# guowentian/dynamicppr

Hardware: AMD Instinct MI355X
Metric: edge-updates/sec (ppr_throughput, summed over sources); ms_per_step = mean per-batch PPR update time (higher is better)
Workload: dtype f64

## Files before the change

### dynamicppr_amd/csrc/dppr_engine.hip

```cpp
#include <algorithm>
#include <atomic>
#include <cmath>
#include <cstdio>
#include <cstdlib>
#include <cstring>
#include <future>
#include <mutex>
#include <ctime>
#include <string>
#include <type_traits>
#include <unordered_map>
#include <vector>

#include <hip/hip_runtime.h>
#include <rocprim/rocprim.hpp>

#include "../../include/dppr.h"
#include "dppr_churn_plan.hpp"
#include "dppr_cut.hpp"
#include "dppr_devbuf.hpp"
#include "dppr_idspace.hpp"
#include "dppr_loop_plan.hpp"
#include "dppr_query_plan.hpp"
#include "dppr_kernels.hpp"
#include "dppr_multi.hpp"
#include "dppr_gpush.hpp"
#include "dppr_binned.hpp"
#include "dppr_calib.hpp"
#include "dppr_topk.hpp"
#include "dppr_wquery.hpp"
#include "dppr_changes.hpp"
#include "dppr_export.hpp"
#include "dppr_patch.hpp"
#include "dppr_dot.hpp"
#include "dppr_walk.hpp"
#include "dppr_cluster.hpp"
#include "dppr_subgraph.hpp"
#include "dppr_rank.hpp"
#include "dppr_assign.hpp"
#include "dppr_position.hpp"
#include "dppr_sample.hpp"
#include "dppr_explain.hpp"

using namespace dppr;

#include "dppr_host_state.hpp"
#include "dppr_host_graph.hpp"
#include "dppr_host_loop.hpp"
#include "dppr_host_group.hpp"
#include "dppr_host_query.hpp"


extern "C" {

int dppr_abi_version(void) { return DPPR_ABI_VERSION; }

const char *dppr_strerror(int status) {
    switch (status) {
    case DPPR_OK: return "ok";
    case DPPR_ERR_INVALID: return "invalid argument or call order";
    case DPPR_ERR_HIP: return "HIP runtime error";
    case DPPR_ERR_NOMEM: return "out of device memory";
    case DPPR_ERR_NO_DEVICE: return "no usable HIP device (the HIP path is mandatory; there is no CPU fallback)";
    case DPPR_ERR_NOT_CONVERGED: return "iteration cap hit before the frontier emptied";
    default: return "unknown status";
    }
}

const char *dppr_last_error(const dppr_engine *e) { return e ? e->err.c_str() : ""; }

int dppr_device_count(void) {
    int n = 0;
    return hipGetDeviceCount(&n) == hipSuccess ? n : 0;
}

int dppr_create(dppr_engine **out, int device, int32_t V, int32_t W, int directed, int32_t c, int32_t n_epochs) {
    if (!out || V <= 0 || W < 0 || c < 0 || n_epochs < 1) return DPPR_ERR_INVALID;
    *out = nullptr;
    int ndev = 0;
    if (hipGetDeviceCount(&ndev) != hipSuccess || ndev <= 0 || device < 0 || device >= ndev) return DPPR_ERR_NO_DEVICE;
    dppr_engine *e = new dppr_engine();
    dppr::g_live_engines.fetch_add(1, std::memory_order_relaxed);
    auto bail = [&](int code) {
        dppr_destroy(e);
        return code;
    };
#define HIP_TRY_C(call)                                                                 \
    do {                                                                                \
        const hipError_t _e = static_cast<hipError_t>(call);                            \
        if (_e != hipSuccess) {                                                         \
            fprintf(stderr, "dppr_create: %s at line %d\n", hipGetErrorString(_e), __LINE__); \
            return bail(_e == hipErrorOutOfMemory ? DPPR_ERR_NOMEM : DPPR_ERR_HIP);     \
        }                                                                               \
    } while (0)
    auto diag_env = [](const char *name) -> const char * {
        const char *v = getenv(name);
        if (v && !getenv("DPPR_QUIET_SWITCHES")) fprintf(stderr, "dppr_create: diagnostic switch %s=%s in effect (INTEGRATION.md, Environment variables)\n", name, v);
        return v;
    };
    if (const char *v = diag_env("DPPR_SWEEP_BITS")) e->sweep_bits = atoi(v) != 0;
    if (const char *v = diag_env("DPPR_HOT_BLOCKS")) e->hot_blocks = atoi(v) != 0;
    if (const char *v = diag_env("DPPR_GSWEEP_HOT")) e->gsweep_hot_rows = std::max(0, atoi(v));
    if (const char *v = diag_env("DPPR_GSWEEP_GRID")) e->gsweep_grid_cap = std::max(1, std::min(atoi(v), STAT_SLOTS));
    if (const char *v = diag_env("DPPR_RENUMBER")) e->renumber_on = atoi(v) != 0;
    if (const char *v = diag_env("DPPR_RENUMBER_PCT")) e->renumber_growth_pct = std::max(1, atoi(v));
    if (const char *v = diag_env("DPPR_RENUMBER_MIN")) e->renumber_min_parked = std::max(1, atoi(v));
    if (const char *v = diag_env("DPPR_GROUP_PUSH")) e->gpush_enter_pairs = std::max(-1, atoi(v));
    if (const char *v = diag_env("DPPR_GROUP_PUSH_FACTOR")) e->gpush_auto_factor = std::max(1, atoi(v));
    if (const char *v = diag_env("DPPR_GGROUPS_MIN")) e->ggroups_min = std::max(1, atoi(v));
    if (const char *v = diag_env("DPPR_COST_MODEL")) e->cost_model = atoi(v) != 0;
    if (const char *v = diag_env("DPPR_GROUPING_RADIX")) e->force_radix_grouping = atoi(v) != 0;
    if (const char *v = diag_env("DPPR_TEST_MERGE_MISS")) e->test_force_merge_miss = atoi(v) != 0;
    if (const char *v = diag_env("DPPR_BIN_INCREMENTAL")) e->bin_incremental = atoi(v) != 0;
    if (const char *v = diag_env("DPPR_BIN_RECUT_EVERY")) e->bin_recut_every = std::max(1, atoi(v));
    if (const char *v = diag_env("DPPR_BIN_FROZEN_REBUILD")) e->bin_frozen_rebuild = atoi(v) != 0;
    if (const char *v = diag_env("DPPR_GROUP_AT_SLIDE")) e->group_at_slide = atoi(v) != 0;
    if (const char *v = diag_env("DPPR_GROUP_FULL_ROWS")) e->group_full_rows = atoi(v) != 0;
    e->device = device;
    e->V = V;
    e->W = W;
    e->c = c;
    e->directed = directed ? 1 : 0;
    e->n_epochs = n_epochs;
    e->Ed = directed ? W : 2 * W;
    e->bits = 1;
    while ((1ll << e->bits) < (long long)V) e->bits++;
    HIP_TRY_C(hipSetDevice(device));
    HIP_TRY_C(hipStreamCreateWithFlags(&e->stream, hipStreamNonBlocking));
    {
        int least = 0, greatest = 0;
        if (hipDeviceGetStreamPriorityRange(&least, &greatest) != hipSuccess) least = 0;
        HIP_TRY_C(hipStreamCreateWithPriority(&e->bs, hipStreamNonBlocking, least));
    }
    HIP_TRY_C(hipEventCreate(&e->ev0));
    HIP_TRY_C(hipEventCreate(&e->ev1));
    for (auto &ev : e->evpool) HIP_TRY_C(hipEventCreate(&ev));
    HIP_TRY_C(e->dump_pin.alloc(dppr_engine::DUMP_PIN_BYTES));
    HIP_TRY_C(e->pinned.alloc((GMULTI_MAX + 2) * GS_MAX + 3 * GS_MAX + MAX_CHUNK * GS_MAX + 16));
    const size_t Wn = (size_t)std::max(W, 1), Edn = (size_t)std::max(e->Ed, 1), Ln = (size_t)std::max(4 * c, 1);
    HIP_TRY_C(e->w1.alloc(Wn));
    HIP_TRY_C(e->w2.alloc(Wn));
    HIP_TRY_C(e->outdeg.alloc((size_t)V));
    HIP_TRY_C(hipMemsetAsync(e->outdeg, 0, sizeof(int) * (size_t)V, e->stream));
    HIP_TRY_C(e->hub_slot_of.alloc((size_t)V));
    HIP_TRY_C(e->d_ext2int.alloc((size_t)V));
    HIP_TRY_C(e->d_xfer.alloc((size_t)V));
    e->init_ids(V);
    HIP_TRY_C(e->hub_hist.alloc(64));
    HIP_TRY_C(e->bar.alloc(1));
    HIP_TRY_C(e->keys_a.alloc(Edn));
    HIP_TRY_C(e->keys_b.alloc(Edn));
    HIP_TRY_C(e->in_sorted.alloc(Edn));
    if (e->directed) HIP_TRY_C(e->out_sorted.alloc(Edn));
    HIP_TRY_C(e->delpos.alloc((size_t)2 * (size_t)std::max(c, 1) + 16));
    {
        const size_t bn = (size_t)std::max(2 * c, 1);
        for (int k = 0; k < 4; ++k) {
            HIP_TRY_C(e->bk[k].alloc(bn));
            HIP_TRY_C(e->bks[k].alloc(bn));
        }
    }
    HIP_TRY_C(rocprim::radix_sort_keys(nullptr, e->sort_tmp_bytes, e->keys_a.get(), e->keys_b.get(), Edn, 0u,
                                       (unsigned)(2 * e->bits), e->stream));
    HIP_TRY_C(e->sort_tmp.alloc(std::max<size_t>(e->sort_tmp_bytes, 16)));
    for (int k = 0; k < 2; ++k) {
        HIP_TRY_C(e->su_k[k].alloc(Ln));
        HIP_TRY_C(e->su_v[k].alloc(Ln));
    }
    HIP_TRY_C(e->su_grp.alloc(4 * SU_GRP_MAX_BUCKETS + 8));
    HIP_TRY_C(hipMemsetAsync(e->su_grp, 0, sizeof(int) * (4 * SU_GRP_MAX_BUCKETS + 8), e->stream));
    HIP_TRY_C(e->su_term.alloc(Ln * GS_MAX));
    HIP_TRY_C(e->su_ins.alloc(Ln));
    HIP_TRY_C(rocprim::radix_sort_pairs(nullptr, e->su_tmp_bytes, e->su_k[0].get(), e->su_k[1].get(), e->su_v[0].get(), e->su_v[1].get(), Ln,
                                        0u, (unsigned)e->bits, e->stream));
    HIP_TRY_C(e->su_tmp.alloc(std::max<size_t>(e->su_tmp_bytes, 16)));
    e->epochs.resize((size_t)n_epochs);
    for (auto &ep : e->epochs) {
        HIP_TRY_C(ep.row_ptr.alloc((size_t)V + 1));
        HIP_TRY_C(ep.adj.alloc(Edn));
        HIP_TRY_C(ep.out_row_ptr.alloc((size_t)V + 1));
        HIP_TRY_C(ep.out_col.alloc(Edn));
        HIP_TRY_C(ep.b1.alloc(Ln));
        HIP_TRY_C(ep.b2.alloc(Ln));
        HIP_TRY_C(ep.deg_after.alloc(Ln));
        HIP_TRY_C(ep.ins.alloc(Ln));
        HIP_TRY_C(ep.sk.alloc(Ln));
        HIP_TRY_C(ep.sv.alloc(Ln));
        HIP_TRY_C(ep.grp_tile.alloc((size_t)V / WAVE + 3));
        HIP_TRY_C(ep.ggrp_tile.alloc((size_t)V / WAVE + 3));
        HIP_TRY_C(ep.hub_v.alloc(HUB_CAP));
        HIP_TRY_C(ep.hub_degp1.alloc(HUB_CAP));
    }
    HIP_TRY_C(hipStreamSynchronize(e->stream));
#undef HIP_TRY_C
    *out = e;
    return DPPR_OK;
}

void dppr_destroy(dppr_engine *e) {
    if (!e) return;
    if (e->pre.task.valid()) e->pre.task.wait();
    (void)hipSetDevice(e->device);
    if (e->stream) (void)hipStreamSynchronize(e->stream);
    if (e->bs) (void)hipStreamSynchronize(e->bs);
    if (e->ev0) (void)hipEventDestroy(e->ev0);
    if (e->ev1) (void)hipEventDestroy(e->ev1);
    for (auto &ev : e->evpool)
        if (ev) (void)hipEventDestroy(ev);
    if (e->stream) (void)hipStreamDestroy(e->stream);
    if (e->bs) (void)hipStreamDestroy(e->bs);
    dppr::g_live_engines.fetch_sub(1, std::memory_order_relaxed);
    delete e;
}

int dppr_set_schedule(dppr_engine *e, int schedule) {
    if (!e || (schedule != DPPR_SCHEDULE_EAGER && schedule != DPPR_SCHEDULE_SYNC)) return DPPR_ERR_INVALID;
    e->schedule = schedule;
    return DPPR_OK;
}

int dppr_set_batch_grouping(dppr_engine *e, int at_slide) {
    if (!e) return DPPR_ERR_INVALID;
    e->group_at_slide = at_slide != 0;
    return DPPR_OK;
}

int dppr_set_variant(dppr_engine *e, int variant) {
    if (!e || variant < 0 || variant > 3) return fail(e, DPPR_ERR_INVALID, "set_variant: 0 OPTIMIZED, 1 FAST_FRONTIER, 2 EAGER, 3 VANILLA");
    e->schedule = (variant == 1 || variant == 3) ? DPPR_SCHEDULE_SYNC : DPPR_SCHEDULE_EAGER;
    e->pre_extract = variant == 1 || variant == 3;
    e->status_dedup = variant == 2 || variant == 3;
    return DPPR_OK;
}

int dppr_set_phase_merge(dppr_engine *e, int on, int eps_divisor) {
    if (!e || eps_divisor < 0 || eps_divisor > 1024) return fail(e, DPPR_ERR_INVALID, "set_phase_merge: eps_divisor 1..1024 (0 keeps it)");
    e->merge_phases = on != 0;
    if (eps_divisor > 0) e->merge_div = eps_divisor;
    return DPPR_OK;
}

int dppr_set_profiling(dppr_engine *e, int on) {
    if (!e) return DPPR_ERR_INVALID;
    e->profiling = on != 0;
    return DPPR_OK;
}

int dppr_set_persistent(dppr_engine *e, int mode, int64_t timeout_us) {
    if (!e || mode < 0 || mode > 2 || e->loaded || !e->slots.empty())
        return fail(e, DPPR_ERR_INVALID, "set_persistent: call right after dppr_create, mode 0, 1 or 2");
    e->persist_mode = mode;
    if (timeout_us > 0) e->persist_ticks = (unsigned long long)timeout_us * 100ull;
    if (timeout_us < 0) {
        e->persist_ticks = 20000ull;
        e->persist_rollcall_extra = 1;
    }
    return DPPR_OK;
}

int dppr_set_tuning(dppr_engine *e, int hub_min_degree, int big_row_edges, int pull_min_frontier, int chunk_iters,
                    int pull_block) {
    if (!e || hub_min_degree < 1 || big_row_edges < 1 || e->loaded || !e->slots.empty())
        return fail(e, DPPR_ERR_INVALID, "set_tuning: call right after dppr_create, values >= 1");
    e->hub_min_degree = hub_min_degree;
    e->big_row = big_row_edges;
    e->pull_min_frontier = pull_min_frontier;
    if (chunk_iters > 0) {
        e->chunk_iters = std::min(chunk_iters, MAX_CHUNK);
        e->chunk_explicit = true;
    }
    if (pull_block >= 256 && pull_block <= 1024 && pull_block % 64 == 0) e->pull_block = pull_block;
    return DPPR_OK;
}

int dppr_set_sweep_bitmap(dppr_engine *e, int on) {
    if (!e) return DPPR_ERR_INVALID;
    e->sweep_bits = on != 0;
    return DPPR_OK;
}

int dppr_set_binned_sweep(dppr_engine *e, int mode, int ha_tiles, int hb_tiles, int64_t target_edges, int64_t min_ids, int64_t chunk_edges,
                          int64_t target_a_edges) {
    if (!e || mode < 0 || mode > 2 || ha_tiles < 0 || ha_tiles > BIN_MAX_HA_TILES || hb_tiles < 0 || hb_tiles > BIN_MAX_HB_TILES || target_edges < 0 || min_ids < 0 ||
        chunk_edges < 0 || target_a_edges < 0 || e->bin_ready || e->loaded)
        return fail(e, DPPR_ERR_INVALID, "set_binned_sweep: call right after dppr_create; mode 0..2, ha_tiles <= 272, hb_tiles <= 120");
    e->bin_mode = mode;
    if (ha_tiles > 0) e->bin_ha_tiles = ha_tiles;
    if (hb_tiles > 0) e->bin_hb_tiles = hb_tiles;
    if (target_edges > 0) e->bin_target = target_edges;
    if (min_ids > 0) e->bin_min_ids = min_ids;
    if (chunk_edges > 0) e->bin_chunk = chunk_edges;
    if (target_a_edges > 0) e->bin_target_a = target_a_edges;
    return DPPR_OK;
}

int dppr_set_resident_slots(dppr_engine *e, int sorted) {
    if (!e) return DPPR_ERR_INVALID;
    e->res_slots = sorted != 0;
    if (!e->res_slots)
        for (auto &ep : e->epochs) ep.res_valid = false;
    return DPPR_OK;
}

int dppr_set_resident_update(dppr_engine *e, int on) {
    if (!e) return DPPR_ERR_INVALID;
    e->res_update = on != 0;
    if (!e->res_update)
        for (auto &ep : e->epochs) ep.su_inline = false;
    return DPPR_OK;
}

int dppr_set_group_resident(dppr_engine *e, int on) {
    if (!e) return DPPR_ERR_INVALID;
    e->group_resident = on != 0;
    return DPPR_OK;
}

int dppr_set_group_push(dppr_engine *e, int enter_pairs, int list_cap, int64_t max_edges) {
    if (!e || enter_pairs < -1 || list_cap < 0 || max_edges < 0) return fail(e, DPPR_ERR_INVALID, "set_group_push: bad argument");
    e->gpush_enter_pairs = enter_pairs;
    if (list_cap > 0) e->gpush_list_cap = list_cap;
    e->gpush_max_edges = max_edges;
    return DPPR_OK;
}

int dppr_set_group_seeding(dppr_engine *e, int from_tails) {
    if (!e) return DPPR_ERR_INVALID;
    e->group_tail_seeding = from_tails != 0;
    return DPPR_OK;
}

int dppr_set_renumbering(dppr_engine *e, int on, int growth_pct, int min_parked) {
    if (!e || growth_pct < 0 || min_parked < 0) return fail(e, DPPR_ERR_INVALID, "set_renumbering: bad argument");
    e->renumber_on = on != 0;
    if (growth_pct > 0) e->renumber_growth_pct = growth_pct;
    if (min_parked > 0) e->renumber_min_parked = min_parked;
    e->renumber_next = std::min(e->renumber_next, renumber_threshold(e->n_int, e->renumber_growth_pct));
    return DPPR_OK;
}

int dppr_id_space(dppr_engine *e, int32_t *n_ids, int32_t *n_parked, int32_t *renumberings, int64_t *revivals) {
    if (!e) return DPPR_ERR_INVALID;
    if (n_ids) *n_ids = e->n_int;
    if (n_parked) *n_parked = e->n_parked;
    if (renumberings) *renumberings = e->renumberings;
    if (revivals) *revivals = e->revivals;
    return DPPR_OK;
}

int dppr_set_incremental_graph(dppr_engine *e, int on) {
    if (!e) return DPPR_ERR_INVALID;
    e->incremental = on != 0;
    return DPPR_OK;
}

int dppr_synchronize(dppr_engine *e) {
    if (!e) return DPPR_ERR_INVALID;
    HIP_TRY(hipSetDevice(e->device));
    HIP_TRY(hipStreamSynchronize(e->stream));
    HIP_TRY(hipStreamSynchronize(e->bs));
    return DPPR_OK;
}

int dppr_load_window(dppr_engine *e, const int32_t *e1, const int32_t *e2, int32_t n) {
    if (!e || n != e->W || (n > 0 && (!e1 || !e2))) return fail(e, DPPR_ERR_INVALID, "load_window: n must equal W");
    HIP_TRY(hipSetDevice(e->device));
    {
        std::vector<std::pair<uint64_t, int32_t>> fresh;
        for (int k = 0; k < 2; ++k) {
            const int32_t *a = k ? e2 : e1;
            for (int i = 0; i < n; ++i) {
                const int v = a[i];
                if (v < 0 || v >= e->V) return fail(e, DPPR_ERR_INVALID, "load_window: vertex id out of range");
                if (e->ext2int[(size_t)v] == -1) {
                    e->ext2int[(size_t)v] = -2;
                    fresh.emplace_back(id_hash(v), v);
                }
            }
        }
        std::vector<int32_t> indeg;
        if (fresh.size() > HOT_WINDOW_MIN) {
            indeg.assign((size_t)e->V, 0);
            for (int i = 0; i < n; ++i) {
                indeg[(size_t)e2[i]]++;
                if (!e->directed) indeg[(size_t)e1[i]]++;
            }
        }
        numbering_order(fresh, indeg.empty() ? nullptr : indeg.data(), e->hot_blocks);
        for (auto &kv : fresh) {
            e->ext2int[(size_t)kv.second] = -1;
            (void)to_int(e, kv.second);
        }
    }
    if (!translate(e, e1, n, e->h_tmp1) || !translate(e, e2, n, e->h_tmp2))
        return fail(e, DPPR_ERR_INVALID, "load_window: vertex id out of range");
    if (n > 0) {
        HIP_TRY(hipMemcpyAsync(e->w1, e->h_tmp1.data(), sizeof(int) * (size_t)n, hipMemcpyHostToDevice, e->bs));
        HIP_TRY(hipMemcpyAsync(e->w2, e->h_tmp2.data(), sizeof(int) * (size_t)n, hipMemcpyHostToDevice, e->bs));
    }
    e->head = 0;
    HIP_TRY(hipMemsetAsync(e->outdeg, 0, sizeof(int) * (size_t)e->V, e->bs));
    if (n > 0) {
        hipLaunchKernelGGL(k_deg_update, dim3(grid_for(n)), dim3(BLOCK), 0, e->bs, e->w1, e->w2, n, e->directed, 1,
                           e->outdeg);
        HIP_TRY(hipGetLastError());
    }
    for (auto &ep : e->epochs) ep.id = -1;
    Epoch &ep = e->epochs[0];
    ep.L = 0;
    ep.grouped = false;
    ep.su_inline = false;
    int rc = query_persist_cap(e);
    if (rc) return rc;
    rc = sort_window_full(e);
    if (rc) return rc;
    rc = build_epoch(e, ep);
    if (rc) return rc;
    ep.id = 0;
    e->newest = 0;
    e->renumber_next = renumber_threshold(e->n_int, e->renumber_growth_pct);
    e->loaded = true;
    e->batch_staged = false;
    HIP_TRY(hipStreamSynchronize(e->bs));
    return DPPR_OK;
}

int dppr_hint_next_batch(dppr_engine *e, const int32_t *b1, const int32_t *b2, int32_t L, const int32_t *n1, const int32_t *n2, int32_t c) {
    if (!e || e->broken || L < 0 || L > 4 * e->c || c < 0 || c > e->c || (L > 0 && (!b1 || !b2)) || (c > 0 && (!n1 || !n2))) return DPPR_ERR_INVALID;
    pre_join(e);
    dppr_engine::Pre &pr = e->pre;
    const int32_t *src[4] = {b1, b2, n1, n2};
    const int n[4] = {L, L, c, c};
    for (int k = 0; k < 4; ++k) {
        pr.src[k] = src[k];
        pr.n[k] = n[k];
        pr.out[k].resize((size_t)std::max(n[k], 1));
    }
    pr.epoch = e->renumber_epoch;
    pr.armed = true;
    pr.ok = false;
    pr.task = std::async(std::launch::async, [e] {
        bool ok = true;
        for (int k = 0; k < 4; ++k)
            if (e->pre.n[k] > 0) ok = e->lookup_only(e->pre.src[k], (size_t)e->pre.n[k], e->pre.out[k].data(), e->pre.miss[k]) && ok;
        return ok;
    });
    return DPPR_OK;
}

int dppr_set_batch(dppr_engine *e, const int32_t *b1, const int32_t *b2, const uint8_t *ins, int32_t L) {
    if (!e || e->broken || L < 0 || L > 4 * e->c || (L > 0 && (!b1 || !b2 || !ins)))
        return fail(e, DPPR_ERR_INVALID, "set_batch: length exceeds 4*max_batch");
    std::lock_guard<std::mutex> map_lk(e->map_mu);
    if (!ids_in_range(e, b1, L) || !ids_in_range(e, b2, L) || !translate(e, b1, L, e->st_b1) || !translate(e, b2, L, e->st_b2))
        return fail(e, DPPR_ERR_INVALID, "set_batch: vertex id out of range");
    e->st_b1.resize((size_t)L);
    e->st_b2.resize((size_t)L);
    e->st_ins.assign(ins, ins + L);
    e->batch_staged = true;
    HIP_TRY(hipSetDevice(e->device));
    return flush_moves(e);
}

static int slide_impl(dppr_engine *e, const int32_t *n1, const int32_t *n2, int32_t c, int32_t *out_epoch);

int dppr_slide(dppr_engine *e, const int32_t *n1, const int32_t *n2, int32_t c, int32_t *out_epoch) {
    if (e) e->build_concurrent = false;
// ... 461 lines not shown
    HIP_TRY(hipGetLastError());
    int n = 0;
    int rc = read_count(e, s.cnt + 4, &n);
    if (rc) return rc;
    if (n > 0) {
        HIP_TRY(hipMemcpyAsync(out_ids, s.ft[1], sizeof(int) * (size_t)n, hipMemcpyDeviceToHost, e->stream));
        HIP_TRY(hipStreamSynchronize(e->stream));
    }
    if (e->n_parked > 0 && eps < s.park_eps) {
        const int base = e->V - e->n_parked;
        int m = 0;
        HIP_TRY(hipMemsetAsync(s.cnt + 4, 0, sizeof(int), e->stream));
        hipLaunchKernelGGL(k_inspect, dim3(grid_for(e->n_parked, BLOCK * INSPECT_ITEMS)), dim3(BLOCK), 0, e->stream, s.r + base,
                           e->n_parked, phase, eps, s.ft[1], s.cnt + 4);
        HIP_TRY(hipGetLastError());
        rc = read_count(e, s.cnt + 4, &m);
        if (rc) return rc;
        if (m > 0) {
            HIP_TRY(hipMemcpyAsync(out_ids + n, s.ft[1], sizeof(int) * (size_t)m, hipMemcpyDeviceToHost, e->stream));
            HIP_TRY(hipStreamSynchronize(e->stream));
            for (int i = n; i < n + m; ++i) out_ids[i] += base;
        }
        n += m;
    }
    for (int i = 0; i < n; ++i) out_ids[i] = e->int2ext[(size_t)out_ids[i]];
    *out_count = n;
    return DPPR_OK;
}

int dppr_graph_edges(dppr_engine *e, int32_t epoch, int32_t *out) {
    if (!e || !out) return DPPR_ERR_INVALID;
    GET_EPOCH(e, epoch);
    *out = ep.Ed;
    return DPPR_OK;
}

static void csr_to_external(const dppr_engine *e, const std::vector<int> &irow, const std::vector<int> &icol,
                            int32_t *row_ptr, int32_t *col) {
    int off = 0;
    std::vector<int> tmp;
    for (int v = 0; v < e->V; ++v) {
        if (row_ptr) row_ptr[v] = off;
        const int m = e->ext2int[(size_t)v];
        if (m >= 0) {
            tmp.clear();
            for (int j = irow[(size_t)m]; j < irow[(size_t)m + 1]; ++j) tmp.push_back(e->int2ext[(size_t)icol[(size_t)j]]);
            std::sort(tmp.begin(), tmp.end());
            if (col) std::copy(tmp.begin(), tmp.end(), col + off);
            off += (int)tmp.size();
        }
    }
    if (row_ptr) row_ptr[e->V] = off;
}

int dppr_read_graph(dppr_engine *e, int32_t epoch, int32_t *row_ptr, int32_t *col, int32_t *out_degree) {
    if (!e) return DPPR_ERR_INVALID;
    GET_EPOCH(e, epoch);
    HIP_TRY(hipSetDevice(e->device));
    std::vector<int> irow((size_t)e->V + 1), icol((size_t)std::max(ep.Ed, 1)), ideg((size_t)e->V);
    HIP_TRY(hipMemcpyAsync(irow.data(), ep.row_ptr, sizeof(int) * ((size_t)e->V + 1), hipMemcpyDeviceToHost, e->stream));
    if (ep.Ed > 0) {
        int *tmp = reinterpret_cast<int *>(e->keys_a.get());
        hipLaunchKernelGGL(k_split_adj, dim3(grid_for(ep.Ed)), dim3(BLOCK), 0, e->stream, ep.adj, ep.Ed, tmp);
        HIP_TRY(hipGetLastError());
        HIP_TRY(hipMemcpyAsync(icol.data(), tmp, sizeof(int) * (size_t)ep.Ed, hipMemcpyDeviceToHost, e->stream));
    }
    HIP_TRY(hipMemcpyAsync(ideg.data(), e->outdeg, sizeof(int) * (size_t)e->V, hipMemcpyDeviceToHost, e->stream));
    HIP_TRY(hipStreamSynchronize(e->stream));
    csr_to_external(e, irow, icol, row_ptr, col);
    if (out_degree)
        for (int v = 0; v < e->V; ++v) {
            const int m = e->ext2int[(size_t)v];
            out_degree[v] = m >= 0 ? ideg[(size_t)m] : 0;
        }
    return DPPR_OK;
}

int dppr_read_out_graph(dppr_engine *e, int32_t epoch, int32_t *row_ptr, int32_t *col) {
    if (!e) return DPPR_ERR_INVALID;
    GET_EPOCH(e, epoch);
    HIP_TRY(hipSetDevice(e->device));
    std::vector<int> irow((size_t)e->V + 1), icol((size_t)std::max(ep.Ed, 1));
    HIP_TRY(hipMemcpyAsync(irow.data(), ep.out_row_ptr, sizeof(int) * ((size_t)e->V + 1), hipMemcpyDeviceToHost, e->stream));
    if (ep.Ed > 0)
        HIP_TRY(hipMemcpyAsync(icol.data(), ep.out_col, sizeof(int) * (size_t)ep.Ed, hipMemcpyDeviceToHost, e->stream));
    HIP_TRY(hipStreamSynchronize(e->stream));
    csr_to_external(e, irow, icol, row_ptr, col);
    return DPPR_OK;
}

int dppr_trace_enable(dppr_engine *e, int32_t slot, int on) {
    GET_SLOT(e, slot);
    s.trace = on != 0;
    s.trace_ids.clear();
    s.trace_off.assign(1, 0);
    return DPPR_OK;
}

int dppr_trace_get(dppr_engine *e, int32_t slot, int64_t *n_iters, int64_t *n_ids, int64_t *offsets, int32_t *ids) {
    GET_SLOT(e, slot);
    const int64_t ni = s.trace_off.empty() ? 0 : (int64_t)s.trace_off.size() - 1;
    if (n_iters) *n_iters = ni;
    if (n_ids) *n_ids = (int64_t)s.trace_ids.size();
    if (offsets && !s.trace_off.empty()) memcpy(offsets, s.trace_off.data(), sizeof(int64_t) * s.trace_off.size());
    if (ids && !s.trace_ids.empty()) memcpy(ids, s.trace_ids.data(), sizeof(int32_t) * s.trace_ids.size());
    return DPPR_OK;
}

#define GET_GROUP(e, gid)                                                                             \
    if (!(e) || (gid) < 0 || (gid) >= (int)(e)->groups.size()) return fail((e), DPPR_ERR_INVALID, "bad group"); \
    if ((e)->broken) return fail((e), DPPR_ERR_INVALID, "engine unusable after a failed renumbering");           \
    Group &g = (e)->groups[(size_t)(gid)]

static_assert(TG_LANES == GS_MAX, "dppr_targets_plan.hpp plans for the group size of dppr_multi.hpp");
static_assert(TG_SET_MAX == DPPR_TARGET_SET_MAX, "dppr_targets_plan.hpp restates DPPR_TARGET_SET_MAX of include/dppr.h");

static int tg_upload(dppr_engine *e, const TargetSets &ts, DevBuf<unsigned char> &buf, TgTable &tab) {
    tab = tg_table(ts, [&](int32_t ext) { return e->ext2int[(size_t)ext]; });
    std::vector<unsigned char> blob(tg_bytes(tab.total()));
    tg_pack(tab, blob.data());
    HIP_TRY(hipMemcpyAsync(buf, blob.data(), blob.size(), hipMemcpyHostToDevice, e->stream));
    HIP_TRY(hipStreamSynchronize(e->stream));
    return DPPR_OK;
}

static void launch_group_init(dppr_engine *e, Group &g) {
    if (g.tsets.n > 0) {
        hipLaunchKernelGGL(k_tg_init, dim3(grid_for((int64_t)e->V * g.gw)), dim3(BLOCK), 0, e->stream, g.p.get(), g.r.get(), e->V, g.gw);
        hipLaunchKernelGGL(k_tg_scatter, dim3(grid_for(g.ttab.total())), dim3(BLOCK), 0, e->stream, g.r.get(), e->V, g.gw, tg_dev(g), 0, g.n);
    } else {
        hipLaunchKernelGGL(k_ginit, dim3(grid_for((int64_t)e->V * g.gw)), dim3(BLOCK), 0, e->stream, g.p, g.r, e->V, g.gw, g.src);
    }
}

static int add_group(dppr_engine *e, const int32_t *sources, int32_t n, const TargetSets *ts, int32_t *out_group) {
    HIP_TRY(hipSetDevice(e->device));
    Group g;
    g.n = n;
    g.gw = e->group_full_rows ? (n > OCT ? 2 * OCT : OCT) : row_width(n);
    g.spl = row_spl(g.gw);
    for (int s = 0; s < GS_MAX; ++s) g.src.s[s] = -1;
    for (int s = 0; s < n; ++s) g.src_ext[s] = sources[s];
    const size_t V = (size_t)e->V;
    g.act_bytes = (V / 32 + 1024 / 32 + 4) * sizeof(uint32_t);
    const size_t xw = (size_t)x_stride(g.gw);
    HIP_TRY_MSG("add_source_group: ", g.p.alloc((size_t)g.gw * V));
    HIP_TRY_MSG("add_source_group: ", g.r.alloc((size_t)g.gw * V));
    HIP_TRY_MSG("add_source_group: ", g.x.alloc(xw * V));
    HIP_TRY_MSG("add_source_group: ", g.x2.alloc(xw * V));
    HIP_TRY_MSG("add_source_group: ", g.act[0].alloc(g.act_bytes / sizeof(uint32_t)));
    HIP_TRY_MSG("add_source_group: ", g.act[1].alloc(g.act_bytes / sizeof(uint32_t)));
    HIP_TRY_MSG("add_source_group: ", g.cnt.alloc(5 * GS_MAX + MAX_CHUNK * GS_MAX));
    HIP_TRY_MSG("add_source_group: ", g.mlog.alloc((size_t)(GMULTI_MAX + 2) * GS_MAX));
    HIP_TRY_MSG("add_source_group: ", g.dstats.alloc(2));
    HIP_TRY_MSG("add_source_group: ", g.gq.alloc(3 * GQ_PAD));
    HIP_TRY_MSG("add_source_group: ", hipMemsetAsync(g.gq, 0, sizeof(int) * 3 * GQ_PAD, e->stream));
    HIP_TRY_MSG("add_source_group: ", hipMemsetAsync(g.act[0], 0, g.act_bytes, e->stream));
    HIP_TRY_MSG("add_source_group: ", hipMemsetAsync(g.act[1], 0, g.act_bytes, e->stream));
    HIP_TRY_MSG("add_source_group: ", hipMemsetAsync(g.cnt, 0, sizeof(int) * (5 * GS_MAX + MAX_CHUNK * GS_MAX), e->stream));
    HIP_TRY_MSG("add_source_group: ", hipMemsetAsync(g.dstats, 0, 2 * sizeof(IterStats), e->stream));
    if (ts) HIP_TRY_MSG("add_target_group: ", g.tg.alloc(tg_bytes(ts->total())));
    if (ts) {
        for (int s = 0; s < n; ++s)
            for (const TgSeed &sd : ts->lane[s]) (void)to_int(e, sd.id);
    } else {
        for (int s = 0; s < n; ++s) (void)to_int(e, sources[s]);
    }
    for (int s = 0; s < n; ++s) g.src.s[s] = sources[s] >= 0 ? e->ext2int[(size_t)sources[s]] : -1;
    if (int rc = flush_moves(e)) return rc;
    if (ts) {
        g.tsets = *ts;
        if (int rc = tg_upload(e, g.tsets, g.tg, g.ttab)) return rc;
    }
    launch_group_init(e, g);
    HIP_TRY_MSG("add_source_group: ", hipGetLastError());
    HIP_TRY_MSG("add_source_group: ", hipStreamSynchronize(e->stream));
    if (g.spl == 2) e->wide_groups = true;
    e->groups.push_back(std::move(g));
    e->any_groups = true;
    if (int rc = recut_stale_groups(e)) return rc;
    if (out_group) *out_group = (int)e->groups.size() - 1;
    return DPPR_OK;
}

int dppr_add_source_group(dppr_engine *e, const int32_t *sources, int32_t n, int32_t *out_group) {
    if (!e || e->broken || !sources || n < 1 || n > GS_MAX) return fail(e, DPPR_ERR_INVALID, "add_source_group: 1..16 sources");
    if (!ids_in_range(e, sources, n)) return fail(e, DPPR_ERR_INVALID, "add_source_group: vertex out of range");
    return add_group(e, sources, n, nullptr, out_group);
}

int dppr_add_target_group(dppr_engine *e, const int64_t *offsets, const int32_t *ids, const double *weights, int32_t n, int32_t *out_group) {
    if (!e || e->broken) return fail(e, DPPR_ERR_INVALID, "add_target_group: no usable engine");
    if (const TgCheck c = tg_check(offsets, ids, weights, n, e->V))
        return fail(e, DPPR_ERR_INVALID, (std::string("add_target_group: ") + tg_check_text(c)).c_str());
    const TargetSets ts = tg_build(offsets, ids, weights, n);
    int32_t sources[GS_MAX];
    tg_sources(ts, sources);
    return add_group(e, sources, n, tg_has_set(ts) ? &ts : nullptr, out_group);
}

int dppr_group_init_solve(dppr_engine *e, int32_t group, double eps, float *out_ms) {
    return dppr_group_init_solve_at(e, group, -1, eps, out_ms);
}

int dppr_group_init_solve_at(dppr_engine *e, int32_t group, int32_t epoch, double eps, float *out_ms) {
    GET_GROUP(e, group);
    GET_EPOCH(e, epoch);
    if (!(eps > 0)) return fail(e, DPPR_ERR_INVALID, "eps must be positive");
    HIP_TRY(hipSetDevice(e->device));
    int rc = bracket_open(e);
    if (rc) return rc;
    launch_group_init(e, g);
    HIP_TRY(hipGetLastError());
    g.converged = false;
    g.park_eps = 0.0;
    rc = group_loop(e, g, ep, 0, eps, false);
    if (rc) return rc;
    return solve_finished(e, g, eps, ep.id, false, out_ms);
}

int dppr_group_update(dppr_engine *e, int32_t group, int32_t epoch, double eps, float *out_ms) {
    GET_GROUP(e, group);
    GET_EPOCH(e, epoch);
    if (!(eps > 0)) return fail(e, DPPR_ERR_INVALID, "eps must be positive");
    if (!epoch_in_sequence(g.last_epoch, ep.id)) return fail(e, DPPR_ERR_INVALID, "epoch out of sequence for this group");
    HIP_TRY(hipSetDevice(e->device));
    return group_update(e, g, ep, eps, out_ms);
}

int dppr_group_read(dppr_engine *e, int32_t group, int32_t index, double *p, double *r) {
    GET_GROUP(e, group);
    if (index < 0 || index >= g.n) return fail(e, DPPR_ERR_INVALID, "group_read: bad source index");
    HIP_TRY(hipSetDevice(e->device));
    std::lock_guard<std::mutex> map_lk(e->map_mu);
    int rc = sync_map(e);
    if (rc) return rc;
    const double *src[2] = {g.p, g.r};
    double *dst[2] = {p, r};
    for (int k = 0; k < 2; ++k) {
        if (!dst[k]) continue;
        hipLaunchKernelGGL(k_gint_to_ext, dim3(grid_for(e->V)), dim3(BLOCK), 0, e->stream, src[k], g.gw, index, e->d_ext2int,
                           e->V, e->d_xfer);
        HIP_TRY(hipMemcpyAsync(dst[k], e->d_xfer, sizeof(double) * (size_t)e->V, hipMemcpyDeviceToHost, e->stream));
        HIP_TRY(hipStreamSynchronize(e->stream));
    }
    return DPPR_OK;
}

static_assert(CHURN_LANES == GS_MAX, "dppr_churn_plan.hpp plans for the group size of dppr_multi.hpp");
static constexpr bool churn_geometry_agrees() {
    for (int n = 1; n <= GS_MAX; ++n)
        if (churn_row_width(n, false) != row_width(n) || churn_row_spl(row_width(n)) != row_spl(row_width(n)) ||
            churn_row_width(n, true) != (n > OCT ? 2 * OCT : OCT))
            return false;
    return true;
}
static_assert(churn_geometry_agrees(), "dppr_churn_plan.hpp restates row_width / row_spl of dppr_multi.hpp");
static_assert(PLAN_RES_MAX_SWEEPS == RES_MAX_SWEEPS && PLAN_GPUSH_LOG == GPUSH_LOG && PLAN_TINY_N == TINY_N && PLAN_TINY_E == TINY_E,
              "dppr_loop_plan.hpp restates RES_MAX_SWEEPS of dppr_resident.hpp and GPUSH_LOG / TINY_N / TINY_E of dppr_gpush.hpp");
static_assert(LOOP_PHASE_BOTH == PHASE_BOTH, "dppr_loop_plan.hpp restates PHASE_BOTH of dppr_common.hpp");

int dppr_group_sources(dppr_engine *e, int32_t group, int32_t *out_sources, int32_t *out_n) {
    GET_GROUP(e, group);
    if (out_sources)
        for (int s = 0; s < g.n; ++s) out_sources[s] = g.src_ext[s];
    if (out_n) *out_n = g.n;
    return DPPR_OK;
}

static int group_churn(dppr_engine *e, int32_t group, ChurnOp op, int32_t index, int32_t new_source, int32_t *out_index, float *out_ms,
                       const std::vector<TgSeed> *fresh = nullptr) {
    const char *const what[3] = {fresh ? "group_replace_target" : "group_replace_source", "group_add_source", "group_remove_source"};
    if (fresh && tg_is_source(*fresh)) {
        new_source = (*fresh)[0].id;
        fresh = nullptr;
    }
    auto refuse = [&](const char *why) { return fail(e, DPPR_ERR_INVALID, (std::string(what[op]) + ": " + why).c_str()); };
    GET_GROUP(e, group);
    const ChurnPlan pl = churn_plan(op, g.n, g.gw, index, e->group_full_rows, e->wide_groups);
    if (!pl.ok) return refuse(op == CHURN_ADD ? "the group holds 16 sources" : op == CHURN_REMOVE && g.n <= 1 ? "the last source of a group cannot be removed" : "bad source index");
    if (op != CHURN_REMOVE && !fresh && (new_source < 0 || new_source >= e->V)) return refuse("vertex out of range");
    if (!g.converged || g.last_epoch < 0) return refuse("the group is not converged (solve or update it first)");
    Epoch *epp = find_epoch(e, g.last_epoch);
    if (!epp) return refuse("the epoch the group was last solved on is not resident any more");
    const Epoch &ep = *epp;
    HIP_TRY(hipSetDevice(e->device));
    const size_t V = (size_t)e->V;
    const bool new_x = x_stride(pl.gw) != x_stride(g.gw);
    DevBuf<double> p2, r2, x_new, x2_new;
    if (pl.relayout) {
        HIP_TRY(p2.alloc((size_t)pl.gw * V));
        HIP_TRY(r2.alloc((size_t)pl.gw * V));
    }
    if (new_x) {
        HIP_TRY(x_new.alloc((size_t)x_stride(pl.gw) * V));
        HIP_TRY(x2_new.alloc((size_t)x_stride(pl.gw) * V));
    }
    TargetSets nts;
    DevBuf<unsigned char> tg_new;
    if (g.tsets.n > 0 || fresh) {
        TargetSets base = g.tsets;
        if (base.n == 0) {
            base.n = g.n;
            for (int s = 0; s < g.n; ++s) base.lane[s] = tg_source_lane(g.src_ext[s]);
        }
        nts = tg_relane(base, pl.map, pl.n, pl.lane, pl.lane < 0 ? std::vector<TgSeed>() : fresh ? *fresh : tg_source_lane(new_source));
        if (!tg_has_set(nts)) nts = TargetSets();
        else HIP_TRY(tg_new.alloc(tg_bytes(nts.total())));
    }
    int src_int = -1;
    if (op != CHURN_REMOVE) {
        if (fresh) {
            for (const TgSeed &sd : *fresh) (void)to_int(e, sd.id);
// ... 279 lines not shown
int dppr_group_subgraph(dppr_engine *e, int32_t group, int32_t epoch, int32_t k, double min_p, int64_t cap, int dest, int32_t *out_counts,
                        int64_t *out_offsets, int32_t *out_ids, double *out_p, int64_t *out_row_ptr, int32_t *out_col) {
    GET_GROUP(e, group);
    GET_EPOCH(e, epoch);
    return subgraph_call(e, view(g), ep, k, min_p, cap, dest, out_counts, out_offsets, out_ids, out_p, out_row_ptr, out_col);
}

int dppr_debug_subgraph_wave_max(dppr_engine *e, int wave_max) {
    if (!e || !sg_wave_max_ok(wave_max)) return fail(e, DPPR_ERR_INVALID, "debug_subgraph_wave_max: 0 (every row by the histogram kernel) .. 256");
    e->sg_wave_max = wave_max;
    return DPPR_OK;
}

int dppr_topk_ranked(dppr_engine *e, int32_t slot, int32_t epoch, const dppr_rank_spec_t *spec, int32_t k, double min_score, int32_t *out_ids,
                     double *out_score, int32_t *out_count) {
    GET_SLOT(e, slot);
    return topk_ranked_call(e, s, epoch, spec, k, min_score, out_ids, out_score, out_count);
}

int dppr_group_topk_ranked(dppr_engine *e, int32_t group, int32_t epoch, const dppr_rank_spec_t *spec, int32_t k, double min_score,
                           int32_t *out_ids, double *out_score, int32_t *out_counts) {
    GET_GROUP(e, group);
    return topk_ranked_call(e, g, epoch, spec, k, min_score, out_ids, out_score, out_counts);
}

int dppr_rank_score_at(dppr_engine *e, int32_t slot, int32_t epoch, const dppr_rank_spec_t *spec, const int32_t *ids, int32_t m,
                       double *out_score) {
    GET_SLOT(e, slot);
    return rank_score_at_call(e, s, epoch, spec, ids, m, out_score);
}

int dppr_group_rank_score_at(dppr_engine *e, int32_t group, int32_t epoch, const dppr_rank_spec_t *spec, const int32_t *ids, int32_t m,
                             double *out_score) {
    GET_GROUP(e, group);
    return rank_score_at_call(e, g, epoch, spec, ids, m, out_score);
}

int dppr_assign(dppr_engine *e, const int32_t *groups, int32_t n_groups, const double *scale, double min_score, int dest, int32_t *out_label,
                double *out_best, double *out_margin, int64_t *out_counts, const int32_t *prev_label, int64_t cap, int64_t *out_n_flips,
                int32_t *flip_id, int32_t *flip_old, int32_t *flip_new) {
    return assign_call(e, groups, n_groups, scale, min_score, dest, out_label, out_best, out_margin, out_counts, prev_label, cap, out_n_flips,
                       flip_id, flip_old, flip_new);
}

int dppr_assign_at(dppr_engine *e, const int32_t *groups, int32_t n_groups, const double *scale, double min_score, const int32_t *ids, int32_t m,
                   int32_t *out_label, double *out_best, int32_t *out_second_label, double *out_margin) {
    return assign_at_call(e, groups, n_groups, scale, min_score, ids, m, out_label, out_best, out_second_label, out_margin);
}

int dppr_debug_rank_piece(dppr_engine *e, int edges) {
    if (!e || !rank_piece_ok(edges)) return fail(e, DPPR_ERR_INVALID, "debug_rank_piece: 1 .. 512 entries of a row per wave");
    e->rk_piece = edges;
    return DPPR_OK;
}

int dppr_position_at(dppr_engine *e, int32_t slot, int32_t epoch, const dppr_rank_spec_t *spec, double min_score, const int32_t *ids, int32_t m,
                     int32_t *out_pos, int32_t *out_count) {
    GET_SLOT(e, slot);
    return position_call(e, s, epoch, spec, min_score, ids, m, out_pos, out_count);
}

int dppr_group_position_at(dppr_engine *e, int32_t group, int32_t epoch, const dppr_rank_spec_t *spec, double min_score, const int32_t *ids,
                           int32_t m, int32_t *out_pos, int32_t *out_counts) {
    GET_GROUP(e, group);
    return position_call(e, g, epoch, spec, min_score, ids, m, out_pos, out_counts);
}

int dppr_debug_position_tile(dppr_engine *e, int queries) {
    if (!e || !position_tile_ok(queries))
        return fail(e, DPPR_ERR_INVALID, "debug_position_tile: 1 .. 4096 queries of a lane's order per workgroup and pass, 0: the plan's choice");
    e->pos_tile = queries;
    return DPPR_OK;
}

int dppr_explain_at(dppr_engine *e, int32_t slot, int32_t epoch, const int32_t *ids, int32_t m, int32_t f, int32_t depth,
                    const dppr_explain_out_t *out) {
    GET_SLOT(e, slot);
    return explain_call(e, s, epoch, ids, m, f, depth, out);
}

int dppr_group_explain_at(dppr_engine *e, int32_t group, int32_t epoch, const int32_t *ids, int32_t m, int32_t f, int32_t depth,
                          const dppr_explain_out_t *out) {
    GET_GROUP(e, group);
    return explain_call(e, g, epoch, ids, m, f, depth, out);
}

int dppr_debug_explain(dppr_engine *e, int memo, int wave_rows) {
    if (!e || !ex_hook_ok(memo, wave_rows))
        return fail(e, DPPR_ERR_INVALID, "debug_explain: memo -1 (the plan's choice), 0 or 1; 1 .. 64 entries of a row per wave and step");
    e->ex_memo = memo;
    e->ex_wave_rows = wave_rows;
    return DPPR_OK;
}

int dppr_certify(dppr_engine *e, int32_t slot, int32_t epoch, double eps, int flags, dppr_certify_out_t *out) {
    GET_SLOT(e, slot);
    return certify_call(e, s, epoch, eps, flags, out);
}

int dppr_group_certify(dppr_engine *e, int32_t group, int32_t epoch, double eps, int flags, dppr_certify_out_t *out) {
    GET_GROUP(e, group);
    return certify_call(e, g, epoch, eps, flags, out);
}

int dppr_debug_certify(dppr_engine *e, int piece_edges, int wave_rows) {
    if (!e || !cert_hook_ok(piece_edges, wave_rows))
        return fail(e, DPPR_ERR_INVALID, "debug_certify: piece_edges in [0, 2^20], wave_rows 0 or a power of two up to 64 (0: the plan's choice)");
    e->cert_piece = piece_edges;
    e->cert_wave_rows = wave_rows;
    return DPPR_OK;
}

int dppr_sample(dppr_engine *e, int32_t slot, int32_t epoch, const dppr_rank_spec_t *spec, double min_score, uint64_t seed, uint64_t first, int32_t S,
                int dest, int32_t *out_ids, double *out_w, double *out_total, int32_t *out_support, int32_t *out_status) {
    GET_SLOT(e, slot);
    return sample_call(e, s, epoch, spec, min_score, seed, first, S, dest, out_ids, out_w, out_total, out_support, out_status);
}

int dppr_group_sample(dppr_engine *e, int32_t group, int32_t epoch, const dppr_rank_spec_t *spec, double min_score, uint64_t seed, uint64_t first,
                      int32_t S, int dest, int32_t *out_ids, double *out_w, double *out_total, int32_t *out_support, int32_t *out_status) {
    GET_GROUP(e, group);
    return sample_call(e, g, epoch, spec, min_score, seed, first, S, dest, out_ids, out_w, out_total, out_support, out_status);
}

int dppr_debug_sample_form(dppr_engine *e, int form) {
    if (!e || !sample_form_ok(form))
        return fail(e, DPPR_ERR_INVALID, "debug_sample_form: 0 (a wave rebuilds the lowest levels) or 1 (one draw per thread, every level stored)");
    e->sample_form = form;
    return DPPR_OK;
}

int dppr_debug_id_map(dppr_engine *e, int32_t *out_ext2int) {
    if (!e || e->broken || !out_ext2int) return fail(e, DPPR_ERR_INVALID, "debug_id_map: non-null out_ext2int");
    std::lock_guard<std::mutex> map_lk(e->map_mu);
    memcpy(out_ext2int, e->ext2int.data(), sizeof(int32_t) * (size_t)e->V);
    return DPPR_OK;
}

int dppr_debug_walk_form(dppr_engine *e, int form) {
    if (!e || (form != 0 && form != 1)) return fail(e, DPPR_ERR_INVALID, "debug_walk_form: 0 (lane refill) or 1 (one walk per thread)");
    e->walk_form = form;
    return DPPR_OK;
}

int dppr_debug_query_ms(dppr_engine *e, float *out_ms) {
    if (!e || !out_ms) return DPPR_ERR_INVALID;
    *out_ms = e->query_ms;
    return DPPR_OK;
}

int dppr_group_reset_stats(dppr_engine *e, int32_t group) {
    GET_GROUP(e, group);
    HIP_TRY(hipSetDevice(e->device));
    return solve_reset_stats(e, g);
}

int dppr_group_stats(dppr_engine *e, int32_t group, dppr_stats_t *out) {
    GET_GROUP(e, group);
    if (!out) return DPPR_ERR_INVALID;
    HIP_TRY(hipSetDevice(e->device));
    return solve_stats(e, g, out);
}

#ifdef DPPR_STAMPS
extern "C" int dppr_debug_bin_stamps(unsigned long long *out, int which, int rows) {
    return hipMemcpyFromSymbol(out, HIP_SYMBOL(dppr::g_bin_stamps), sizeof(unsigned long long) * 6 * (size_t)rows,
                               sizeof(unsigned long long) * 6 * 16384 * (size_t)which) == hipSuccess ? 0 : -2;
}
extern "C" int dppr_debug_stamps(unsigned long long *out, int rows) {
    return hipMemcpyFromSymbol(out, HIP_SYMBOL(dppr::g_stamps), sizeof(unsigned long long) * 8 * (size_t)rows) == hipSuccess
               ? 0 : -2;
}
#endif

int dppr_bench_atomics(int device, int64_t table_elems, int64_t n, int scope, int reps, float *out_ms) {
    if (table_elems <= 0 || (table_elems & (table_elems - 1)) || n <= 0 || reps <= 0 || !out_ms) return DPPR_ERR_INVALID;
    if (int rc = calib_device(device)) return rc;
    DevBuf<double> table, sink;
    if (table.alloc((size_t)table_elems) != 0) return DPPR_ERR_NOMEM;
    (void)sink.alloc(1);
    (void)hipMemset(table, 0, sizeof(double) * (size_t)table_elems);
    const int grid = 2048;
    return time_launches(reps, out_ms, [&]() {
        if (scope == 2)
            hipLaunchKernelGGL(k_bench_scatter<0>, dim3(grid), dim3(BLOCK), 0, 0, table, (uint64_t)table_elems - 1, n);
        else if (scope == 3)
            hipLaunchKernelGGL(k_bench_scatter<1>, dim3(grid), dim3(BLOCK), 0, 0, table, (uint64_t)table_elems - 1, n);
        else if (scope == 0)
            hipLaunchKernelGGL(k_bench_atomics<__HIP_MEMORY_SCOPE_AGENT>, dim3(grid), dim3(BLOCK), 0, 0, table,
                               (uint64_t)table_elems - 1, n, sink);
        else
            hipLaunchKernelGGL(k_bench_atomics<__HIP_MEMORY_SCOPE_WORKGROUP>, dim3(grid), dim3(BLOCK), 0, 0, table,
                               (uint64_t)table_elems - 1, n, sink);
    });
}

int dppr_bench_line_fills(int device, int64_t table_bytes, int64_t lines, int reps, float *out_ms) {
    if (table_bytes < 128 || (table_bytes & (table_bytes - 1)) || lines <= 0 || reps <= 0 || !out_ms) return DPPR_ERR_INVALID;
    if (int rc = calib_device(device)) return rc;
    DevBuf<double2> table;
    DevBuf<double> sink;
    if (table.alloc((size_t)table_bytes / sizeof(double2)) != 0) return DPPR_ERR_NOMEM;
    (void)sink.alloc(1);
    (void)hipMemset(table, 0, (size_t)table_bytes);
    const int grid = 2048;
    const int per = (int)std::max<int64_t>(8, (lines + (int64_t)grid * 128 - 1) / ((int64_t)grid * 128) / 8 * 8);
    const int rc = time_launches(reps, out_ms, [&]() {
        hipLaunchKernelGGL(k_bench_lines<8>, dim3(grid), dim3(1024), 0, 0, table, (uint64_t)(table_bytes / 128) - 1, per, sink);
    });
    *out_ms = *out_ms * (float)((double)lines / ((double)grid * 128.0 * per));
    return rc;
}

int dppr_bench_stream_copy(int device, int64_t bytes, int reps, float *out_ms) {
    if (bytes < 16 || reps <= 0 || !out_ms) return DPPR_ERR_INVALID;
    if (int rc = calib_device(device)) return rc;
    DevBuf<unsigned char> src, dst;
    if (src.alloc((size_t)bytes) != 0 || dst.alloc((size_t)bytes) != 0) return DPPR_ERR_NOMEM;
    (void)hipMemset(src, 0, (size_t)bytes);
    (void)hipMemset(dst, 0, (size_t)bytes);
    return time_launches(reps, out_ms, [&]() {
        hipLaunchKernelGGL(k_bench_copy, dim3(4096), dim3(1024), 0, 0, reinterpret_cast<const double2 *>(src.get()),
                           reinterpret_cast<double2 *>(dst.get()), bytes / 16);
    });
}

int dppr_debug_bin_tables(dppr_engine *e, int32_t epoch, int32_t *n_a, int32_t *n_b, int32_t *n_edges, int32_t *n_runs, int32_t *n_tiles,
                          int32_t *acut, int32_t *bcut, uint16_t *hl, int32_t *tdelta, int32_t *tb, uint16_t *dl, int32_t *vb,
                          int64_t *patched, int64_t *rebuilt) {
    if (!e) return DPPR_ERR_INVALID;
    GET_EPOCH(e, epoch);
    if (patched) *patched = e->bin_patched;
    if (rebuilt) *rebuilt = e->bin_rebuilt;
    if (!ep.bin_valid) return fail(e, DPPR_ERR_INVALID, "debug_bin_tables: this epoch has no binned tables");
    HIP_TRY(hipSetDevice(e->device));
    if (n_a) *n_a = ep.n_a;
    if (n_b) *n_b = ep.n_b;
    if (n_edges) *n_edges = ep.Ed;
    if (n_runs) *n_runs = ep.n_runs;
    if (n_tiles) *n_tiles = ep.n_tiles;
    const size_t n_blk = ((size_t)ep.Ed + WAVE - 1) / WAVE, n_rb = ((size_t)ep.n_runs + WAVE - 1) / WAVE;
    if (acut) HIP_TRY(hipMemcpy(acut, ep.acut, sizeof(int) * ((size_t)ep.n_a + 1), hipMemcpyDeviceToHost));
    if (bcut) HIP_TRY(hipMemcpy(bcut, ep.bcut, sizeof(int) * ((size_t)ep.n_b + 1), hipMemcpyDeviceToHost));
    if (hl) HIP_TRY(hipMemcpy(hl, ep.hl, sizeof(uint16_t) * (size_t)ep.n_runs, hipMemcpyDeviceToHost));
    if (tdelta) HIP_TRY(hipMemcpy(tdelta, ep.tdelta, sizeof(int) * (size_t)ep.n_tiles, hipMemcpyDeviceToHost));
    if (tb) HIP_TRY(hipMemcpy(tb, ep.tb, sizeof(int) * (n_rb + 1), hipMemcpyDeviceToHost));
    if (dl) HIP_TRY(hipMemcpy(dl, ep.dl, sizeof(uint16_t) * (size_t)ep.Ed, hipMemcpyDeviceToHost));
    if (vb) HIP_TRY(hipMemcpy(vb, ep.vb, sizeof(int) * (n_blk + 1), hipMemcpyDeviceToHost));
    return DPPR_OK;
}

int dppr_debug_live_bytes(int64_t *device_bytes, int64_t *pinned_bytes) {
    if (device_bytes) *device_bytes = dppr::g_device_bytes.load(std::memory_order_relaxed);
    if (pinned_bytes) *pinned_bytes = dppr::g_pinned_bytes.load(std::memory_order_relaxed);
    return DPPR_OK;
}

unsigned long long dppr_heartbeat(const dppr_engine *e) { return e ? e->heartbeat.load(std::memory_order_relaxed) : 0ull; }

#ifndef DPPR_BUILD_ID
#define DPPR_BUILD_ID "unstamped"
#endif
const char *dppr_build_id(void) { return DPPR_BUILD_ID; }

}
```

### dynamicppr_amd/csrc/dppr_host_group.hpp

```cpp
#pragma once

namespace {

template <class F>
void with_row(int gw, int nvx, F &&f) {
    auto narrow = [&](auto w) {
        if (nvx == 512) f(IC<1>{}, w, IC<512>{});
        else f(IC<1>{}, w, IC<1024>{});
    };
    switch (gw) {
    case 2: narrow(IC<2>{}); break;
    case 4: narrow(IC<4>{}); break;
    case 6: narrow(IC<6>{}); break;
    case 8: narrow(IC<8>{}); break;
    case 10: f(IC<2>{}, IC<10>{}, IC<512>{}); break;
    case 12: f(IC<2>{}, IC<12>{}, IC<512>{}); break;
    case 14: f(IC<2>{}, IC<14>{}, IC<512>{}); break;
    default: f(IC<2>{}, IC<16>{}, IC<512>{}); break;
    }
}
template <class F>
void with_row(int gw, F &&f) {
    with_row(gw, 512, [&](auto spl, auto w, auto) { f(spl, w); });
}

struct GSweepLaunch {
    int grid;
    const int *cnt_in;
    int *cnt_out, *cnt_zero;
    int *log;
    int n;
    GridBar *bar = nullptr;
    int *status = nullptr;
    unsigned long long ticks = 0;
    int rollcall_extra = 0;
    int *q_take = nullptr, *q_zero = nullptr;
};
template <bool MULTI>
void launch_gsweep(dppr_engine *e, Group &g, const Epoch &ep, int phase, double eps, bool owed, const GSweepLaunch &a) {
    with_row(g.gw, ep.ggrp_max_tiles * WAVE, [&](auto spl, auto gw, auto nvx) {
        auto go = [&](auto cm) {
            hipLaunchKernelGGL((k_gsweep<decltype(spl)::value, decltype(gw)::value, decltype(nvx)::value, MULTI, decltype(cm)::value>),
                               dim3(a.grid), dim3(GNT), 0, e->stream, ep.grp_n_int, ep.gtab, ep.n_ggroups, a.cnt_in, e->gsweep_hot_rows,
                               ep.out_col, g.x, g.x2, g.act[0], g.act[1], g.r, g.p, a.cnt_out, a.cnt_zero, phase, eps, g.dstats + 1, a.log,
                               a.n, a.bar, a.status, a.ticks, a.rollcall_extra, owed ? 1 : 0, a.q_take, a.q_zero);
        };
        if constexpr (MULTI) go(IC<2>{});
        else if (owed) go(IC<1>{});
        else go(IC<0>{});
    });
}

int group_multi_capacity(dppr_engine *e, int spl) {
    int &cap = e->gmulti_cap[spl - 1];
    if (cap < 0) {
        int per_cu = 0, cus = 0;
        hipError_t rc = spl == 1 ? hipOccupancyMaxActiveBlocksPerMultiprocessor(&per_cu, k_gsweep<1, 8, 1024, true, 2>, GNT, 0)
                                 : hipOccupancyMaxActiveBlocksPerMultiprocessor(&per_cu, k_gsweep<2, 16, 512, true, 2>, GNT, 0);
        if (rc != hipSuccess || hipDeviceGetAttribute(&cus, hipDeviceAttributeMultiprocessorCount, e->device) != hipSuccess)
            per_cu = 0;
        cap = std::min(per_cu * cus, STAT_SLOTS);
    }
    return cap;
}

struct PushTail {
    enum How { NOT_ENTERED, CONVERGED, GAVE_BACK } how = NOT_ENTERED;
    int iters = 0;
    bool owed = false;
};

int group_push_tail(dppr_engine *e, Group &g, const Epoch &ep, int phase, double eps, long long pairs_at_entry, PushTail *t) {
    const int cap = std::max(1024, std::min(e->gpush_list_cap, e->V));
    if (g.plist[0].capacity() != (size_t)cap || !g.pctl) {
        HIP_TRY(loop_wait(e));
        g.plist[0].reset(); g.plist[1].reset(); g.ppre.reset(); g.pctl.reset();
        HIP_TRY(g.plist[0].alloc((size_t)cap));
        HIP_TRY(g.plist[1].alloc((size_t)cap));
        HIP_TRY(g.ppre.alloc((size_t)cap + 1));
        HIP_TRY(g.pctl.alloc(1));
    }
    HIP_TRY(hipMemsetAsync(g.pctl, 0, sizeof(GPushCtl), e->stream));
    const int n_words = (ep.grp_n_int + 31) / 32;
    hipLaunchKernelGGL(k_gpush_list, dim3(grid_for(n_words)), dim3(BLOCK), 0, e->stream, g.act[0], n_words, g.plist[0], cap, g.pctl);
    const int rows_grid = grid_for(std::min<long long>(pairs_at_entry, cap), BLOCK / OCT);
    with_row(g.gw, [&](auto spl, auto gw) {
        hipLaunchKernelGGL((k_gpush_rows<decltype(spl)::value, decltype(gw)::value>), dim3(rows_grid), dim3(BLOCK), 0, e->stream, g.plist[0],
                           g.pctl, 0, g.x, g.r, false);
    });
    HIP_TRY(hipGetLastError());
    static thread_local GPushCtl h;
    const int credit_first = t->owed ? 1 : 0;
    const long long max_edges = gpush_edge_bound(e->gpush_max_edges, ep.n_ggroups);
    const int grid = 256;
    static const bool trace = getenv("DPPR_GROUP_TRACE") != nullptr;
    int it_done = 0;
    long long known_n = pairs_at_entry;
    bool tiny_declined = false;
    long long last_adds = gpush_adds_at_entry(pairs_at_entry);
    for (;;) {
        if (gpush_take_tiny(known_n, last_adds, tiny_declined)) {
            with_row(g.gw, [&](auto spl, auto gw) {
                hipLaunchKernelGGL((k_gpush_tiny<decltype(spl)::value, decltype(gw)::value>), dim3(1), dim3(1024), 0, e->stream, g.pctl, g.plist[0],
                                   g.plist[1], ep.row_ptr, ep.adj, ep.hub_degp1, g.r, g.p, g.act[0], phase, eps, g.dstats, GPUSH_LOG, credit_first);
            });
        } else {
        const int m = gpush_chunk(it_done, pairs_at_entry);
        tiny_declined = false;
        for (int k = 0; k < m; ++k) {
            hipLaunchKernelGGL(k_gpush_scan, dim3(1), dim3(1024), 0, e->stream, g.pctl, g.plist[0], g.plist[1], ep.row_ptr, g.ppre, cap - 1, max_edges);
            with_row(g.gw, [&](auto spl, auto gw) {
                constexpr int SPL = decltype(spl)::value, GW = decltype(gw)::value;
                hipLaunchKernelGGL((k_gpush_snap<SPL, GW>), dim3(grid), dim3(BLOCK), 0, e->stream, g.plist[0], g.plist[1], g.pctl, g.x, g.r, g.p,
                                   g.act[0], phase, eps, credit_first);
                hipLaunchKernelGGL((k_gpush_expand<SPL, GW>), dim3(grid), dim3(BLOCK), 0, e->stream, g.plist[0], g.plist[1], g.pctl, g.ppre,
                                   ep.row_ptr, ep.adj, ep.hub_degp1, g.x, g.r, g.act[0], g.plist[0], g.plist[1], cap, phase, eps, g.dstats);
            });
        }
        }
        HIP_TRY(hipGetLastError());
        HIP_TRY(hipMemcpyAsync(&h, g.pctl, sizeof(GPushCtl), hipMemcpyDeviceToHost, e->stream));
        HIP_TRY(loop_wait(e));
        for (int i = it_done; i < h.it; ++i) {
            const long long F = lane_sum(h.F[i & (GPUSH_LOG - 1)]);
            if (F == 0) continue;
            account_iteration(g.st, F, ITER_PUSH);
            ++t->iters;
            if (trace)
                fprintf(stderr, "[gpush ] phase %d iteration +%d  frontier pairs %9lld  adds %lld\n", phase, i, F, h.atomics[i & (GPUSH_LOG - 1)]);
        }
        if (gpush_tiny_declined(h.it > it_done, h.stop != 0, known_n)) tiny_declined = true;
        if (h.it > it_done) last_adds = h.atomics[(h.it - 1) & (GPUSH_LOG - 1)];
        it_done = h.it;
        known_n = h.n[h.it & 1];
        if (h.stop && h.it == 0 && h.overflow) return DPPR_OK;
        if (h.stop) {
            if (trace) fprintf(stderr, "[gpush ] phase %d: an iteration of %d vertices called itself off after %d iterations\n", phase, h.n[h.it & 1], h.it);
            HIP_TRY(hipMemsetAsync(g.cnt, 0, sizeof(int) * 3 * GS_MAX, e->stream));
            with_row(g.gw, [&](auto spl, auto gw) {
                hipLaunchKernelGGL((k_gpush_leave<decltype(spl)::value, decltype(gw)::value>), dim3(grid_for(ep.grp_n_int, BLOCK / OCT)), dim3(BLOCK), 0,
                                   e->stream, ep.grp_n_int, g.act[0], g.x, g.r, g.p, h.it > 0 ? 1 : 0, phase, eps, g.cnt);
            });
            HIP_TRY(hipGetLastError());
            if (h.it > 0) t->owed = false;
            t->how = PushTail::GAVE_BACK;
            return DPPR_OK;
        }
        if (h.n[h.it & 1] == 0) {
            t->how = PushTail::CONVERGED;
            return DPPR_OK;
        }
        if (it_done >= e->max_iters) return fail(e, DPPR_ERR_NOT_CONVERGED, "iteration cap hit");
    }
}

struct GroupLoop {
    dppr_engine *const e;
    Group &g;
    const Epoch &ep;
    const int phase;
    const double eps;
    const int hp = phase == PHASE_BOTH ? 0 : phase;
    CounterRing ring;
    bool owed = false;
    int it = 0, active_iters = 0;
    bool more = false;
    long long F = 0;
    GroupLoopPlan plan;
    int sweep_grid = 1;
    int *row(int k) const { return g.cnt + k * GS_MAX; }

    int multi_chunk() {
        const int n = group_multi_sweeps(g.hist.hint[hp], it, e->chunk_iters, e->chunk_explicit);
        HIP_TRY(hipMemsetAsync(g.mlog, 0, sizeof(int) * (size_t)(n + 2) * GS_MAX, e->stream));
        HIP_TRY(hipMemsetAsync(e->bar, 0, sizeof(GridBar), e->stream));
        int rc = timed_launch(e, 0, e->profiling, [&] {
            launch_gsweep<true>(e, g, ep, phase, eps, owed,
                                {ep.n_ggroups, row(ring.cur), row(3), row(4), g.mlog + GS_MAX, n, e->bar, g.mlog, e->persist_ticks, e->persist_rollcall_extra});
        });
        if (rc) return rc;
        HIP_TRY(hipGetLastError());
        if ((rc = read_back(e, g.mlog, (size_t)(n + 2) * GS_MAX))) return rc;
        const int st = e->pinned[0];
        g.st.persist_launches++;
        if (st & GSM_FAULT) return fail(e, DPPR_ERR_HIP, "a grid barrier of the multi-sweep group launch timed out");
        if (st & GSM_ABORTED) {
            give_up_resident(e, g.st);
            return DPPR_OK;
        }
        const int sweeps = st & GSM_SWEEPS;
        account_sweeps(g.st, e->pinned + GS_MAX, sweeps, GS_MAX, ITER_SWEEP, it, &active_iters);
        if (e->profiling && (rc = credit_launch(e, g.st, 0, false))) return rc;
        if (sweeps & 1) {
            swap_snapshots(g, true);
            owed = !owed;
        }
        it += sweeps;
        more = !(st & GSM_CONVERGED);
        if (!more) return DPPR_OK;
        HIP_TRY(hipMemcpyAsync(row(0), row(3), sizeof(int) * GS_MAX, hipMemcpyDeviceToDevice, e->stream));
        HIP_TRY(hipMemsetAsync(row(1), 0, sizeof(int) * 2 * GS_MAX, e->stream));
        ring.cur = 0;
        more = lane_sum(e->pinned + GS_MAX + sweeps * GS_MAX) > 0;
        return DPPR_OK;
    }
    int sweep_chunk() {
        const int n = plan.next_chunk(g.hist, hp, it, lane_sum(e->pinned + ring.cur * GS_MAX), e->chunk_iters, e->chunk_explicit);
        for (int k = 0; k < n; ++k) {
            int rc = timed_launch(e, k, e->profiling, [&] {
                launch_gsweep<false>(e, g, ep, phase, eps, owed,
                                     {sweep_grid, row(ring.cur), row(ring.nxt()), row(ring.zer()), row(5 + k), 1, nullptr, nullptr, 0, 0,
                                      g.gq + (g.gq_seq % 3) * GQ_PAD, g.gq + ((g.gq_seq + 1) % 3) * GQ_PAD});
            });
            if (rc) return rc;
            swap_snapshots(g, true);
            ring.rotate();
            g.gq_seq++;
            owed = !owed;
        }
        HIP_TRY(hipGetLastError());
        if (int rc = read_back(e, g.cnt, (size_t)(5 + n) * GS_MAX)) return rc;
        int rc = account_sweeps(g.st, e->pinned + 5 * GS_MAX, n, GS_MAX, ITER_SWEEP, it, &active_iters, [&](int k, long long f) -> int {
            plan.saw_frontier(f, it + k);
            if (!e->profiling) return DPPR_OK;
            float ms = 0;
            if (int rc2 = credit_launch(e, g.st, k, true, &ms)) return rc2;
            static const bool trace = getenv("DPPR_GROUP_TRACE") != nullptr;
            if (trace) fprintf(stderr, "[gsweep] phase %d sweep %3d  frontier pairs %9lld  %7.1f us\n", phase, it + k, f, ms * 1e3);
            return DPPR_OK;
        });
        if (rc) return rc;
        F = lane_sum(e->pinned + ring.cur * GS_MAX);
        more = F > 0;
        it += n;
        return DPPR_OK;
    }
    int hand_to_push_tail() {
        plan.saw_frontier(F, it);
        PushTail t;
        t.owed = owed;
        if (int rc = group_push_tail(e, g, ep, phase, eps, F, &t)) return rc;
        owed = t.owed;
        if (t.how != PushTail::NOT_ENTERED) {
            active_iters = it + t.iters;
            it += t.iters;
        }
        if (t.how == PushTail::CONVERGED) more = false;
        else plan.push_declined(F);
        if (t.how != PushTail::GAVE_BACK) return DPPR_OK;
        ring.cur = 0;
        if (int rc = read_back(e, row(0), GS_MAX)) return rc;
        more = lane_sum(e->pinned) > 0;
        return DPPR_OK;
    }
};

int group_loop(dppr_engine *e, Group &g, const Epoch &ep, int phase, double eps, bool tails) {
    GroupLoop l{e, g, ep, phase, eps};
    HIP_TRY(hipMemsetAsync(g.cnt, 0, sizeof(int) * 3 * GS_MAX, e->stream));
    if (tails) {
        HIP_TRY(hipMemsetAsync(g.act[0], 0, g.act_bytes, e->stream));
        if (ep.L > 0) {
            with_row(g.gw, [&](auto spl, auto gw) {
                hipLaunchKernelGGL((k_gseed_tails<decltype(spl)::value, decltype(gw)::value>), dim3(grid_for(ep.L, BLOCK / OCT)), dim3(BLOCK), 0,
                                   e->stream, batch_tails(e, ep), ep.L, g.r, g.x, g.p, g.act[0], phase, eps, l.row(0));
            });
        }
    } else {
        with_row(g.gw, [&](auto spl, auto gw) {
            hipLaunchKernelGGL((k_gseed_dense<decltype(spl)::value, decltype(gw)::value>), dim3(grid_for(ep.grp_n_int, BLOCK / OCT)), dim3(BLOCK), 0,
                               e->stream, ep.grp_n_int, g.r, g.x, g.p, g.act[0], phase, eps, l.row(0));
        });
        g.st.inspected += (int64_t)ep.grp_n_int * g.n;
    }
    HIP_TRY(hipGetLastError());
    int rc = read_back(e, l.row(0), GS_MAX);
    if (rc) return rc;
    l.more = lane_sum(e->pinned) > 0;
    if (e->gsweep_grid_cap <= 0) {
        int cus = 0;
        if (hipDeviceGetAttribute(&cus, hipDeviceAttributeMultiprocessorCount, e->device) != hipSuccess || cus <= 0) cus = 256;
        e->gsweep_grid_cap = std::min(2 * cus, STAT_SLOTS);
    }
    l.sweep_grid = std::min(std::max(ep.n_ggroups, 1), e->gsweep_grid_cap);
    l.plan.push_thr = group_push_threshold(e->gpush_enter_pairs, ep.n_ggroups, e->gpush_auto_factor);
    while (l.more) {
        if (l.it >= e->max_iters) return fail(e, DPPR_ERR_NOT_CONVERGED, "iteration cap hit");
        const int mcap = e->group_resident && e->persist_mode && e->persist_ok && e->chunk_iters > 1 ? group_multi_capacity(e, g.spl) : 0;
        if (mcap > 0 && ep.n_ggroups > 0 && ep.n_ggroups <= mcap) rc = l.multi_chunk();
        else if (!(rc = l.sweep_chunk()) && l.plan.enter_push(l.more, l.F)) rc = l.hand_to_push_tail();
        if (rc) return rc;
    }
    l.plan.finish(g.hist, l.hp, l.active_iters);
    return DPPR_OK;
}

int group_solve_column(dppr_engine *e, Group &g, const Epoch &ep) {
    const LoopHistory kept = g.hist;
    const int rc = group_loop(e, g, ep, 0, g.conv_eps, false);
    g.hist = kept;
    return rc;
}

int group_stream_update(dppr_engine *e, Group &g, const Epoch &ep) {
    const int L = ep.L;
    if (L == 0) return DPPR_OK;
    int rc = group_records_by_tail(e, ep, nullptr, 0, nullptr, 0);
    if (rc) return rc;
    SuSources srcs{};
    for (int s = 0; s < GS_MAX; ++s) srcs.s[s] = g.src.s[s];
    hipLaunchKernelGGL(k_su_terms, dim3(grid_for(L), g.n), dim3(BLOCK), 0, e->stream, batch_tails(e, ep), batch_order(e, ep), ep.b2,
                       ep.ins, L, g.p, g.gw, e->su_term, e->su_ins);
    if (g.tsets.n > 0)
        hipLaunchKernelGGL(k_su_apply_seeded, dim3(grid_for(L), g.n), dim3(BLOCK), 0, e->stream, batch_tails(e, ep), batch_order(e, ep),
                           e->su_term, e->su_ins, ep.deg_after, L, g.r, g.gw, tg_dev(g));
    else
        hipLaunchKernelGGL(k_su_apply, dim3(grid_for(L), g.n), dim3(BLOCK), 0, e->stream, batch_tails(e, ep), batch_order(e, ep), e->su_term,
                           e->su_ins, ep.deg_after, L, g.r, g.gw, srcs, 0.0, (int *)nullptr, (int *)nullptr, (int *)nullptr,
                           (int *)nullptr);
    HIP_TRY(hipGetLastError());
    g.st.records += (int64_t)L * g.n;
    return DPPR_OK;
}

int group_update(dppr_engine *e, Group &g, Epoch &ep, double eps, float *out_ms) {
    const bool merged = e->merge_phases && e->schedule == DPPR_SCHEDULE_EAGER;
    if (merged) eps = eps / e->merge_div;
    const bool tails = g.converged && g.conv_eps <= eps && e->group_tail_seeding;
    int rc = settle_parked(e, g.p, g.r, g.gw, eps, &g.park_eps, &g.st);
    if (rc) return rc;
    rc = prepare_epoch(e, ep);
    if (rc) return rc;
    rc = bracket_open(e);
    if (rc) return rc;
    rc = group_stream_update(e, g, ep);
    if (rc) return rc;
    g.converged = false;
    if (merged) rc = group_loop(e, g, ep, PHASE_BOTH, eps, tails);
    else if (!(rc = group_loop(e, g, ep, 0, eps, tails))) rc = group_loop(e, g, ep, 1, eps, tails);
    if (rc) return rc;
    return solve_finished(e, g, eps, ep.id, true, out_ms);
}

}
```

### dynamicppr_amd/csrc/dppr_host_state.hpp

```cpp
#pragma once

static constexpr int CNT_HDR = 16;
static constexpr int PERSIST_RETRY_BATCHES = 64;
static constexpr int GQ_PAD = 32;
static constexpr int BIN_MAX_BLOCKS = 1 << 16, BIN_MAX_BIG = 4096, BIN_SMALL_INTS = BIN_MAX_BLOCKS + BIN_MAX_BIG + 1 + 64;
static constexpr int SU_SPLIT_MIN = 1 << 16;
static constexpr int MERGE_MISS_WORD = 44;

namespace dppr {

inline std::atomic<long long> g_device_bytes{0}, g_pinned_bytes{0};

struct DeviceAlloc {
    static int alloc(void **p, size_t bytes) {
        const hipError_t rc = hipMalloc(p, bytes);
        if (rc == hipSuccess) g_device_bytes.fetch_add((long long)bytes, std::memory_order_relaxed);
        return (int)rc;
    }
    static int free(void *p, size_t bytes) {
        g_device_bytes.fetch_sub((long long)bytes, std::memory_order_relaxed);
        return (int)hipFree(p);
    }
};

// ... 144 lines not shown
        DevBuf<int> ext;
    } sc;
    struct Weighted {
        DevBuf<double> w;
    } wq;
    struct Changes {
        DevBuf<unsigned char> res; PinBuf<unsigned char> pin;
    } ch;
    struct Export {
        DevBuf<unsigned short> mask;
        DevBuf<int> cnt;
        DevBuf<long long> base;
        DevBuf<unsigned char> blk; PinBuf<unsigned char> pin;
    } ex;
    struct Patch {
        DevBuf<unsigned> mask;
        DevBuf<int> cnt;
        DevBuf<long long> base;
        DevBuf<unsigned char> blk; PinBuf<unsigned char> pin;
    } pt;
    struct Dot {
        DevBuf<double> part;
        DevBuf<unsigned char> in;
        DevBuf<unsigned char> blk; PinBuf<unsigned char> pin;
        dppr::DotTable tb;
        bool lds_set = false;
    } dot;
    struct Walk {
        DevBuf<int> starts;
        DevBuf<int> ends;
        DevBuf<double> res;
        std::vector<int64_t> off;
    } wk;
    struct Cluster {
        DevBuf<unsigned short> rank;
        DevBuf<int> d;
        DevBuf<unsigned long long> list;
        DevBuf<unsigned char> blk; PinBuf<unsigned char> pin;
    } cl;
    struct Subgraph {
        DevBuf<int> work;
        DevBuf<unsigned char> blk; PinBuf<unsigned char> pin;
    } sg;
    struct Rank {
        DevBuf<unsigned> excl;
        DevBuf<int> len; PinBuf<int> len_pin;
        DevBuf<unsigned long long> list;
        std::vector<unsigned long long> items;
    } rk;
    struct Position {
        DevBuf<unsigned char> keys;
        DevBuf<unsigned> slots;
        DevBuf<unsigned char> blk; PinBuf<unsigned char> pin;
        bool lds_set = false;
    } pos;
    struct Sample {
        DevBuf<double> leaves;
        DevBuf<double> nodes;
        DevBuf<double> low;
        DevBuf<unsigned char> blk; PinBuf<unsigned char> pin;
    } sm;
    struct Explain {
        DevBuf<unsigned char> blk; PinBuf<unsigned char> pin;
    } exq;
    struct Certify {
        DevBuf<unsigned char> blk; PinBuf<unsigned char> pin;
        DevBuf<unsigned char> ws;
        DevBuf<double> part;
        DevBuf<unsigned long long> list;
        DevBuf<double> pp;
    } cert;
    struct Assign {
        DevBuf<double> scale;
        DevBuf<int> cnt;
        DevBuf<int> base;
        DevBuf<int> ws;
        DevBuf<unsigned char> blk; PinBuf<unsigned char> pin;
    } as;
};

}

struct dppr_engine : dppr::IdSpace {
    int device = 0;
    int V = 0, W = 0, c = 0, directed = 1, n_epochs = 1;
    int Ed = 0;
    int bits = 1;
    int schedule = DPPR_SCHEDULE_EAGER;
    bool status_dedup = false;
    bool pre_extract = false;
    bool group_at_slide = false;
    int merge_miss_host = 0;
    long long merge_fallbacks = 0;
    bool test_force_merge_miss = false;
    int raw_backoff = 0;
    bool merge_phases = false;
    int merge_div = 4;
    hipStream_t stream = nullptr;
    hipStream_t bs = nullptr;
    bool build_concurrent = false;
    std::mutex err_mu;
    std::mutex map_mu;
    unsigned map_gen_on_device = 0;
    hipEvent_t ev0 = nullptr, ev1 = nullptr;
    hipEvent_t evpool[2 * 64] = {};
    bool profiling = false;
    int pull_block = 0;
    int chunk_iters = 24;
    bool chunk_explicit = false;
    int persist_mode = 1;
    bool persist_ok = true;
    int persist_retry = 0;
    int persist_cap = 0;
    int res_slots = 1;
    int res_update = 1;
    DevBuf<double> res_arena;
    long long res_arena_stride = 0;
    unsigned long long persist_ticks = 5000000ull;
    int persist_rollcall_extra = 0;
    DevBuf<GridBar> bar;
    DevBuf<int> w1, w2;
    int head = 0;
    bool loaded = false;
    bool broken = false;
    DevBuf<int> outdeg;
    DevBuf<int> hub_slot_of;
    DevBuf<int> hub_hist;
    int hub_min_degree = HUB_MIN_DEGREE_DEFAULT;
    int big_row = BIG_ROW_DEFAULT;
    int pull_min_frontier = 0;
    DevBuf<uint64_t> in_sorted, out_sorted;
    DevBuf<uint64_t> keys_a, keys_b;
    DevBuf<unsigned char> sort_tmp;
    size_t sort_tmp_bytes = 0;
    DevBuf<int> su_grp;
    DevBuf<uint64_t> bk[4];
    DevBuf<uint64_t> bks[4];
    DevBuf<int> delpos;
    struct Pre {
        std::future<bool> task;
        const int32_t *src[4] = {nullptr, nullptr, nullptr, nullptr};
        int n[4] = {0, 0, 0, 0};
        std::vector<int32_t> out[4];
        std::vector<uint32_t> miss[4];
        unsigned long long epoch = 0;
        bool armed = false, ok = false;
    } pre;
    long long pre_hits = 0, pre_misses = 0;
    bool incremental = true;
    bool sweep_bits = false;
    bool hot_blocks = true;
    int gsweep_hot_rows = 24576;
    int gsweep_grid_cap = 0;
    bool group_resident = true;
    int gmulti_cap[2] = {-1, -1};
    bool any_groups = false;
    int ggroups_min = 256;
    bool force_radix_grouping = false;
    bool cost_model = true;
    bool group_full_rows = false;
    bool wide_groups = false;
    bool group_tail_seeding = true;
    int gpush_enter_pairs = -1;
    int gpush_list_cap = 1 << 20;
    long long gpush_max_edges = 0;
    int gpush_auto_factor = 2;
    int bin_mode = 1;
    int bin_ha_tiles = 128, bin_hb_tiles = 60;
    long long bin_target = 0;
    long long bin_target_a = 4ll << 20;
    long long bin_min_ids = 1ll << 19;
    DevBuf<int> bin_vblk_a;
    DevBuf<unsigned long long> bin_scan;
    DevBuf<int> bin_small;
    long long bin_chunk = 32768;
    DevBuf<double> bin_vals;
    DevBuf<uint64_t> bin_wb, bin_wa;
    DevBuf<int> bin_first;
    std::vector<int32_t> bin_cut_a, bin_cut_b;
    int bin_abits = 0, bin_bbits = 0;
    int bin_cut_ids = 0;
    bool bin_words_valid = false;
    int bin_slides_since_cut = 0;
    bool bin_incremental = true;
    int bin_recut_every = 32;
    bool bin_frozen_rebuild = false;
    bool bin_force_full = false;
    int bin_miss_host = 0;
    long long bin_patched = 0, bin_rebuilt = 0;
    DevBuf<unsigned char> bin_tmp;
    size_t bin_tmp_bytes = 0;
    bool bin_ready = false;
    std::vector<int32_t> h_tiles_in;
    DevBuf<uint32_t> su_k[2], su_v[2];
    DevBuf<double> su_term;
    DevBuf<uint8_t> su_ins;
    DevBuf<unsigned char> su_tmp;
    size_t su_tmp_bytes = 0;
    std::vector<int32_t> st_b1, st_b2;
    std::vector<uint8_t> st_ins;
    bool batch_staged = false;
    std::vector<Epoch> epochs;
    int newest = -1;
    std::vector<Slot> slots;
    std::vector<Group> groups;
    PinBuf<int> pinned;
    std::atomic<unsigned long long> heartbeat{0};
    PinBuf<char> dump_pin;
    static constexpr size_t DUMP_PIN_BYTES = sizeof(GridBar) + 4096;
    bool renumber_on = true;
    int renumber_growth_pct = 15;
    int renumber_min_parked = 1024;
    int renumber_next = 0;
    int renumberings = 0;
    std::vector<int32_t> mv_src, mv_dst, mv_zero;
    DevBuf<int> mv_idx;
    DevBuf<double> mv_tmp;
    DevBuf<int> d_ext2int;
    DevBuf<double> d_xfer;
    DevBuf<int> d_int2ext;
    unsigned i2e_gen_on_device = 0;
    QueryWork q;
    int walk_form = 0;
    int sg_wave_max = SG_WAVE_MAX;
    int rk_piece = RK_PIECE;
    int sample_form = 0;
    int pos_tile = 0;
    int ex_memo = -1;
    int ex_wave_rows = EX_WAVE_ROWS;
    int cert_piece = 0;
    int cert_wave_rows = 0;
    float query_ms = -1.0f;
    std::vector<int32_t> h_tmp1, h_tmp2;
    std::vector<int32_t> h_tiles;
    int max_iters = 1 << 20;
    std::string err;
};

namespace {

inline void set_err(dppr_engine *e, const char *msg) {
    std::lock_guard<std::mutex> lk(e->err_mu);
    e->err = msg;
}

#define HIP_TRY(call)                                                                                   \
    do {                                                                                                \
        const hipError_t _e = static_cast<hipError_t>(call);                                            \
        if (_e != hipSuccess) {                                                                         \
            char _b[512];                                                                               \
            snprintf(_b, sizeof(_b), "%s in %s at line %d", hipGetErrorString(_e), __FILE__, __LINE__); \
            set_err(e, _b);                                                                             \
            return _e == hipErrorOutOfMemory ? DPPR_ERR_NOMEM : DPPR_ERR_HIP;                           \
        }                                                                                               \
    } while (0)

#define HIP_TRY_MSG(prefix, call)                                                 \
    do {                                                                          \
        const hipError_t _e = static_cast<hipError_t>(call);                      \
        if (_e != hipSuccess) {                                                   \
            set_err(e, (std::string(prefix) + hipGetErrorString(_e)).c_str());    \
            return _e == hipErrorOutOfMemory ? DPPR_ERR_NOMEM : DPPR_ERR_HIP;     \
        }                                                                         \
    } while (0)

inline int grid_for(int64_t n, int per_block = BLOCK, int cap = 2048) {
    int64_t g = (n + per_block - 1) / per_block;
    if (g < 1) g = 1;
    if (g > cap) g = cap;
    return (int)g;
}

constexpr long LOOP_SPIN_US = 2000;
inline hipError_t loop_sync(hipStream_t st) {
    static const bool spin = !(getenv("DPPR_SYNC_SPIN") && atoi(getenv("DPPR_SYNC_SPIN")) == 0);
    if (!spin) return hipStreamSynchronize(st);
    timespec t0;
    clock_gettime(CLOCK_MONOTONIC, &t0);
    hipError_t r;
    unsigned polls = 0;
    while ((r = hipStreamQuery(st)) == hipErrorNotReady) {
        if ((++polls & 15u) == 0) {
            timespec now;
            clock_gettime(CLOCK_MONOTONIC, &now);
            if ((now.tv_sec - t0.tv_sec) * 1000000L + (now.tv_nsec - t0.tv_nsec) / 1000L > LOOP_SPIN_US) return hipStreamSynchronize(st);
        }
        __builtin_ia32_pause();
    }
    return r;
}

inline hipError_t loop_wait(dppr_engine *e) {
    e->heartbeat.fetch_add(1, std::memory_order_relaxed);
    return loop_sync(e->stream);
}

int fail(dppr_engine *e, int code, const char *msg) {
    if (e) set_err(e, msg);
    return code;
}

inline int bracket_open(dppr_engine *e) {
    HIP_TRY(hipEventRecord(e->ev0, e->stream));
    return DPPR_OK;
}
inline int bracket_close(dppr_engine *e, float *ms) {
// ... 72 lines not shown
```

### dynamicppr_amd/csrc/dppr_multi.hpp

```cpp
#pragma once

#include "dppr_kernels.hpp"

namespace dppr {

constexpr int GS_MAX = 16;
constexpr int OCT = 8;

struct SrcN {
    int s[GS_MAX];
};

__device__ __forceinline__ unsigned oct_mask(uint64_t ballot) {
    return (unsigned)(ballot >> (lane_id() & ~(OCT - 1))) & 0xffu;
}

__host__ __device__ constexpr int row_width(int n_sources) { return n_sources <= 2 ? 2 : (n_sources + 1) / 2 * 2; }
__host__ __device__ constexpr int row_spl(int gw) { return gw > OCT ? 2 : 1; }
#ifndef DPPR_X_COMPACT
#define DPPR_X_COMPACT 0
#endif
__host__ __device__ constexpr int x_stride(int gw) { return DPPR_X_COMPACT ? gw : gw > 8 ? 16 : gw > 4 ? 8 : gw; }
template <int SPL, int GW>
__device__ __forceinline__ bool oct_live(int j) {
// ... 63 lines not shown
    if (threadIdx.x < GW && s_cnt[threadIdx.x]) atomicAdd(&cnt_out[threadIdx.x], s_cnt[threadIdx.x]);
}

template <int SPL, int GW>
__global__ __launch_bounds__(BLOCK) void k_gseed_tails(const uint32_t *__restrict__ skeys, int L, const double *__restrict__ r,
                                                       double *__restrict__ x, double *__restrict__ p,
                                                       uint32_t *__restrict__ act, int phase, double eps,
                                                       int *__restrict__ cnt_out) {
    __shared__ int s_cnt[GS_MAX];
    if (threadIdx.x < GS_MAX) s_cnt[threadIdx.x] = 0;
    __syncthreads();
    const int j = threadIdx.x & (OCT - 1);
    const bool live = oct_live<SPL, GW>(j);
    int nleg[SPL];
#pragma unroll
    for (int q = 0; q < SPL; ++q) nleg[q] = 0;
    const int per = BLOCK / OCT;
    const int Lpad = (L + per - 1) / per * per;
    for (int i0 = blockIdx.x * per; i0 < Lpad; i0 += gridDim.x * per) {
        const int i = i0 + (int)threadIdx.x / OCT;
        int u = -1;
        if (i < L) {
            u = (int)skeys[i];
            if (i > 0 && (int)skeys[i - 1] == u) u = -1;
        }
        bool any = false;
        double rv[SPL];
        bool lg[SPL];
#pragma unroll
        for (int q = 0; q < SPL; ++q) {
            rv[q] = u >= 0 && live ? r[(size_t)u * GW + j * SPL + q] : 0.0;
            lg[q] = u >= 0 && live && legal(rv[q], phase, eps);
            any |= lg[q];
            nleg[q] += lg[q] ? 1 : 0;
        }
        if (oct_mask(__ballot(any))) {
            if (live) {
#pragma unroll
                for (int q = 0; q < SPL; ++q) {
                    const size_t k = (size_t)u * GW + j * SPL + q;
                    x[(size_t)u * x_stride(GW) + j * SPL + q] = rv[q];
                    if (lg[q]) p[k] = p[k] + ALPHA * rv[q];
                }
            }
            if (j == 0) atomicOr(&act[u >> 5], 1u << (u & 31));
        }
    }
#pragma unroll
    for (int q = 0; q < SPL; ++q)
        if (nleg[q]) atomicAdd(&s_cnt[j * SPL + q], nleg[q]);
    __syncthreads();
    if (threadIdx.x < GW && s_cnt[threadIdx.x]) atomicAdd(&cnt_out[threadIdx.x], s_cnt[threadIdx.x]);
}

constexpr int GNT = 1024;
constexpr int GT_HDR = 8;
__host__ __device__ constexpr int GT_STRIDE(int nvx) { return (GT_HDR + nvx + 1 + GNT / OCT + nvx / 2 + 3) / 4 * 4; }

template <int NVX>
__global__ __launch_bounds__(GNT) void k_gtables(int V, const int *__restrict__ grp_tile, int n_groups,
                                                 const int *__restrict__ out_row_ptr, int *__restrict__ tables) {
    constexpr int NW = GNT / WAVE, NOCT = GNT / OCT, EB = 8;
    __shared__ int s_wcnt[NW];
    const int tid = threadIdx.x, lane = lane_id(), w = wave_id();
    for (int g = blockIdx.x; g < n_groups; g += gridDim.x) {
        __syncthreads();
        int *T = tables + (size_t)g * GT_STRIDE(NVX);
        const int t0 = grp_tile[g], t1 = grp_tile[g + 1];
        const int v0 = t0 * WAVE;
        const int nv = min((t1 - t0) * WAVE, V - v0);
        const int E0 = out_row_ptr[v0];
        const int Eg = out_row_ptr[v0 + nv] - E0;
        int rs = 0, d = 0;
        if (tid < nv) {
            rs = out_row_ptr[v0 + tid] - E0;
            d = out_row_ptr[v0 + tid + 1] - E0 - rs;
        }
        const int per = ((Eg + NOCT - 1) / NOCT + EB - 1) / EB * EB;
        const uint64_t ne = __ballot(d > 0);
        if (lane == 0) s_wcnt[w] = __popcll(ne);
        __syncthreads();
        int woff = 0, ncomp = 0;
#pragma unroll
        for (int k = 0; k < NW; ++k) {
            const int c = s_wcnt[k];
            woff += k < w ? c : 0;
            ncomp += c;
        }
        int *cstart = T + GT_HDR, *ostart = T + GT_HDR + NVX + 1;
        unsigned short *cvid = reinterpret_cast<unsigned short *>(T + GT_HDR + NVX + 1 + NOCT);
        if (tid <= NVX && tid >= ncomp) cstart[tid] = Eg;
        if (tid == 0 && NVX >= GNT) cstart[NVX] = Eg;
        if (tid < NOCT) ostart[tid] = 0;
        if (tid < NVX && tid >= ncomp) cvid[tid] = 0;
        if (tid == 0) {
            T[0] = v0; T[1] = nv; T[2] = E0; T[3] = Eg; T[4] = per; T[5] = ncomp; T[6] = 0; T[7] = 0;
        }
        asm volatile("s_waitcnt vmcnt(0)" ::: "memory");
        __syncthreads();
        if (d > 0) {
            const int idx = woff + mbcnt(ne);
            cstart[idx] = rs;
            cvid[idx] = (unsigned short)tid;
            const int o_first = (rs + per - 1) / per, o_last = min((rs + d + per - 1) / per - 1, NOCT - 1);
            for (int o = o_first; o <= o_last; ++o) ostart[o] = idx;
        }
    }
}

template <bool COH>
__device__ __forceinline__ double gs_ld(const double *p) {
    if constexpr (COH)
        return __longlong_as_double((long long)__hip_atomic_load(reinterpret_cast<const unsigned long long *>(p),
                                                                 __ATOMIC_RELAXED, __HIP_MEMORY_SCOPE_AGENT));
    else
        return *p;
}
template <bool COH>
__device__ __forceinline__ uint32_t gs_ldu(const uint32_t *p) {
    if constexpr (COH) return __hip_atomic_load(p, __ATOMIC_RELAXED, __HIP_MEMORY_SCOPE_AGENT);
    else return *p;
}
template <bool COH>
__device__ __forceinline__ void gs_st(double *p, double v) {
    if constexpr (COH)
        __hip_atomic_store(reinterpret_cast<unsigned long long *>(p), (unsigned long long)__double_as_longlong(v),
                           __ATOMIC_RELAXED, __HIP_MEMORY_SCOPE_AGENT);
    else
        *p = v;
}
template <bool COH>
__device__ __forceinline__ void gs_stu(uint32_t *p, uint32_t v) {
    if constexpr (COH) __hip_atomic_store(p, v, __ATOMIC_RELAXED, __HIP_MEMORY_SCOPE_AGENT);
    else *p = v;
}

#ifndef DPPR_GS_NT
#define DPPR_GS_NT 0
#endif
#ifndef DPPR_WHATIF
#define DPPR_WHATIF 0
#endif
template <bool COH, int BIT>
__device__ __forceinline__ double gs_ld_once(const double *p) {
    if constexpr (!COH && (DPPR_GS_NT & BIT)) return __builtin_nontemporal_load(p);
    else return gs_ld<COH>(p);
}
template <bool COH, int BIT>
__device__ __forceinline__ void gs_st_once(double *p, double v) {
    if constexpr (!COH && (DPPR_GS_NT & BIT)) __builtin_nontemporal_store(v, p);
    else gs_st<COH>(p, v);
}

constexpr int GSM_ABORTED = 1 << 30;
constexpr int GSM_FAULT = 1 << 29;
constexpr int GSM_CONVERGED = 1 << 28;
constexpr int GSM_SWEEPS = (1 << 16) - 1;

template <int SPL, int GW, int NVX, bool MULTI, int CM>
__global__ __launch_bounds__(GNT, MULTI ? 4 : 8) void k_gsweep(int V, const int *__restrict__ gtab, int n_groups,
                                                   const int *cnt_in, int hot_rows,
                                                   const int *__restrict__ out_col, double *x_a, double *x_b,
                                                   uint32_t *act_a, uint32_t *act_b, double *r, double *p, int *cnt_out,
                                                   int *cnt_zero, int phase, double eps, IterStats *__restrict__ stats,
                                                   int *log_slot, int n_iter, GridBar *bar, int *status,
                                                   unsigned long long limit_ticks, int rollcall_extra, int credit0,
                                                   int *q_take, int *q_zero) {
    constexpr int NOCT = GNT / OCT, WORDS = NVX / 32, XS = x_stride(GW);
    static_assert(sizeof(double) * NVX * GW <= 64 * 1024, "two workgroups per CU");
    constexpr int EB = 8;
    constexpr int GB = EB / SPL;
#ifndef DPPR_GS_FU
#define DPPR_GS_FU (4 / SPL)
#endif
    constexpr int FU_WANT = CM == 0 && SPL == 2 ? 2 * (DPPR_GS_FU) : (DPPR_GS_FU);
    constexpr int FU = MULTI ? NVX / NOCT : FU_WANT <= NVX / NOCT ? FU_WANT : NVX / NOCT;
    static_assert(MULTI == (CM == 2), "the multi-sweep form decides per sweep, a one-sweep launch is compiled for its mode");
    static_assert(NVX % NOCT == 0 && (NVX / NOCT) % FU == 0, "vertex phase covers the group in whole steps");
    __shared__ double s_acc[NVX * GW];
    __shared__ int s_cstart[NVX + 1];
    __shared__ unsigned short s_cvid[NVX];
    __shared__ int s_ostart[NOCT];
    __shared__ uint32_t s_actin[WORDS], s_actout[WORDS], s_touched[WORDS];
    __shared__ int s_cnt[GS_MAX];
    __shared__ unsigned long long s_edges;
    __shared__ int s_flag[2];
    __shared__ int s_ticket;
    const int tid0 = threadIdx.x, lane = lane_id(), w = wave_id();
    const int j = tid0 & (OCT - 1);
    auto opaque = [](int v) {
#ifndef DPPR_NO_OPAQUE
        asm volatile("" : "+v"(v));
#endif
        return v;
    };

    bool stamp_dense = false;
    if constexpr (!MULTI) {
        const int my_cnt = lane < GW ? cnt_in[lane] : 0;
        if (blockIdx.x == 0 && tid0 < GW) {
            cnt_zero[tid0] = 0;
            log_slot[tid0] = my_cnt;
        }
        if (blockIdx.x == 0 && tid0 == 0) *q_zero = 0;
        if (__ballot(my_cnt != 0) == 0) return;
#ifdef DPPR_STAMPS
#if defined(DPPR_STAMP_MID)
        {
            const long long tot = __builtin_amdgcn_readlane(wave_inclusive_scan(my_cnt), WAVE - 1);
            stamp_dense = tot * 16 > (long long)V && tot * 2 < (long long)V;
        }
#elif defined(DPPR_STAMP_SPARSE)
        stamp_dense = (long long)__builtin_amdgcn_readlane(wave_inclusive_scan(my_cnt), WAVE - 1) * 64 < (long long)V;
#else
        stamp_dense = (long long)__builtin_amdgcn_readlane(wave_inclusive_scan(my_cnt), WAVE - 1) > 4ll * V;
#endif
#endif
    }
    (void)stamp_dense;
#ifdef DPPR_STAMPS
    if (stamp_dense) STAMP(7);
    if (!MULTI && stamp_dense && tid0 == 0 && blockIdx.x < 4096) g_stamps[blockIdx.x * 8 + 5] = wall_clock64();
#endif
    for (int k = tid0; k < NVX * GW; k += GNT) s_acc[k] = 0.0;
    if (tid0 < WORDS) {
        s_actout[tid0] = 0u;
        s_touched[tid0] = 0u;
    }
    if (tid0 < GS_MAX) s_cnt[tid0] = 0;
    if (tid0 == 0) {
        s_edges = 0ull;
        s_flag[0] = 1;
        s_flag[1] = 0;
    }
    int nleg[SPL];
#pragma unroll
    for (int q = 0; q < SPL; ++q) nleg[q] = 0;
    unsigned ecount = 0;

    const unsigned G = gridDim.x;
    const unsigned subs_used = G < (unsigned)BAR_SUBS ? G : (unsigned)BAR_SUBS;
    const unsigned long long n_sub = lane < (int)subs_used ? (G - lane + BAR_SUBS - 1) / BAR_SUBS : 0;
    const int my_rep = (blockIdx.x / BAR_SUBS) % BAR_REPS;
    if constexpr (MULTI) {
        const unsigned long long t_entry = wall_clock64();
        __syncthreads();
        if (tid0 == 0)
            __hip_atomic_fetch_add(&bar->roll[blockIdx.x % BAR_SUBS].w, 1ull << 32, __ATOMIC_RELAXED, __HIP_MEMORY_SCOPE_AGENT);
        if (w == 0) {
            if (blockIdx.x == 0) {
                unsigned polls = 0;
                bool all_here = false;
                for (;;) {
                    const unsigned long long word = lane < (int)subs_used ? bar_load(&bar->roll[lane].w) : 0;
                    if (__ballot((word >> 32) >= n_sub + (lane == 0 ? (unsigned long long)rollcall_extra : 0ull)) == ~0ull) {
                        all_here = true;
                        break;
                    }
                    if ((polls++ & 31u) == 0 && (bar_load(&bar->gen.w) != 0 || wall_clock64() - t_entry > limit_ticks)) break;
                    __builtin_amdgcn_s_sleep(1);
                }
                if (lane == 0) (void)bar_cas(&bar->gen.w, 0ull, all_here ? BAR_READY : BAR_ABORT);
            }
            if (lane == 0) {
                unsigned long long word;
                unsigned polls = 0;
                while ((word = bar_load(&bar->gen.w)) == 0) {
                    if ((polls++ & 31u) == 0 && wall_clock64() - t_entry > limit_ticks) (void)bar_cas(&bar->gen.w, 0ull, BAR_ABORT);
                    __builtin_amdgcn_s_sleep(1);
                }
                s_flag[0] = word != BAR_ABORT;
            }
        }
        __syncthreads();
        if (!s_flag[0]) {
            if (blockIdx.x == 0 && tid0 == 0) *status = GSM_ABORTED;
            return;
        }
    }

    constexpr int STRIDE = GT_STRIDE(NVX);
    int hv0 = 0, hnv = 0, hE0 = 0, hEg = 0, hper = 0;
    if ((int)blockIdx.x < n_groups) {
        const int *H = gtab + (size_t)blockIdx.x * STRIDE;
        hv0 = H[0]; hnv = H[1]; hE0 = H[2]; hEg = H[3]; hper = H[4];
    }
    int sweeps_done = 0;
    bool converged = false, fault = false;
    for (int g = blockIdx.x; g < n_groups;) {
        __syncthreads();
        int ticket = 0, g_next = n_groups;
        if (!MULTI && tid0 == 0) ticket = (int)gridDim.x + atomicAdd(q_take, 1);
        const int *T = gtab + (size_t)g * STRIDE;
        const int tid = opaque(tid0);
        const int j = tid & (OCT - 1), oid = tid / OCT;
        const bool live = oct_live<SPL, GW>(j);
        const int v0 = hv0, nv = hnv, E0 = hE0, Eg = hEg, per = hper;
        const int e_begin = oid * per, e_end = min(Eg, e_begin + per);
        const int *cols = out_col + E0;
        {
            const int c0 = tid < NVX ? T[GT_HDR + tid] : 0;
            const int os = tid < NOCT ? T[GT_HDR + NVX + 1 + tid] : 0;
            const unsigned short cv = tid < NVX ? reinterpret_cast<const unsigned short *>(T + GT_HDR + NVX + 1 + NOCT)[tid] : 0;
            if (tid < WORDS) s_actin[tid] = tid * 32 < nv ? gs_ldu<MULTI>(act_a + (v0 >> 5) + tid) : 0u;
            if (tid < NVX) {
                s_cstart[tid] = c0;
                s_cvid[tid] = cv;
            }
            if (tid < NOCT) s_ostart[tid] = os;
            if (tid == 0) s_cstart[NVX] = Eg;
        }
        int mycol = e_begin + j < e_end ? ld_stream(&cols[e_begin + j]) : -1;
        int ncol = e_begin + EB + j < e_end ? ld_stream(&cols[e_begin + EB + j]) : -1;

        for (int it = 0; it < (MULTI ? n_iter : 1); ++it) {
            const double *x = (it & 1) ? x_b : x_a;
            double *x_new = (it & 1) ? x_a : x_b;
            const uint32_t *act_in = (it & 1) ? act_b : act_a;
            uint32_t *act_out = (it & 1) ? act_a : act_b;
            const bool credit = CM == 2 ? ((credit0 ^ it) & 1) != 0 : CM == 1;
            if constexpr (MULTI) {
                const int *row = it == 0 ? cnt_in : log_slot + (size_t)it * GS_MAX;
                const int f = lane < GW ? (int)gs_ldu<true>(reinterpret_cast<const uint32_t *>(row + lane)) : 0;
                if (it == 0 && blockIdx.x == 0 && tid < GW) log_slot[tid] = f;
                if (__ballot(f != 0) == 0) {
                    converged = true;
                    break;
                }
            }
#define GSTAMP(i) do { if (MULTI ? it == 12 : stamp_dense) STAMP(i); } while (0)
            GSTAMP(0);
            if (it > 0) {
                if (tid < WORDS) s_actin[tid] = tid * 32 < nv ? gs_ldu<MULTI>(act_in + (v0 >> 5) + tid) : 0u;
                mycol = e_begin + j < e_end ? ld_stream(&cols[e_begin + j]) : -1;
                ncol = e_begin + EB + j < e_end ? ld_stream(&cols[e_begin + EB + j]) : -1;
            }
            __syncthreads();

            if (e_begin < e_end) {
                int crow = s_ostart[oid];
                int row_beg = s_cstart[crow], row_end = s_cstart[crow + 1];
                double den = (double)(row_end - row_beg + 1);
                double rcp = 1.0 / den;
                double acc[SPL];
#pragma unroll
                for (int q = 0; q < SPL; ++q) acc[q] = 0.0;
                auto flush = [&]() {
                    const int vl = s_cvid[crow];
                    bool nz = false;
#pragma unroll
                    for (int q = 0; q < SPL; ++q) {
                        if (acc[q] != 0.0) lds_add(&s_acc[vl * GW + j * SPL + q], acc[q]);
                        nz |= acc[q] != 0.0;
                        acc[q] = 0.0;
                    }
                    if (nz) atomicOr(&s_touched[vl >> 5], 1u << (vl & 31));
                };
                uint32_t aw = mycol >= 0 ? gs_ldu<MULTI>(act_in + (mycol >> 5)) : 0u;
                for (int e = e_begin; e < e_end; e += EB) {
                    const bool a = mycol >= 0 && ((aw >> (mycol & 31)) & 1u);
                    const uint32_t naw = ncol >= 0 ? gs_ldu<MULTI>(act_in + (ncol >> 5)) : 0u;
                    const int nncol = e + 2 * EB + j < e_end ? ld_stream(&cols[e + 2 * EB + j]) : -1;
                    const unsigned m = oct_mask(__ballot(a));
#pragma unroll
                    for (int h = 0; h < EB; h += GB) {
                        const unsigned mh = (m >> h) & ((1u << GB) - 1u);
                        if (mh) {
                            double xv[GB][SPL];
#pragma unroll
                            for (int k = 0; k < GB; ++k) {
                                const int ck = __shfl(mycol, (lane & ~(OCT - 1)) + h + k, WAVE);
#pragma unroll
                                for (int q = 0; q < SPL; ++q) xv[k][q] = 0.0;
#if DPPR_WHATIF & 4
                                if (((mh >> k) & 1u) && live) { xv[k][0] = 1e-7 * (ck & 7); }
                                else
#endif
#if DPPR_WHATIF & 16
                                if (((mh >> k) & 1u) && live) {
#pragma unroll
                                    for (int q = 0; q < SPL; ++q) xv[k][q] = gs_ld<MULTI>(x + (size_t)(ck & 4095) * XS + j * SPL + q);
                                } else
#endif
                                if (((mh >> k) & 1u) && live) {
                                    if (MULTI || !(DPPR_GS_NT & 1) || ck < hot_rows) {
#pragma unroll
                                        for (int q = 0; q < SPL; ++q) xv[k][q] = gs_ld<MULTI>(x + (size_t)ck * XS + j * SPL + q);
                                    } else {
#pragma unroll
                                        for (int q = 0; q < SPL; ++q) xv[k][q] = gs_ld_once<MULTI, 1>(x + (size_t)ck * XS + j * SPL + q);
                                    }
                                }
                            }
#pragma unroll
                            for (int k = 0; k < GB; ++k) {
                                if ((mh >> k) & 1u) {
                                    const int ek = e + h + k;
                                    if (ek >= row_end) {
                                        flush();
                                        do {
                                            ++crow;
                                            row_beg = row_end;
                                            row_end = s_cstart[crow + 1];
                                        } while (ek >= row_end);
                                        den = (double)(row_end - row_beg + 1);
                                        rcp = 1.0 / den;
                                    }
#pragma unroll
                                    for (int q = 0; q < SPL; ++q) {
                                        if (legal(xv[k][q], phase, eps)) {
                                            acc[q] += push_term(xv[k][q], den, rcp);
                                            ++ecount;
                                        }
                                    }
                                }
                            }
                        }
                    }
                    mycol = ncol;
                    aw = naw;
                    ncol = nncol;
                }
                flush();
            }
            if (!MULTI && tid0 == 0) s_ticket = ticket;
            GSTAMP(1);
            __syncthreads();
            GSTAMP(2);
            if constexpr (!MULTI) {
                g_next = __builtin_amdgcn_readfirstlane(s_ticket);
                if (g_next < n_groups) {
                    const int *H = gtab + (size_t)g_next * STRIDE;
                    hv0 = H[0]; hnv = H[1]; hE0 = H[2]; hEg = H[3]; hper = H[4];
                }
            }

            for (int i0 = 0; i0 < NVX / NOCT; i0 += FU) {
                const int tid_v = opaque(tid0);
                const int j = tid_v & (OCT - 1), oid = tid_v / OCT;
                const bool live = oct_live<SPL, GW>(j);
                int vl[FU];
                bool tch[FU], wasact[FU];
                double cur[FU][SPL], pv[FU][SPL];
#pragma unroll
                for (int i = 0; i < FU; ++i) {
                    vl[i] = oid + (i0 + i) * NOCT;
                    const unsigned bit = 1u << (vl[i] & 31);
                    wasact[i] = (s_actin[vl[i] >> 5] & bit) != 0;
                    tch[i] = vl[i] < nv && (wasact[i] || (s_touched[vl[i] >> 5] & bit) != 0);
#pragma unroll
                    for (int q = 0; q < SPL; ++q) {
                        cur[i][q] = 0.0;
                        pv[i][q] = 0.0;
                    }
                    if (tch[i] && live) {
                        const size_t base = (size_t)(v0 + vl[i]) * GW + j * SPL;
                        const double *row = wasact[i] ? x + (size_t)(v0 + vl[i]) * XS + j * SPL : r + base;
#pragma unroll
                        for (int q = 0; q < SPL; ++q) {
#if DPPR_WHATIF & 2
                            if (!wasact[i])
#endif
                            cur[i][q] = gs_ld_once<MULTI, 2>(row + q);
#if DPPR_WHATIF & 2
                            else cur[i][q] = 1.0;
#endif
#if !(DPPR_WHATIF & 1)
                            if (credit) pv[i][q] = gs_ld_once<MULTI, 2>(p + base + q);
#endif
                        }
                    }
                }
#pragma unroll
                for (int i = 0; i < FU; ++i) {
                    if (tch[i]) {
                        const size_t base = (size_t)(v0 + vl[i]) * GW + j * SPL;
                        double rn[SPL];
                        bool lg[SPL], pushed[SPL], any = false, changed = false;
#pragma unroll
                        for (int q = 0; q < SPL; ++q) {
                            double a = 0.0;
                            if (live) {
                                double *ap = &s_acc[vl[i] * GW + j * SPL + q];
                                a = *ap;
                                *ap = 0.0;
                            }
                            pushed[q] = wasact[i] && legal(cur[i][q], phase, eps);
                            rn[q] = pushed[q] ? a : cur[i][q] + a;
                            lg[q] = legal(rn[q], phase, eps);
                            any |= lg[q];
                            changed |= rn[q] != cur[i][q];
                            nleg[q] += lg[q] ? 1 : 0;
                        }
#if !(DPPR_WHATIF & 1)
                        if (credit && live) {
#pragma unroll
                            for (int q = 0; q < SPL; ++q) {
                                if (pushed[q] || lg[q]) {
                                    double pn = pv[i][q];
                                    if (pushed[q]) pn = pn + ALPHA * cur[i][q];
                                    if (lg[q]) pn = pn + ALPHA * rn[q];
                                    gs_st_once<false, 4>(p + base + q, pn);
                                }
                            }
                        }
#endif
                        if (oct_mask(__ballot(any))) {
                            if (live && !(DPPR_WHATIF & 8)) {
#pragma unroll
                                for (int q = 0; q < SPL; ++q) gs_st_once<MULTI, 4>(x_new + (size_t)(v0 + vl[i]) * XS + j * SPL + q, rn[q]);
                            }
                            if (j == 0) atomicOr(&s_actout[vl[i] >> 5], 1u << (vl[i] & 31));
                        } else if ((wasact[i] || changed) && live) {
#pragma unroll
                            for (int q = 0; q < SPL; ++q) gs_st_once<false, 4>(r + base + q, rn[q]);
                        }
                    }
                }
            }
            GSTAMP(3);
            __syncthreads();
            GSTAMP(4);
            if (tid < WORDS) {
                if (tid * 32 < nv) gs_stu<MULTI>(act_out + (v0 >> 5) + tid, s_actout[tid]);
                s_actout[tid] = 0u;
                s_touched[tid] = 0u;
            }
            if constexpr (MULTI) {
#pragma unroll
                for (int q = 0; q < SPL; ++q) {
                    if (nleg[q]) atomicAdd(&s_cnt[j * SPL + q], nleg[q]);
                    nleg[q] = 0;
                }
                asm volatile("s_waitcnt vmcnt(0)" ::: "memory");
                __syncthreads();
                GSTAMP(5);
                if (tid < GW) {
                    if (s_cnt[tid])
                        __hip_atomic_fetch_add(log_slot + (size_t)(it + 1) * GS_MAX + tid, s_cnt[tid], __ATOMIC_RELAXED,
                                               __HIP_MEMORY_SCOPE_AGENT);
                    s_cnt[tid] = 0;
                }
                if (w == 0) {
                    asm volatile("s_waitcnt vmcnt(0)" ::: "memory");
                    if (lane < BAR_REPS)
                        __hip_atomic_fetch_add(&bar->sub[it & 1][lane][blockIdx.x % BAR_SUBS].w, 1ull << 32, __ATOMIC_RELAXED,
                                               __HIP_MEMORY_SCOPE_AGENT);
                    const unsigned long long rounds = (unsigned long long)((it >> 1) + 1);
                    unsigned polls = 0;
                    const unsigned long long t_start = wall_clock64();
                    bool ok = true;
                    for (;;) {
                        const unsigned long long word = lane < (int)subs_used ? bar_load(&bar->sub[it & 1][my_rep][lane].w) : 0;
                        if (__ballot((word >> 32) >= n_sub * rounds) == ~0ull) break;
                        if ((polls++ & 63u) == 63u && wall_clock64() - t_start > limit_ticks + 100000000ull) {
                            ok = false;
                            break;
                        }
                        __builtin_amdgcn_s_sleep(BAR_POLL_SLEEP);
                    }
                    if (lane == 0 && !ok) s_flag[1] = 1;
                }
                __syncthreads();
                GSTAMP(6);
                sweeps_done = it + 1;
                if (s_flag[1]) {
                    fault = true;
                    break;
                }
            }
        }
        if constexpr (MULTI) break;
        g = g_next;
    }
    const int tid = tid0;
    if constexpr (MULTI) {
        if (blockIdx.x == 0 && tid < GS_MAX) {
            const int f = (tid < GW && !converged && !fault)
                              ? (int)gs_ldu<true>(reinterpret_cast<const uint32_t *>(log_slot + (size_t)sweeps_done * GS_MAX + tid)) : 0;
            cnt_out[tid] = f;
            cnt_zero[tid] = 0;
        }
        if (blockIdx.x == 0 && tid == 0)
            *status = sweeps_done | (fault ? GSM_FAULT : 0) | (converged ? GSM_CONVERGED : 0);
        if (ecount) atomicAdd(&s_edges, (unsigned long long)ecount);
        __syncthreads();
        if (tid == 0 && s_edges) stats->blk_E[blockIdx.x] += s_edges;
        return;
    }
#ifdef DPPR_STAMPS
    if (!MULTI && stamp_dense && tid == 0 && blockIdx.x < 4096) g_stamps[blockIdx.x * 8 + 6] = wall_clock64();
#endif
#pragma unroll
    for (int q = 0; q < SPL; ++q)
        if (nleg[q]) atomicAdd(&s_cnt[j * SPL + q], nleg[q]);
    if (ecount) atomicAdd(&s_edges, (unsigned long long)ecount);
    __syncthreads();
    if (tid < GW && s_cnt[tid]) atomicAdd(&cnt_out[tid], s_cnt[tid]);
    if (tid == 0 && s_edges) stats->blk_E[blockIdx.x] += s_edges;
}

__global__ __launch_bounds__(BLOCK) void k_gint_to_ext(const double *__restrict__ a_int, int gw, int lane_s,
                                                       const int *__restrict__ ext2int, int V,
                                                       double *__restrict__ a_ext) {
    for (int v = blockIdx.x * BLOCK + threadIdx.x; v < V; v += gridDim.x * BLOCK) {
        const int m = ext2int[v];
        a_ext[v] = m >= 0 ? a_int[(size_t)m * gw + lane_s] : 0.0;
    }
}

}
```

### dynamicppr_amd/engine.py

```python
from __future__ import annotations

import ctypes as C
import os
import subprocess

import numpy as np

_HERE = os.path.dirname(os.path.abspath(__file__))
LIB_PATH = os.environ.get("DPPR_LIB") or os.path.join(_HERE, "libdppr_hip.so")

SCHEDULE_EAGER = 0
SCHEDULE_SYNC = 1


class DpprError(RuntimeError):
    pass


class Stats(C.Structure):
    _fields_ = [("iterations", C.c_int64), ("sum_F", C.c_int64), ("sum_E", C.c_int64), ("sum_N", C.c_int64),
                ("records", C.c_int64), ("inspected", C.c_int64), ("batches", C.c_int64),
                ("pull_iterations", C.c_int64),
                ("algorithmic_bytes", C.c_int64), ("gpu_ms", C.c_double), ("push_ms", C.c_double),
                ("push_launches", C.c_int64), ("persist_launches", C.c_int64), ("persist_aborts", C.c_int64),
                ("binned_sweeps", C.c_int64), ("sweep_F", C.c_int64), ("sweep_E", C.c_int64), ("sweep_ms", C.c_double),
                ("sweep_launches", C.c_int64)]

    def as_dict(self):
        return {k: getattr(self, k) for k, _ in self._fields_}


def build(force: bool = False) -> str:
    csrc = os.path.join(_HERE, "csrc")
    srcs = [os.path.join(csrc, f) for f in os.listdir(csrc) if f.endswith((".hip", ".hpp"))]
    srcs.append(os.path.join(os.path.dirname(_HERE), "include", "dppr.h"))
    stale = (not os.path.exists(LIB_PATH)) or any(os.path.getmtime(s) > os.path.getmtime(LIB_PATH) for s in srcs)
    if force or stale:
        subprocess.check_call(["make", "-C", csrc, "-s", "all"])
    return LIB_PATH


_lib = None
EXPORTS = [
    "dppr_abi_version", "dppr_strerror", "dppr_last_error", "dppr_create", "dppr_destroy", "dppr_set_schedule", "dppr_set_profiling", "dppr_set_tuning", "dppr_set_persistent", "dppr_set_incremental_graph",
    "dppr_load_window", "dppr_set_batch", "dppr_slide", "dppr_add_source", "dppr_init_solve", "dppr_update",
    "dppr_incremental_batch_update", "dppr_execute_main_loop", "dppr_read", "dppr_write", "dppr_stats",
    "dppr_reset_stats", "dppr_inspect", "dppr_read_graph", "dppr_graph_edges", "dppr_read_out_graph", "dppr_trace_enable",
    "dppr_trace_get", "dppr_synchronize", "dppr_bench_atomics",
    "dppr_add_source_group", "dppr_group_init_solve", "dppr_group_update", "dppr_group_read", "dppr_group_stats",
    "dppr_group_reset_stats", "dppr_set_group_seeding", "dppr_seed_lists", "dppr_set_sweep_bitmap", "dppr_set_group_resident", "dppr_set_resident_slots", "dppr_set_resident_update",
    "dppr_set_renumbering", "dppr_id_space", "dppr_set_group_push", "dppr_set_binned_sweep", "dppr_device_count", "dppr_set_phase_merge", "dppr_init_solve_at", "dppr_group_init_solve_at", "dppr_set_variant", "dppr_set_batch_grouping",
    "dppr_time_batch_grouping", "dppr_debug_dump", "dppr_hint_next_batch",
    "dppr_bench_line_fills", "dppr_bench_stream_copy", "dppr_build_id", "dppr_heartbeat", "dppr_slide_concurrent", "dppr_renumbering_due", "dppr_debug_bin_tables",
    "dppr_debug_grouping", "dppr_topk", "dppr_group_topk", "dppr_read_at", "dppr_group_read_at", "dppr_debug_live_bytes",
    "dppr_group_sources", "dppr_group_replace_source", "dppr_group_add_source", "dppr_group_remove_source",
    "dppr_group_topk_weighted", "dppr_group_score_at", "dppr_debug_query_ms",
    "dppr_mark", "dppr_group_mark", "dppr_unmark", "dppr_group_unmark", "dppr_changes", "dppr_group_changes",
    "dppr_support", "dppr_group_support", "dppr_export_sparse", "dppr_group_export_sparse", "dppr_export_dense_dev",
    "dppr_group_export_dense_dev",
    "dppr_patch", "dppr_group_patch",
    "dppr_dot_dense_dev", "dppr_group_dot_dense_dev", "dppr_dot_sparse", "dppr_group_dot_sparse",
    "dppr_walks", "dppr_refine_at", "dppr_group_refine_at", "dppr_debug_id_map", "dppr_debug_walk_form",
    "dppr_cluster", "dppr_group_cluster",
    "dppr_subgraph", "dppr_group_subgraph", "dppr_debug_subgraph_wave_max",
    "dppr_add_target_group", "dppr_group_replace_target", "dppr_group_targets",
    "dppr_topk_ranked", "dppr_group_topk_ranked", "dppr_rank_score_at", "dppr_group_rank_score_at", "dppr_debug_rank_piece",
    "dppr_assign", "dppr_assign_at",
    "dppr_position_at", "dppr_group_position_at", "dppr_debug_position_tile",
    "dppr_explain_at", "dppr_group_explain_at", "dppr_debug_explain",
    "dppr_certify", "dppr_group_certify", "dppr_debug_certify",
    "dppr_sample", "dppr_group_sample", "dppr_debug_sample_form",
]

DEST_HOST, DEST_DEVICE = 0, 1
DENSE_P, DENSE_R = 0, 1
F64, F32 = 0, 1
VERTEX_MAJOR, SOURCE_MAJOR = 0, 1
DOT_MAX_F = 4096
H_FEATURE_MAJOR, H_VERTEX_MAJOR = 0, 1
WALK_MAX_M, WALK_MAX_W, WALK_MAX_TOTAL = 4096, 1 << 20, 1 << 26
WALK_REFILL, WALK_PER_THREAD = 0, 1
CLUSTER_MAX = 8192
SUBGRAPH_MAX = 8192
TARGET_SET_MAX = 65536
FACTOR_NONE, FACTOR_DEV, FACTOR_DEG, FACTOR_INV_DEG = 0, 1, 2, 3
MASK_NONE, MASK_ALLOW, MASK_DENY = 0, 1, 2
EXCLUDE_SEEDS, EXCLUDE_IN_NEIGHBOURS, EXCLUDE_OUT_NEIGHBOURS = 1, 2, 4
RANK_PIECE = 512
ASSIGN_GROUPS_MAX, ASSIGN_CLASSES_MAX = 16, 256
POSITION_MAX = 4096
EXPLAIN_MAX_M, EXPLAIN_MAX_F, EXPLAIN_MAX_DEPTH = 4096, 16, 64
END_SEED, END_DEPTH, END_DEAD, END_CYCLE = 0, 1, 2, 3
CERT_RESIDUAL, CERT_INVARIANT = 1, 2
PATCH_KEEP_MARK, PATCH_REMARK_ALL, PATCH_REMARK_EMITTED = 0, 1, 2
SAMPLE_MAX, SAMPLE_MAX_TOTAL = 1 << 20, 1 << 24
SAMPLE_OK, SAMPLE_EMPTY, SAMPLE_NONFINITE = 0, 1, 2
SAMPLE_WAVE, SAMPLE_PER_THREAD = 0, 1


class RankSpec(C.Structure):
    _fields_ = [("factor", C.c_int32), ("factor_dtype", C.c_int32), ("factor_dev", C.c_void_p), ("mask", C.c_int32),
                ("mask_dev", C.c_void_p), ("exclude", C.c_uint32)]


class ExplainOut(C.Structure):
    _ip, _dp = C.POINTER(C.c_int32), C.POINTER(C.c_double)
    _fields_ = [("deg", _ip), ("distinct", _ip), ("self", _dp), ("nbr_count", _ip), ("nbr", _ip), ("nbr_mult", _ip), ("nbr_c", _dp),
                ("len", _ip), ("end", _ip), ("path", _ip), ("path_p", _dp), ("path_c", _dp)]


class CertifyOut(C.Structure):
    _ip, _dp, _lp = C.POINTER(C.c_int32), C.POINTER(C.c_double), C.POINTER(C.c_int64)
    _fields_ = [("max_abs_r", _dp), ("argmax_r", _ip), ("sum_abs_r", _dp), ("sum_p", _dp), ("n_pos", _lp), ("n_neg", _lp),
                ("n_nonfinite", _lp), ("n_p_nonzero", _lp), ("inv_max_err", _dp), ("inv_argmax", _ip),
                ("state_epoch", C.c_int32), ("converged", C.c_int32), ("conv_eps", C.c_double)]


class PatchOut(C.Structure):
    _fields_ = [("up_offsets", C.POINTER(C.c_int64)), ("up_ids", C.c_void_p), ("up_p", C.c_void_p),
                ("del_offsets", C.POINTER(C.c_int64)), ("del_ids", C.c_void_p), ("written", C.c_int32)]


def apply_patch(replica, patch):
    off, ids, p = (np.asarray(a) for a in replica[:3])
    n = len(off) - 1
    uo, do = patch["up_offsets"], patch["del_offsets"]
    if len(uo) != n + 1 or len(do) != n + 1:
        raise ValueError(f"apply_patch: the replica has {n} lanes, the patch {len(uo) - 1}")
    out_ids, out_p, out_off = [], [], np.zeros(n + 1, dtype=np.int64)
    for i in range(n):
        li, lp = ids[off[i]:off[i + 1]], p[off[i]:off[i + 1]]
        ui, up = patch["up_ids"][uo[i]:uo[i + 1]], patch["up_p"][uo[i]:uo[i + 1]]
        di = patch["del_ids"][do[i]:do[i + 1]]
        keep = ~np.isin(li, di) & ~np.isin(li, ui)
        mi, mp = np.concatenate([li[keep], ui]), np.concatenate([lp[keep], up])
        order = np.argsort(mi, kind="stable")
        out_ids.append(mi[order])
        out_p.append(mp[order])
        out_off[i + 1] = out_off[i] + len(mi)
    return out_off, np.concatenate(out_ids).astype(np.int32), np.concatenate(out_p).astype(np.float64)


class Cluster(C.Structure):
    _fields_ = [("count", C.c_int32), ("best_size", C.c_int32), ("best_cut", C.c_int64), ("best_vol", C.c_int64),
                ("best_phi", C.c_double)]

    def as_dict(self):
        return {k: getattr(self, k) for k, _ in self._fields_}


def lib():
    global _lib
    if _lib is not None:
        return _lib
    if not os.path.exists(LIB_PATH):
        raise DpprError(f"{LIB_PATH} is missing: run `python -c 'import __graft_entry__ as g; g.build()'` "
                        "(the HIP extension is mandatory, there is no CPU fallback)")
    L = C.CDLL(LIB_PATH)
    vp, ip, dp, u8p = C.c_void_p, C.POINTER(C.c_int32), C.POINTER(C.c_double), C.POINTER(C.c_uint8)
    i64p, fp = C.POINTER(C.c_int64), C.POINTER(C.c_float)
    L.dppr_abi_version.restype = C.c_int
    L.dppr_strerror.argtypes = [C.c_int]
    L.dppr_strerror.restype = C.c_char_p
    L.dppr_last_error.argtypes = [vp]
    L.dppr_last_error.restype = C.c_char_p
    L.dppr_create.argtypes = [C.POINTER(vp), C.c_int, C.c_int32, C.c_int32, C.c_int, C.c_int32, C.c_int32]
    L.dppr_destroy.argtypes = [vp]
    L.dppr_destroy.restype = None
    L.dppr_set_schedule.argtypes = [vp, C.c_int]
    L.dppr_set_profiling.argtypes = [vp, C.c_int]
    L.dppr_set_incremental_graph.argtypes = [vp, C.c_int]
    L.dppr_set_renumbering.argtypes = [vp, C.c_int, C.c_int, C.c_int]
    L.dppr_set_group_push.argtypes = [vp, C.c_int, C.c_int, C.c_int64]
    L.dppr_id_space.argtypes = [vp, C.POINTER(C.c_int32), C.POINTER(C.c_int32), C.POINTER(C.c_int32), C.POINTER(C.c_int64)]
    L.dppr_set_tuning.argtypes = [vp, C.c_int, C.c_int, C.c_int, C.c_int, C.c_int]
    L.dppr_set_persistent.argtypes = [vp, C.c_int, C.c_int64]
    L.dppr_load_window.argtypes = [vp, ip, ip, C.c_int32]
    L.dppr_set_batch.argtypes = [vp, ip, ip, u8p, C.c_int32]
    L.dppr_slide.argtypes = [vp, ip, ip, C.c_int32, ip]
    L.dppr_add_source.argtypes = [vp, C.c_int32, ip]
    L.dppr_init_solve.argtypes = [vp, C.c_int32, C.c_double, fp]
    L.dppr_init_solve_at.argtypes = [vp, C.c_int32, C.c_int32, C.c_double, fp]
    L.dppr_group_init_solve_at.argtypes = [vp, C.c_int32, C.c_int32, C.c_double, fp]
    L.dppr_update.argtypes = [vp, C.c_int32, C.c_int32, C.c_double, fp]
    L.dppr_incremental_batch_update.argtypes = [vp, C.c_int32, C.c_int32]
    L.dppr_execute_main_loop.argtypes = [vp, C.c_int32, C.c_int32, C.c_int, C.c_double]
    L.dppr_read.argtypes = [vp, C.c_int32, dp, dp]
    L.dppr_write.argtypes = [vp, C.c_int32, dp, dp]
    L.dppr_stats.argtypes = [vp, C.c_int32, C.POINTER(Stats)]
    L.dppr_reset_stats.argtypes = [vp, C.c_int32]
    L.dppr_inspect.argtypes = [vp, C.c_int32, C.c_int, C.c_double, ip, ip]
    L.dppr_read_graph.argtypes = [vp, C.c_int32, ip, ip, ip]
    L.dppr_graph_edges.argtypes = [vp, C.c_int32, ip]
    L.dppr_read_out_graph.argtypes = [vp, C.c_int32, ip, ip]
    L.dppr_trace_enable.argtypes = [vp, C.c_int32, C.c_int]
    L.dppr_trace_get.argtypes = [vp, C.c_int32, i64p, i64p, i64p, ip]
    L.dppr_synchronize.argtypes = [vp]
    L.dppr_add_source_group.argtypes = [vp, ip, C.c_int32, ip]
    L.dppr_group_init_solve.argtypes = [vp, C.c_int32, C.c_double, fp]
    L.dppr_group_update.argtypes = [vp, C.c_int32, C.c_int32, C.c_double, fp]
    L.dppr_group_read.argtypes = [vp, C.c_int32, C.c_int32, dp, dp]
    L.dppr_group_stats.argtypes = [vp, C.c_int32, C.POINTER(Stats)]
    L.dppr_set_sweep_bitmap.argtypes = [vp, C.c_int]
    L.dppr_set_phase_merge.argtypes = [vp, C.c_int, C.c_int]
    L.dppr_set_variant.argtypes = [vp, C.c_int]
    L.dppr_set_batch_grouping.argtypes = [vp, C.c_int]
    L.dppr_set_binned_sweep.argtypes = [vp, C.c_int, C.c_int, C.c_int, C.c_int64, C.c_int64, C.c_int64, C.c_int64]
    L.dppr_set_group_resident.argtypes = [vp, C.c_int]
    L.dppr_set_resident_slots.argtypes = [vp, C.c_int]
    L.dppr_set_resident_update.argtypes = [vp, C.c_int]
    L.dppr_seed_lists.argtypes = [vp, C.c_int32, C.c_int, ip, ip]
    L.dppr_group_reset_stats.argtypes = [vp, C.c_int32]
    L.dppr_set_group_seeding.argtypes = [vp, C.c_int]
    L.dppr_bench_atomics.argtypes = [C.c_int, C.c_int64, C.c_int64, C.c_int, C.c_int, fp]
    L.dppr_time_batch_grouping.argtypes = [vp, C.c_int32, C.c_int32, fp]
    L.dppr_debug_dump.argtypes = [vp, C.c_char_p, C.c_int32]
    L.dppr_hint_next_batch.argtypes = [vp, ip, ip, C.c_int32, ip, ip, C.c_int32]
    L.dppr_bench_line_fills.argtypes = [C.c_int, C.c_int64, C.c_int64, C.c_int, fp]
    L.dppr_bench_stream_copy.argtypes = [C.c_int, C.c_int64, C.c_int, fp]
    L.dppr_build_id.restype = C.c_char_p
    L.dppr_heartbeat.argtypes = [vp]
    L.dppr_slide_concurrent.argtypes = [vp, ip, ip, C.c_int32, ip]
    L.dppr_renumbering_due.argtypes = [vp]
    u16p = C.POINTER(C.c_uint16)
    L.dppr_debug_bin_tables.argtypes = [vp, C.c_int32, ip, ip, ip, ip, ip, ip, ip, u16p, ip, ip, u16p, ip, i64p, i64p]
    u32p = C.POINTER(C.c_uint32)
    L.dppr_debug_grouping.argtypes = [vp, C.c_int32, C.c_int32, u32p, u32p, ip, ip, ip]
    L.dppr_heartbeat.restype = C.c_ulonglong
    L.dppr_topk.argtypes = [vp, C.c_int32, C.c_int32, C.c_double, ip, dp, dp, ip]
    L.dppr_group_topk.argtypes = [vp, C.c_int32, C.c_int32, C.c_double, ip, dp, dp, ip]
    L.dppr_read_at.argtypes = [vp, C.c_int32, ip, C.c_int32, dp, dp]
    L.dppr_group_read_at.argtypes = [vp, C.c_int32, ip, C.c_int32, dp, dp]
    L.dppr_debug_live_bytes.argtypes = [i64p, i64p]
    L.dppr_group_sources.argtypes = [vp, C.c_int32, ip, ip]
    L.dppr_group_replace_source.argtypes = [vp, C.c_int32, C.c_int32, C.c_int32, fp]
    L.dppr_group_add_source.argtypes = [vp, C.c_int32, C.c_int32, ip, fp]
    L.dppr_group_remove_source.argtypes = [vp, C.c_int32, C.c_int32]
    L.dppr_group_topk_weighted.argtypes = [vp, C.c_int32, dp, C.c_int32, C.c_int32, C.c_double, ip, dp, ip]
    L.dppr_group_score_at.argtypes = [vp, C.c_int32, dp, C.c_int32, ip, C.c_int32, dp]
    L.dppr_debug_query_ms.argtypes = [vp, fp]
    for name in ("dppr_mark", "dppr_group_mark", "dppr_unmark", "dppr_group_unmark"):
        getattr(L, name).argtypes = [vp, C.c_int32]
    L.dppr_changes.argtypes = [vp, C.c_int32, C.c_int32, C.c_double, C.c_int, ip, dp, dp, ip, ip]
    L.dppr_group_changes.argtypes = [vp, C.c_int32, C.c_int32, C.c_double, C.c_int, ip, dp, dp, ip, ip]
    L.dppr_support.argtypes = [vp, C.c_int32, C.c_double, i64p]
    L.dppr_group_support.argtypes = [vp, C.c_int32, C.c_double, i64p]
    L.dppr_export_sparse.argtypes = [vp, C.c_int32, C.c_double, C.c_int64, C.c_int, i64p, vp, vp, vp]
    L.dppr_group_export_sparse.argtypes = [vp, C.c_int32, C.c_double, C.c_int64, C.c_int, i64p, vp, vp, vp]
    L.dppr_export_dense_dev.argtypes = [vp, C.c_int32, C.c_int, C.c_int, vp]
    L.dppr_patch.argtypes = [vp, C.c_int32, C.c_double, C.c_double, C.c_int64, C.c_int64, C.c_int, C.c_int, vp]
    L.dppr_group_patch.argtypes = [vp, C.c_int32, C.c_double, C.c_double, C.c_int64, C.c_int64, C.c_int, C.c_int, vp]
    L.dppr_group_export_dense_dev.argtypes = [vp, C.c_int32, C.c_int, C.c_int, C.c_int, vp]
    L.dppr_dot_dense_dev.argtypes = [vp, C.c_int32, C.c_int, vp, C.c_int, C.c_int, C.c_int32, C.c_int, vp]
    L.dppr_group_dot_dense_dev.argtypes = [vp, C.c_int32, C.c_int, vp, C.c_int, C.c_int, C.c_int32, C.c_int, vp]
    L.dppr_dot_sparse.argtypes = [vp, C.c_int32, C.c_int, i64p, vp, vp, C.c_int, C.c_int32, C.c_int, vp]
    L.dppr_group_dot_sparse.argtypes = [vp, C.c_int32, C.c_int, i64p, vp, vp, C.c_int, C.c_int32, C.c_int, vp]
    L.dppr_walks.argtypes = [vp, C.c_int32, ip, C.c_int32, C.c_int32, C.c_uint64, C.c_int, vp]
    L.dppr_refine_at.argtypes = [vp, C.c_int32, C.c_int32, ip, C.c_int32, C.c_int32, C.c_uint64, vp, vp, vp]
    L.dppr_group_refine_at.argtypes = [vp, C.c_int32, C.c_int32, ip, C.c_int32, C.c_int32, C.c_uint64, vp, vp, vp]
    L.dppr_debug_id_map.argtypes = [vp, ip]
    L.dppr_cluster.argtypes = [vp, C.c_int32, C.c_int32, C.c_int32, C.c_double, C.c_int32, vp, vp, vp, vp, vp]
    L.dppr_group_cluster.argtypes = [vp, C.c_int32, C.c_int32, C.c_int32, C.c_double, C.c_int32, vp, vp, vp, vp, vp]
    L.dppr_subgraph.argtypes = [vp, C.c_int32, C.c_int32, C.c_int32, C.c_double, C.c_int64, C.c_int, vp, vp, vp, vp, vp, vp]
    L.dppr_group_subgraph.argtypes = [vp, C.c_int32, C.c_int32, C.c_int32, C.c_double, C.c_int64, C.c_int, vp, vp, vp, vp, vp, vp]
    L.dppr_debug_subgraph_wave_max.argtypes = [vp, C.c_int]
    L.dppr_debug_walk_form.argtypes = [vp, C.c_int]
    L.dppr_add_target_group.argtypes = [vp, i64p, ip, dp, C.c_int32, ip]
    L.dppr_group_replace_target.argtypes = [vp, C.c_int32, C.c_int32, ip, dp, C.c_int32, fp]
    L.dppr_group_targets.argtypes = [vp, C.c_int32, i64p, ip, dp, C.c_int64]
    L.dppr_topk_ranked.argtypes = [vp, C.c_int32, C.c_int32, vp, C.c_int32, C.c_double, ip, dp, ip]
    L.dppr_group_topk_ranked.argtypes = [vp, C.c_int32, C.c_int32, vp, C.c_int32, C.c_double, ip, dp, ip]
    L.dppr_rank_score_at.argtypes = [vp, C.c_int32, C.c_int32, vp, ip, C.c_int32, dp]
    L.dppr_group_rank_score_at.argtypes = [vp, C.c_int32, C.c_int32, vp, ip, C.c_int32, dp]
    L.dppr_debug_rank_piece.argtypes = [vp, C.c_int]
    L.dppr_position_at.argtypes = [vp, C.c_int32, C.c_int32, vp, C.c_double, ip, C.c_int32, ip, ip]
    L.dppr_group_position_at.argtypes = [vp, C.c_int32, C.c_int32, vp, C.c_double, ip, C.c_int32, ip, ip]
    L.dppr_debug_position_tile.argtypes = [vp, C.c_int]
    L.dppr_sample.argtypes = [vp, C.c_int32, C.c_int32, vp, C.c_double, C.c_uint64, C.c_uint64, C.c_int32, C.c_int, vp, vp, dp, ip, ip]
    L.dppr_group_sample.argtypes = [vp, C.c_int32, C.c_int32, vp, C.c_double, C.c_uint64, C.c_uint64, C.c_int32, C.c_int, vp, vp, dp, ip, ip]
    L.dppr_debug_sample_form.argtypes = [vp, C.c_int]
    L.dppr_explain_at.argtypes = [vp, C.c_int32, C.c_int32, ip, C.c_int32, C.c_int32, C.c_int32, vp]
    L.dppr_group_explain_at.argtypes = [vp, C.c_int32, C.c_int32, ip, C.c_int32, C.c_int32, C.c_int32, vp]
    L.dppr_debug_explain.argtypes = [vp, C.c_int, C.c_int]
    L.dppr_certify.argtypes = [vp, C.c_int32, C.c_int32, C.c_double, C.c_int, vp]
    L.dppr_group_certify.argtypes = [vp, C.c_int32, C.c_int32, C.c_double, C.c_int, vp]
    L.dppr_debug_certify.argtypes = [vp, C.c_int, C.c_int]
    L.dppr_assign.argtypes = [vp, ip, C.c_int32, dp, C.c_double, C.c_int, vp, vp, vp, i64p, vp, C.c_int64, i64p, vp, vp, vp]
    L.dppr_assign_at.argtypes = [vp, ip, C.c_int32, dp, C.c_double, ip, C.c_int32, ip, dp, ip, dp]
    for name in EXPORTS:
        if name not in ("dppr_strerror", "dppr_last_error", "dppr_destroy", "dppr_build_id", "dppr_heartbeat"):
            getattr(L, name).restype = C.c_int
    _lib = L
    return L


def rank_metrics(pos_column, ks):
    pos = [int(p) for p in np.asarray(pos_column).reshape(-1)]
    ks = [int(k) for k in ks]
    rr, hits = 0.0, {k: 0 for k in ks}
    for p in pos:
        if p < 0:
            continue
        rr += 1.0 / (p + 1)
        for k in ks:
            if p < k:
                hits[k] += 1
    m = len(pos)
    if m == 0:
        return 0.0, {k: 0.0 for k in ks}
    return rr / m, {k: hits[k] / m for k in ks}


def _i32(a):
    a = np.ascontiguousarray(a, dtype=np.int32)
    return a, a.ctypes.data_as(C.POINTER(C.c_int32))


class Engine:

    def __init__(self, V, W, directed, max_batch, n_epochs=1, device=0, schedule=SCHEDULE_EAGER,
                 hub_min_degree=None, big_row_edges=None, pull_min_frontier=None, chunk_iters=None, pull_block=None,
                 persistent=None, persist_timeout_us=None, sweep_bitmap=None, binned=None, merge_phases=None, variant=None, group_at_slide=None, resident_slots=None, resident_update=None):
        self._L = lib()
        self._h = C.c_void_p()
        self._batch_len, self._staged_len = {0: 0}, 0
        self._group_n = {}
        self.V, self.W, self.directed, self.c = int(V), int(W), int(directed), int(max_batch)
        self.device = int(device)
        rc = self._L.dppr_create(C.byref(self._h), int(device), self.V, self.W, self.directed, self.c, int(n_epochs))
        if rc:
            self._h = C.c_void_p()
            raise DpprError(f"dppr_create: {self._L.dppr_strerror(rc).decode()}")
        self.set_schedule(schedule)
        if variant is not None:
            self._ck(self._L.dppr_set_variant(self._h, int(variant)), "set_variant")
        if any(v is not None for v in (hub_min_degree, big_row_edges, pull_min_frontier, chunk_iters, pull_block)):
            self._ck(self._L.dppr_set_tuning(self._h, int(hub_min_degree or 256), int(big_row_edges or 512),
                                             int(pull_min_frontier or 0), int(chunk_iters or 0),
                                             int(pull_block or 0)), "set_tuning")
        if sweep_bitmap is not None:
            self._ck(self._L.dppr_set_sweep_bitmap(self._h, int(sweep_bitmap)), "set_sweep_bitmap")
        if group_at_slide is not None:
            self._ck(self._L.dppr_set_batch_grouping(self._h, int(group_at_slide)), "set_batch_grouping")
        if resident_slots is not None:
            self.set_resident_slots(resident_slots)
        if resident_update is not None:
            self._ck(self._L.dppr_set_resident_update(self._h, int(resident_update)), "set_resident_update")
        if merge_phases is not None:
            self.set_phase_merge(bool(merge_phases), 0 if merge_phases is True or not merge_phases else int(merge_phases))
        if binned is not None:
            args = (binned,) if isinstance(binned, int) else tuple(binned)
            args = tuple(int(a) for a in args) + (0,) * (7 - len(args))
            self._ck(self._L.dppr_set_binned_sweep(self._h, *args), "set_binned_sweep")
        if persistent is not None or persist_timeout_us is not None:
            self._ck(self._L.dppr_set_persistent(self._h, 1 if persistent is None else int(persistent),
                                                 int(persist_timeout_us or 0)), "set_persistent")

    def _ck(self, rc, what):
        if rc:
            raise DpprError(f"{what}: {self._L.dppr_strerror(rc).decode()} ({self._L.dppr_last_error(self._h).decode()})")

    def close(self):
# ... 677 lines not shown

    def dot_dense_dev(self, slot, h_ptr, F, which=DENSE_P, dtype=F64, layout=H_FEATURE_MAJOR, out_ptr=None):
        return self._dot_dense(self._L.dppr_dot_dense_dev, slot, 1, h_ptr, F, which, dtype, layout, out_ptr, True, "dot_dense_dev")

    def group_dot_dense_dev(self, group, h_ptr, F, which=DENSE_P, dtype=F64, layout=H_FEATURE_MAJOR, out_ptr=None):
        return self._dot_dense(self._L.dppr_group_dot_dense_dev, group, self._group_n.get(group, 1), h_ptr, F, which, dtype, layout,
                               out_ptr, False, "group_dot_dense_dev")

    def _dot_dense(self, fn, handle, n, h_ptr, F, which, dtype, layout, out_ptr, flat, what):
        if out_ptr is not None:
            self._ck(fn(self._h, int(handle), int(which), h_ptr or None, int(dtype), int(layout), int(F), DEST_DEVICE, out_ptr or None), what)
            return None
        out = np.empty((max(int(F), 0), n), dtype=np.float64)
        self._ck(fn(self._h, int(handle), int(which), h_ptr or None, int(dtype), int(layout), int(F), DEST_HOST, out.ctypes.data), what)
        return out[:, 0] if flat else out

    def dot_sparse(self, slot, offsets, ids, w, which=DENSE_P, out_ptr=None):
        return self._dot_sparse(self._L.dppr_dot_sparse, slot, 1, offsets, ids, w, which, out_ptr, True, "dot_sparse")

    def group_dot_sparse(self, group, offsets, ids, w, which=DENSE_P, out_ptr=None):
        return self._dot_sparse(self._L.dppr_group_dot_sparse, group, self._group_n.get(group, 1), offsets, ids, w, which, out_ptr, False,
                                "group_dot_sparse")

    def dot_sparse_dev(self, slot, offsets, ids_ptr, w_ptr, which=DENSE_P, out_ptr=None):
        return self._dot_sparse(self._L.dppr_dot_sparse, slot, 1, offsets, ids_ptr, w_ptr, which, out_ptr, True, "dot_sparse_dev", DEST_DEVICE)

    def group_dot_sparse_dev(self, group, offsets, ids_ptr, w_ptr, which=DENSE_P, out_ptr=None):
        return self._dot_sparse(self._L.dppr_group_dot_sparse, group, self._group_n.get(group, 1), offsets, ids_ptr, w_ptr, which, out_ptr,
                                False, "group_dot_sparse_dev", DEST_DEVICE)

    def _dot_sparse(self, fn, handle, n, offsets, ids, w, which, out_ptr, flat, what, src=DEST_HOST):
        off = np.ascontiguousarray(offsets, dtype=np.int64)
        F = len(off) - 1
        if src == DEST_HOST:
            ids = np.ascontiguousarray(ids, dtype=np.int32)
            w = np.ascontiguousarray(w, dtype=np.float64)
            if len(off) == 0 or len(ids) != len(w) or len(ids) < int(off[-1]):
                raise DpprError(f"{what}: offsets [F + 1]; ids and w must hold offsets[F] entries each")
            ids_ptr, w_ptr = ids.ctypes.data, w.ctypes.data
        else:
            ids_ptr, w_ptr = ids or None, w or None
        offp = off.ctypes.data_as(C.POINTER(C.c_int64))
        if out_ptr is not None:
            self._ck(fn(self._h, int(handle), int(which), offp, ids_ptr, w_ptr, int(src), F, DEST_DEVICE, out_ptr or None), what)
            return None
        out = np.empty((max(F, 0), n), dtype=np.float64)
        self._ck(fn(self._h, int(handle), int(which), offp, ids_ptr, w_ptr, int(src), F, DEST_HOST, out.ctypes.data), what)
        return out[:, 0] if flat else out

    def walks(self, starts, W, seed=0, epoch=-1):
        a, pa = _i32(starts)
        out = np.empty((len(a), max(int(W), 0)), dtype=np.int32)
        self._ck(self._L.dppr_walks(self._h, int(epoch), pa, len(a), int(W), int(seed), DEST_HOST, out.ctypes.data), "walks")
        return out

    def walks_dev(self, starts, W, seed, out_ptr, epoch=-1):
        a, pa = _i32(starts)
        self._ck(self._L.dppr_walks(self._h, int(epoch), pa, len(a), int(W), int(seed), DEST_DEVICE, out_ptr), "walks")

    def refine_at(self, slot, ids, W, seed=0, epoch=-1, corr=True, sumsq=True):
        return self._refine(self._L.dppr_refine_at, slot, 1, ids, W, seed, epoch, corr, sumsq, True, "refine_at")

    def group_refine_at(self, group, ids, W, seed=0, epoch=-1, corr=True, sumsq=True):
        return self._refine(self._L.dppr_group_refine_at, group, self._group_n[group], ids, W, seed, epoch, corr, sumsq, False, "group_refine_at")

    def _refine(self, fn, handle, n, ids, W, seed, epoch, corr, sumsq, flat, what):
        a, pa = _i32(ids)
        outs = [np.empty((len(a), n), dtype=np.float64) if want else None for want in (True, corr, sumsq)]
        self._ck(fn(self._h, int(handle), int(epoch), pa, len(a), int(W), int(seed), *[None if o is None else o.ctypes.data for o in outs]), what)
        return tuple(None if o is None else (o[:, 0] if flat else o) for o in outs)

    def cluster(self, slot, k, min_p=0.0, min_size=1, epoch=-1, profile=False):
        best, arrays = self._cluster(self._L.dppr_cluster, slot, 1, k, min_p, min_size, epoch, profile, "cluster")
        return (best[0], *[a[0] for a in arrays]) if profile else best[0]

    def group_cluster(self, group, k, min_p=0.0, min_size=1, epoch=-1, profile=False):
        best, arrays = self._cluster(self._L.dppr_group_cluster, group, self._group_n.get(group, 1), k, min_p, min_size, epoch, profile,
                                     "group_cluster")
        return (best, *arrays) if profile else best

    def _cluster(self, fn, which, n, k, min_p, min_size, epoch, profile, what):
        kk = max(int(k), 1)
        best = (Cluster * n)()
        arrays = [np.empty((n, kk), dtype=dt) for dt in (np.int32, np.int64, np.int64, np.int64)] if profile else []
        self._ck(fn(self._h, int(which), int(epoch), int(k), float(min_p), int(min_size), C.addressof(best),
                    *([a.ctypes.data for a in arrays] if profile else [None] * 4)), what)
        return [b.as_dict() for b in best], arrays

    def subgraph(self, slot, k, min_p=0.0, epoch=-1):
        cnt, _, ids, p, row_ptr, col = self._subgraph(self._L.dppr_subgraph, slot, 1, k, min_p, epoch, "subgraph")
        return int(cnt[0]), ids[0], p[0], row_ptr[0], col

    def group_subgraph(self, group, k, min_p=0.0, epoch=-1):
        return self._subgraph(self._L.dppr_group_subgraph, group, self._group_n.get(group, 1), k, min_p, epoch, "group_subgraph")

    def _subgraph(self, fn, which, n, k, min_p, epoch, what):
        kk = max(int(k), 1)
        cnt, off = np.zeros(n, dtype=np.int32), np.zeros(n + 1, dtype=np.int64)
        ids, p = np.empty((n, kk), dtype=np.int32), np.empty((n, kk), dtype=np.float64)
        row_ptr = np.empty((n, kk + 1), dtype=np.int64)
        head = (self._h, int(which), int(epoch), int(k), float(min_p))
        self._ck(fn(*head, 0, DEST_HOST, cnt.ctypes.data, off.ctypes.data, ids.ctypes.data, p.ctypes.data, row_ptr.ctypes.data, None), what)
        total = int(off[n])
        col = np.empty(total, dtype=np.int32)
        if total:
            self._ck(fn(*head, total, DEST_HOST, cnt.ctypes.data, off.ctypes.data, None, None, None, col.ctypes.data), what)
            if int(off[n]) != total:
                raise DpprError(f"{what}: the state changed between the size call and the fill")
        return cnt, off, ids, p, row_ptr, col

    def group_subgraph_dev(self, group, k, min_p, cap, ids_ptr, p_ptr, row_ptr_ptr, col_ptr, epoch=-1):
        return self._subgraph_dev(self._L.dppr_group_subgraph, group, self._group_n.get(group, 1), k, min_p, cap, ids_ptr, p_ptr,
                                  row_ptr_ptr, col_ptr, epoch, "group_subgraph_dev")

    def subgraph_dev(self, slot, k, min_p, cap, ids_ptr, p_ptr, row_ptr_ptr, col_ptr, epoch=-1):
        return self._subgraph_dev(self._L.dppr_subgraph, slot, 1, k, min_p, cap, ids_ptr, p_ptr, row_ptr_ptr, col_ptr, epoch, "subgraph_dev")

    def _subgraph_dev(self, fn, which, n, k, min_p, cap, ids_ptr, p_ptr, row_ptr_ptr, col_ptr, epoch, what):
        cnt, off = np.zeros(n, dtype=np.int32), np.zeros(n + 1, dtype=np.int64)
        self._ck(fn(self._h, int(which), int(epoch), int(k), float(min_p), int(cap), DEST_DEVICE, cnt.ctypes.data, off.ctypes.data,
                    ids_ptr or None, p_ptr or None, row_ptr_ptr or None, col_ptr or None), what)
        return cnt, off

    def set_subgraph_wave_max(self, wave_max):
        self._ck(self._L.dppr_debug_subgraph_wave_max(self._h, int(wave_max)), "set_subgraph_wave_max")

    def id_map(self):
        out = np.empty(self.V, dtype=np.int32)
        self._ck(self._L.dppr_debug_id_map(self._h, out.ctypes.data_as(C.POINTER(C.c_int32))), "debug_id_map")
        return out

    def set_walk_form(self, form):
        self._ck(self._L.dppr_debug_walk_form(self._h, int(form)), "debug_walk_form")

    def query_ms(self):
        ms = C.c_float(0)
        self._ck(self._L.dppr_debug_query_ms(self._h, C.byref(ms)), "debug_query_ms")
        return ms.value

    def group_stats(self, group):
        st = Stats()
        self._ck(self._L.dppr_group_stats(self._h, group, C.byref(st)), "group_stats")
        return st.as_dict()

    def group_reset_stats(self, group):
        self._ck(self._L.dppr_group_reset_stats(self._h, group), "group_reset_stats")

    def set_resident_slots(self, sorted_slots):
        self._ck(self._L.dppr_set_resident_slots(self._h, int(sorted_slots)), "set_resident_slots")

    def set_group_resident(self, on):
        self._ck(self._L.dppr_set_group_resident(self._h, int(on)), "set_group_resident")

    def set_group_seeding(self, from_tails):
        self._ck(self._L.dppr_set_group_seeding(self._h, int(from_tails)), "set_group_seeding")

    def synchronize(self):
        self._ck(self._L.dppr_synchronize(self._h), "synchronize")

    def time_batch_grouping(self, epoch=-1, reps=5):
        ms = C.c_float(0)
        self._ck(self._L.dppr_time_batch_grouping(self._h, int(epoch), int(reps), C.byref(ms)), "time_batch_grouping")
        return ms.value

    def debug_grouping(self, epoch=-1, path=0):
        L = self._batch_len.get(max(self._batch_len) if epoch < 0 else int(epoch), 0)
        cap = max(4 * self.c, 1)
        tails, index = np.zeros(cap, np.uint32), np.zeros(cap, np.uint32)
        raw = np.zeros(cap, np.int32)
        taken, nb = C.c_int32(0), C.c_int32(0)
        u32p = C.POINTER(C.c_uint32)
        self._ck(self._L.dppr_debug_grouping(self._h, int(epoch), int(path), tails.ctypes.data_as(u32p), index.ctypes.data_as(u32p),
                                             raw.ctypes.data_as(C.POINTER(C.c_int32)), C.byref(taken), C.byref(nb)), "debug_grouping")
        return tails[:L].copy(), index[:L].copy(), raw[:L].copy(), taken.value, nb.value

    def debug_dump(self):
        buf = C.create_string_buffer(1 << 16)
        n = self._L.dppr_debug_dump(self._h, buf, len(buf))
        return buf.raw[:max(n, 0)].decode(errors="replace")


def bench_atomics(table_elems, n, scope=0, reps=5, device=0):
    ms = C.c_float(0)
    rc = lib().dppr_bench_atomics(int(device), int(table_elems), int(n), int(scope), int(reps), C.byref(ms))
    if rc:
        raise DpprError(f"bench_atomics: {lib().dppr_strerror(rc).decode()}")
    return ms.value


def bench_line_fills(table_bytes=1 << 30, lines=1 << 26, reps=3, device=0):
    ms = C.c_float(0)
    rc = lib().dppr_bench_line_fills(int(device), int(table_bytes), int(lines), int(reps), C.byref(ms))
    if rc:
        raise DpprError(f"bench_line_fills: {lib().dppr_strerror(rc).decode()}")
    return ms.value


def bench_stream_copy(nbytes=1 << 30, reps=5, device=0):
    ms = C.c_float(0)
    rc = lib().dppr_bench_stream_copy(int(device), int(nbytes), int(reps), C.byref(ms))
    if rc:
        raise DpprError(f"bench_stream_copy: {lib().dppr_strerror(rc).decode()}")
    return ms.value


def live_bytes():
    dev, pin = C.c_int64(0), C.c_int64(0)
    rc = lib().dppr_debug_live_bytes(C.byref(dev), C.byref(pin))
    if rc:
        raise DpprError(f"debug_live_bytes: {lib().dppr_strerror(rc).decode()}")
    return dev.value, pin.value


def build_id():
    return lib().dppr_build_id().decode()
```

### include/dppr.h

```cpp
#ifndef DPPR_H
#define DPPR_H

#include <stdint.h>

#ifdef __cplusplus
extern "C" {
#endif

#define DPPR_ABI_VERSION 6

typedef struct dppr_engine dppr_engine;

typedef enum dppr_status {
    DPPR_OK = 0,
    DPPR_ERR_INVALID = -1,
    DPPR_ERR_HIP = -2,
    DPPR_ERR_NOMEM = -3,
    DPPR_ERR_NO_DEVICE = -4,
    DPPR_ERR_NOT_CONVERGED = -5
} dppr_status;

#define DPPR_SCHEDULE_EAGER 0
#define DPPR_SCHEDULE_SYNC 1

// ... 162 lines not shown
#define DPPR_WALK_MAX_M 4096
#define DPPR_WALK_MAX_W (1 << 20)
int dppr_walks(dppr_engine *e, int32_t epoch, const int32_t *starts , int32_t m, int32_t W, uint64_t seed,
               int dest, int32_t *out_ends );
int dppr_refine_at(dppr_engine *e, int32_t slot, int32_t epoch, const int32_t *ids, int32_t m, int32_t W, uint64_t seed,
                   double *out_est , double *out_corr , double *out_sumsq );
int dppr_group_refine_at(dppr_engine *e, int32_t group, int32_t epoch, const int32_t *ids, int32_t m, int32_t W, uint64_t seed,
                         double *out_est , double *out_corr ,
                         double *out_sumsq );
int dppr_debug_id_map(dppr_engine *e, int32_t *out_ext2int );
int dppr_debug_walk_form(dppr_engine *e, int form);

#define DPPR_CLUSTER_MAX DPPR_TOPK_MAX
typedef struct {
    int32_t count;
    int32_t best_size;
    int64_t best_cut;
    int64_t best_vol;
    double  best_phi;
} dppr_cluster_t;
int dppr_cluster(dppr_engine *e, int32_t slot, int32_t epoch, int32_t k, double min_p, int32_t min_size,
                 dppr_cluster_t *out_best,
                 int32_t *out_ids , int64_t *out_cut_out ,
                 int64_t *out_cut_in , int64_t *out_vol );
int dppr_group_cluster(dppr_engine *e, int32_t group, int32_t epoch, int32_t k, double min_p, int32_t min_size,
                       dppr_cluster_t *out_best ,
                       int32_t *out_ids , int64_t *out_cut_out ,
                       int64_t *out_cut_in , int64_t *out_vol );

#define DPPR_SUBGRAPH_MAX DPPR_TOPK_MAX
int dppr_subgraph(dppr_engine *e, int32_t slot, int32_t epoch, int32_t k, double min_p, int64_t cap, int dest,
                  int32_t *out_count , int64_t *out_offsets ,
                  int32_t *out_ids , double *out_p ,
                  int64_t *out_row_ptr , int32_t *out_col );
int dppr_group_subgraph(dppr_engine *e, int32_t group, int32_t epoch, int32_t k, double min_p, int64_t cap, int dest,
                        int32_t *out_counts , int64_t *out_offsets ,
                        int32_t *out_ids , double *out_p ,
                        int64_t *out_row_ptr , int32_t *out_col );
int dppr_debug_subgraph_wave_max(dppr_engine *e, int wave_max);

#define DPPR_FACTOR_NONE      0
#define DPPR_FACTOR_DEV       1
#define DPPR_FACTOR_DEG       2
#define DPPR_FACTOR_INV_DEG   3
#define DPPR_MASK_NONE  0
#define DPPR_MASK_ALLOW 1
#define DPPR_MASK_DENY  2
#define DPPR_EXCLUDE_SEEDS          1u
#define DPPR_EXCLUDE_IN_NEIGHBOURS  2u
#define DPPR_EXCLUDE_OUT_NEIGHBOURS 4u
typedef struct {
    int32_t factor, factor_dtype;
    const void *factor_dev;
    int32_t mask;
    const uint8_t *mask_dev;
    uint32_t exclude;
} dppr_rank_spec_t;
int dppr_topk_ranked(dppr_engine *e, int32_t slot, int32_t epoch, const dppr_rank_spec_t *spec, int32_t k, double min_score,
                     int32_t *out_ids, double *out_score, int32_t *out_count);
int dppr_group_topk_ranked(dppr_engine *e, int32_t group, int32_t epoch, const dppr_rank_spec_t *spec, int32_t k, double min_score,
                           int32_t *out_ids , double *out_score , int32_t *out_counts );
int dppr_rank_score_at(dppr_engine *e, int32_t slot, int32_t epoch, const dppr_rank_spec_t *spec, const int32_t *ids, int32_t m,
                       double *out_score );
int dppr_group_rank_score_at(dppr_engine *e, int32_t group, int32_t epoch, const dppr_rank_spec_t *spec, const int32_t *ids, int32_t m,
                             double *out_score );
int dppr_debug_rank_piece(dppr_engine *e, int edges);

#define DPPR_POSITION_MAX 4096
int dppr_position_at(dppr_engine *e, int32_t slot, int32_t epoch, const dppr_rank_spec_t *spec, double min_score,
                     const int32_t *ids, int32_t m, int32_t *out_pos , int32_t *out_count );
int dppr_group_position_at(dppr_engine *e, int32_t group, int32_t epoch, const dppr_rank_spec_t *spec, double min_score,
                           const int32_t *ids, int32_t m, int32_t *out_pos ,
                           int32_t *out_counts );
int dppr_debug_position_tile(dppr_engine *e, int queries);

#define DPPR_EXPLAIN_MAX_M 4096
#define DPPR_EXPLAIN_MAX_F 16
#define DPPR_EXPLAIN_MAX_DEPTH 64
#define DPPR_EXPLAIN_END_SEED 0
#define DPPR_EXPLAIN_END_DEPTH 1
#define DPPR_EXPLAIN_END_DEAD 2
#define DPPR_EXPLAIN_END_CYCLE 3
typedef struct {
    int32_t *deg, *distinct;
    double *self;
    int32_t *nbr_count;
    int32_t *nbr, *nbr_mult; double *nbr_c;
    int32_t *len, *end;
    int32_t *path; double *path_p;
    double *path_c;
} dppr_explain_out_t;
int dppr_explain_at(dppr_engine *e, int32_t slot, int32_t epoch, const int32_t *ids, int32_t m, int32_t f, int32_t depth,
                    const dppr_explain_out_t *out);
int dppr_group_explain_at(dppr_engine *e, int32_t group, int32_t epoch, const int32_t *ids, int32_t m, int32_t f, int32_t depth,
                          const dppr_explain_out_t *out);
int dppr_debug_explain(dppr_engine *e, int memo , int wave_rows );

#define DPPR_CERT_RESIDUAL  1
#define DPPR_CERT_INVARIANT 2
typedef struct {
    double  *max_abs_r;   int32_t *argmax_r;
    double  *sum_abs_r;   double  *sum_p;
    int64_t *n_pos;       int64_t *n_neg;
    int64_t *n_nonfinite;
    int64_t *n_p_nonzero;
    double  *inv_max_err; int32_t *inv_argmax;
    int32_t state_epoch;  int32_t converged;  double conv_eps;
} dppr_certify_out_t;
int dppr_certify(dppr_engine *e, int32_t slot, int32_t epoch, double eps, int flags, dppr_certify_out_t *out);
int dppr_group_certify(dppr_engine *e, int32_t group, int32_t epoch, double eps, int flags, dppr_certify_out_t *out);
int dppr_debug_certify(dppr_engine *e, int piece_edges , int wave_rows );

#define DPPR_ASSIGN_GROUPS_MAX  16
#define DPPR_ASSIGN_CLASSES_MAX 256
int dppr_assign(dppr_engine *e, const int32_t *groups, int32_t n_groups, const double *scale , double min_score, int dest,
                int32_t *out_label , double *out_best , double *out_margin ,
                int64_t *out_counts , const int32_t *prev_label , int64_t cap,
                int64_t *out_n_flips , int32_t *flip_id, int32_t *flip_old, int32_t *flip_new);
int dppr_assign_at(dppr_engine *e, const int32_t *groups, int32_t n_groups, const double *scale, double min_score, const int32_t *ids,
                   int32_t m, int32_t *out_label , double *out_best , int32_t *out_second_label ,
                   double *out_margin );

#define DPPR_PATCH_KEEP_MARK 0
#define DPPR_PATCH_REMARK_ALL 1
#define DPPR_PATCH_REMARK_EMITTED 2
typedef struct {
    int64_t *up_offsets;
    int32_t *up_ids;
    double *up_p;
    int64_t *del_offsets;
    int32_t *del_ids;
    int32_t written;
} dppr_patch_out_t;
int dppr_patch(dppr_engine *e, int32_t slot, double min_p, double min_delta, int64_t cap_up, int64_t cap_del, int dest, int remark,
               dppr_patch_out_t *out);
int dppr_group_patch(dppr_engine *e, int32_t group, double min_p, double min_delta, int64_t cap_up, int64_t cap_del, int dest,
                     int remark, dppr_patch_out_t *out);

#define DPPR_SAMPLE_MAX        (1 << 20)
#define DPPR_SAMPLE_MAX_TOTAL  (1 << 24)
#define DPPR_SAMPLE_OK         0
#define DPPR_SAMPLE_EMPTY      1
#define DPPR_SAMPLE_NONFINITE  2
int dppr_sample(dppr_engine *e, int32_t slot, int32_t epoch, const dppr_rank_spec_t *spec, double min_score, uint64_t seed,
                uint64_t first, int32_t S, int dest, int32_t *out_ids , double *out_w ,
                double *out_total , int32_t *out_support , int32_t *out_status );
int dppr_group_sample(dppr_engine *e, int32_t group, int32_t epoch, const dppr_rank_spec_t *spec, double min_score, uint64_t seed,
                      uint64_t first, int32_t S, int dest, int32_t *out_ids ,
                      double *out_w , double *out_total ,
                      int32_t *out_support , int32_t *out_status );
int dppr_debug_sample_form(dppr_engine *e, int form);

int dppr_set_group_resident(dppr_engine *e, int on);
int dppr_set_resident_slots(dppr_engine *e, int sorted);
int dppr_set_resident_update(dppr_engine *e, int on);
int dppr_set_group_push(dppr_engine *e, int enter_pairs, int list_cap, int64_t max_edges);

int dppr_set_group_seeding(dppr_engine *e, int from_tails);


int dppr_inspect(dppr_engine *e, int32_t slot, int phase, double eps, int32_t *out_ids, int32_t *out_count);

int dppr_read_graph(dppr_engine *e, int32_t epoch, int32_t *row_ptr, int32_t *col, int32_t *out_degree);
int dppr_graph_edges(dppr_engine *e, int32_t epoch, int32_t *out_directed_edges);
int dppr_read_out_graph(dppr_engine *e, int32_t epoch, int32_t *row_ptr, int32_t *col);

int dppr_trace_enable(dppr_engine *e, int32_t slot, int on);
int dppr_trace_get(dppr_engine *e, int32_t slot, int64_t *n_iters, int64_t *n_ids,
                   int64_t *offsets, int32_t *ids);

int dppr_synchronize(dppr_engine *e);

int dppr_hint_next_batch(dppr_engine *e, const int32_t *b1, const int32_t *b2, int32_t L, const int32_t *n1, const int32_t *n2, int32_t c);

int dppr_time_batch_grouping(dppr_engine *e, int32_t epoch, int32_t reps, float *out_ms);
int dppr_debug_grouping(dppr_engine *e, int32_t epoch, int32_t path, uint32_t *tails_out, uint32_t *index_out, int32_t *raw_tails_out,
                        int32_t *path_taken, int32_t *nb_out);

int dppr_debug_dump(dppr_engine *e, char *buf, int32_t cap);
int dppr_debug_bin_tables(dppr_engine *e, int32_t epoch, int32_t *n_a, int32_t *n_b, int32_t *n_edges, int32_t *n_runs, int32_t *n_tiles,
                          int32_t *acut, int32_t *bcut, uint16_t *hl, int32_t *tdelta, int32_t *tb, uint16_t *dl, int32_t *vb,
                          int64_t *patched, int64_t *rebuilt);
int dppr_debug_live_bytes(int64_t *device_bytes, int64_t *pinned_bytes);

unsigned long long dppr_heartbeat(const dppr_engine *e);

int dppr_bench_atomics(int device, int64_t table_elems, int64_t n, int scope, int reps, float *out_ms);
int dppr_bench_line_fills(int device, int64_t table_bytes, int64_t lines, int reps, float *out_ms);
int dppr_bench_stream_copy(int device, int64_t bytes, int reps, float *out_ms);

const char *dppr_build_id(void);

#ifdef __cplusplus
}
#endif
#endif
```

Baseline: 56.17 million.

## Add list-based group sweep and ticket runs to the group sweep kernel

```diff
diff --git a/dynamicppr_amd/csrc/dppr_engine.hip b/dynamicppr_amd/csrc/dppr_engine.hip
--- a/dynamicppr_amd/csrc/dppr_engine.hip
+++ b/dynamicppr_amd/csrc/dppr_engine.hip
@@ -102,6 +102,15 @@
     if (const char *v = diag_env("DPPR_HOT_BLOCKS")) e->hot_blocks = atoi(v) != 0;
     if (const char *v = diag_env("DPPR_GSWEEP_HOT")) e->gsweep_hot_rows = std::max(0, atoi(v));
     if (const char *v = diag_env("DPPR_GSWEEP_GRID")) e->gsweep_grid_cap = std::max(1, std::min(atoi(v), STAT_SLOTS));
+    if (const char *v = diag_env("DPPR_GSWEEP_FORM")) {
+        int a[4] = {-1, 0, -1, 0};
+        sscanf(v, "%d,%d,%d,%d", &a[0], &a[1], &a[2], &a[3]);
+        (void)dppr_set_group_sweep_form(e, a[0], a[1], a[2], a[3]);
+    }
+    if (const char *v = diag_env("DPPR_GSWEEP_AUTO")) {
+        sscanf(v, "%d,%d,%d", &e->gsweep_auto[0], &e->gsweep_auto[1], &e->gsweep_auto[2]);
+        for (int &x : e->gsweep_auto) x = std::max(0, std::min(x, 1 << 16));
+    }
     if (const char *v = diag_env("DPPR_RENUMBER")) e->renumber_on = atoi(v) != 0;
     if (const char *v = diag_env("DPPR_RENUMBER_PCT")) e->renumber_growth_pct = std::max(1, atoi(v));
     if (const char *v = diag_env("DPPR_RENUMBER_MIN")) e->renumber_min_parked = std::max(1, atoi(v));
@@ -313,6 +322,17 @@
 int dppr_set_group_resident(dppr_engine *e, int on) {
     if (!e) return DPPR_ERR_INVALID;
     e->group_resident = on != 0;
+    return DPPR_OK;
+}
+
+int dppr_set_group_sweep_form(dppr_engine *e, int list_gate, int list_cap, int ticket_run, int grid_cap) {
+    if (!e || list_gate < -1 || list_gate > 1 || list_cap < 0 || list_cap > GS_LIST_MAX || ticket_run < -1 || ticket_run == 0 ||
+        ticket_run > (1 << 16) || grid_cap < 0)
+        return fail(e, DPPR_ERR_INVALID, "set_group_sweep_form: list_gate -1 / 0 / 1, list_cap 0 .. 1024, ticket_run -1 or 1 .. 65536, grid_cap >= 0");
+    e->gsweep_list_gate = list_gate;
+    e->gsweep_list_cap = list_cap;
+    e->gsweep_ticket_run = ticket_run;
+    e->gsweep_grid_test_cap = std::min(grid_cap, STAT_SLOTS);
     return DPPR_OK;
 }
 
@@ -1080,13 +1100,13 @@
     HIP_TRY_MSG("add_source_group: ", g.act[1].alloc(g.act_bytes / sizeof(uint32_t)));
     HIP_TRY_MSG("add_source_group: ", g.cnt.alloc(5 * GS_MAX + MAX_CHUNK * GS_MAX));
     HIP_TRY_MSG("add_source_group: ", g.mlog.alloc((size_t)(GMULTI_MAX + 2) * GS_MAX));
-    HIP_TRY_MSG("add_source_group: ", g.dstats.alloc(2));
+    HIP_TRY_MSG("add_source_group: ", g.dstats.alloc(3));
     HIP_TRY_MSG("add_source_group: ", g.gq.alloc(3 * GQ_PAD));
     HIP_TRY_MSG("add_source_group: ", hipMemsetAsync(g.gq, 0, sizeof(int) * 3 * GQ_PAD, e->stream));
     HIP_TRY_MSG("add_source_group: ", hipMemsetAsync(g.act[0], 0, g.act_bytes, e->stream));
     HIP_TRY_MSG("add_source_group: ", hipMemsetAsync(g.act[1], 0, g.act_bytes, e->stream));
     HIP_TRY_MSG("add_source_group: ", hipMemsetAsync(g.cnt, 0, sizeof(int) * (5 * GS_MAX + MAX_CHUNK * GS_MAX), e->stream));
-    HIP_TRY_MSG("add_source_group: ", hipMemsetAsync(g.dstats, 0, 2 * sizeof(IterStats), e->stream));
+    HIP_TRY_MSG("add_source_group: ", hipMemsetAsync(g.dstats, 0, 3 * sizeof(IterStats), e->stream));
     if (ts) HIP_TRY_MSG("add_target_group: ", g.tg.alloc(tg_bytes(ts->total())));
     if (ts) {
         for (int s = 0; s < n; ++s)
@@ -1672,7 +1692,19 @@
 int dppr_group_reset_stats(dppr_engine *e, int32_t group) {
     GET_GROUP(e, group);
     HIP_TRY(hipSetDevice(e->device));
+    HIP_TRY(hipMemsetAsync(gs_form_words(g.dstats + 1), 0, sizeof(unsigned long long) * GS_FORM_WORDS, e->stream));
     return solve_reset_stats(e, g);
+}
+
+int dppr_debug_group_sweep_forms(dppr_engine *e, int32_t group, int64_t out[4]) {
+    GET_GROUP(e, group);
+    if (!out) return DPPR_ERR_INVALID;
+    HIP_TRY(hipSetDevice(e->device));
+    unsigned long long h[GS_FORM_WORDS];
+    HIP_TRY(hipMemcpyAsync(h, gs_form_words(g.dstats + 1), sizeof(h), hipMemcpyDeviceToHost, e->stream));
+    HIP_TRY(hipStreamSynchronize(e->stream));
+    for (int k = 0; k < GS_FORM_WORDS; ++k) out[k] = (int64_t)h[k];
+    return DPPR_OK;
 }
 
 int dppr_group_stats(dppr_engine *e, int32_t group, dppr_stats_t *out) {
diff --git a/dynamicppr_amd/csrc/dppr_host_group.hpp b/dynamicppr_amd/csrc/dppr_host_group.hpp
--- a/dynamicppr_amd/csrc/dppr_host_group.hpp
+++ b/dynamicppr_amd/csrc/dppr_host_group.hpp
@@ -36,14 +36,29 @@
     int rollcall_extra = 0;
     int *q_take = nullptr, *q_zero = nullptr;
 };
+struct GSweepForm {
+    int list_below, list_cap, run_below, run_len;
+};
+GSweepForm group_sweep_form_args(const dppr_engine *e, int ids) {
+    auto frac = [&](int num, int den) { return (int)std::min<long long>((long long)ids * num / den, INT_MAX); };
+    GSweepForm f;
+    f.list_below = e->gsweep_list_gate < 0 ? frac(e->gsweep_auto[0], 64) : e->gsweep_list_gate ? INT_MAX : 0;
+    f.list_cap = e->gsweep_list_cap > 0 ? std::min(e->gsweep_list_cap, GS_LIST_MAX) : GS_LIST_MAX;
+    f.run_below = e->gsweep_ticket_run < 0 ? frac(e->gsweep_auto[1], 64) : INT_MAX;
+    f.run_len = e->gsweep_ticket_run < 0 ? std::max(e->gsweep_auto[2], 1) : e->gsweep_ticket_run;
+    return f;
+}
+
 template <bool MULTI>
 void launch_gsweep(dppr_engine *e, Group &g, const Epoch &ep, int phase, double eps, bool owed, const GSweepLaunch &a) {
+    const GSweepForm f = MULTI ? GSweepForm{0, GS_LIST_MAX, 0, 1} : group_sweep_form_args(e, ep.grp_n_int);
     with_row(g.gw, ep.ggrp_max_tiles * WAVE, [&](auto spl, auto gw, auto nvx) {
         auto go = [&](auto cm) {
             hipLaunchKernelGGL((k_gsweep<decltype(spl)::value, decltype(gw)::value, decltype(nvx)::value, MULTI, decltype(cm)::value>),
                                dim3(a.grid), dim3(GNT), 0, e->stream, ep.grp_n_int, ep.gtab, ep.n_ggroups, a.cnt_in, e->gsweep_hot_rows,
                                ep.out_col, g.x, g.x2, g.act[0], g.act[1], g.r, g.p, a.cnt_out, a.cnt_zero, phase, eps, g.dstats + 1, a.log,
-                               a.n, a.bar, a.status, a.ticks, a.rollcall_extra, owed ? 1 : 0, a.q_take, a.q_zero);
+                               a.n, a.bar, a.status, a.ticks, a.rollcall_extra, owed ? 1 : 0, a.q_take, a.q_zero, f.list_below, f.list_cap,
+                               f.run_below, f.run_len);
         };
         if constexpr (MULTI) go(IC<2>{});
         else if (owed) go(IC<1>{});
@@ -206,6 +221,17 @@
     }
     int sweep_chunk() {
         const int n = plan.next_chunk(g.hist, hp, it, lane_sum(e->pinned + ring.cur * GS_MAX), e->chunk_iters, e->chunk_explicit);
+        static const bool trace = getenv("DPPR_GROUP_TRACE") != nullptr;
+        static thread_local std::vector<unsigned long long> forms;
+        const bool trace_forms = trace && e->profiling;
+        auto snap_forms = [&](int row) {
+            return hipMemcpyAsync(forms.data() + (size_t)row * GS_FORM_WORDS, gs_form_words(g.dstats + 1), sizeof(unsigned long long) * GS_FORM_WORDS,
+                                  hipMemcpyDeviceToHost, e->stream);
+        };
+        if (trace_forms) {
+            forms.assign((size_t)(n + 1) * GS_FORM_WORDS, 0ull);
+            HIP_TRY(snap_forms(0));
+        }
         for (int k = 0; k < n; ++k) {
             int rc = timed_launch(e, k, e->profiling, [&] {
                 launch_gsweep<false>(e, g, ep, phase, eps, owed,
@@ -213,6 +239,7 @@
                                       g.gq + (g.gq_seq % 3) * GQ_PAD, g.gq + ((g.gq_seq + 1) % 3) * GQ_PAD});
             });
             if (rc) return rc;
+            if (trace_forms) HIP_TRY(snap_forms(k + 1));
             swap_snapshots(g, true);
             ring.rotate();
             g.gq_seq++;
@@ -225,8 +252,11 @@
             if (!e->profiling) return DPPR_OK;
             float ms = 0;
             if (int rc2 = credit_launch(e, g.st, k, true, &ms)) return rc2;
-            static const bool trace = getenv("DPPR_GROUP_TRACE") != nullptr;
-            if (trace) fprintf(stderr, "[gsweep] phase %d sweep %3d  frontier pairs %9lld  %7.1f us\n", phase, it + k, f, ms * 1e3);
+            if (trace) {
+                const unsigned long long *a = forms.data() + (size_t)k * GS_FORM_WORDS, *b = a + GS_FORM_WORDS;
+                fprintf(stderr, "[gsweep] phase %d sweep %3d  frontier pairs %9lld  %7.1f us  groups: list %llu, fell back %llu, no work %llu; run tickets %llu\n",
+                        phase, it + k, f, ms * 1e3, b[0] - a[0], b[1] - a[1], b[2] - a[2], b[3] - a[3]);
+            }
             return DPPR_OK;
         });
         if (rc) return rc;
@@ -282,7 +312,7 @@
         if (hipDeviceGetAttribute(&cus, hipDeviceAttributeMultiprocessorCount, e->device) != hipSuccess || cus <= 0) cus = 256;
         e->gsweep_grid_cap = std::min(2 * cus, STAT_SLOTS);
     }
-    l.sweep_grid = std::min(std::max(ep.n_ggroups, 1), e->gsweep_grid_cap);
+    l.sweep_grid = std::min(std::max(ep.n_ggroups, 1), e->gsweep_grid_test_cap > 0 ? std::min(e->gsweep_grid_test_cap, e->gsweep_grid_cap) : e->gsweep_grid_cap);
     l.plan.push_thr = group_push_threshold(e->gpush_enter_pairs, ep.n_ggroups, e->gpush_auto_factor);
     while (l.more) {
         if (l.it >= e->max_iters) return fail(e, DPPR_ERR_NOT_CONVERGED, "iteration cap hit");
diff --git a/dynamicppr_amd/csrc/dppr_host_state.hpp b/dynamicppr_amd/csrc/dppr_host_state.hpp
--- a/dynamicppr_amd/csrc/dppr_host_state.hpp
+++ b/dynamicppr_amd/csrc/dppr_host_state.hpp
@@ -320,6 +320,11 @@
     bool hot_blocks = true;
     int gsweep_hot_rows = 24576;
     int gsweep_grid_cap = 0;
+    int gsweep_list_gate = -1;
+    int gsweep_list_cap = 0;
+    int gsweep_ticket_run = -1;
+    int gsweep_grid_test_cap = 0;
+    int gsweep_auto[3] = {0, 0, 1};
     bool group_resident = true;
     int gmulti_cap[2] = {-1, -1};
     bool any_groups = false;
diff --git a/dynamicppr_amd/csrc/dppr_multi.hpp b/dynamicppr_amd/csrc/dppr_multi.hpp
--- a/dynamicppr_amd/csrc/dppr_multi.hpp
+++ b/dynamicppr_amd/csrc/dppr_multi.hpp
@@ -239,10 +239,136 @@
     else gs_st<COH>(p, v);
 }
 
+constexpr int GS_LIST_MAX = 1024;
+constexpr int GS_FORM_WORDS = 4;
+__host__ __device__ inline unsigned long long *gs_form_words(IterStats *sweep_block) {
+    return reinterpret_cast<unsigned long long *>(sweep_block + 1);
+}
+
 constexpr int GSM_ABORTED = 1 << 30;
 constexpr int GSM_FAULT = 1 << 29;
 constexpr int GSM_CONVERGED = 1 << 28;
 constexpr int GSM_SWEEPS = (1 << 16) - 1;
+
+#define DPPR_LDS __attribute__((address_space(3)))
+constexpr int GS_LIST_TESTS = 4;
+struct GsListLds {
+    DPPR_LDS double *acc;
+    DPPR_LDS int *cstart;
+    DPPR_LDS unsigned short *cvid;
+    DPPR_LDS int *ostart;
+    DPPR_LDS uint32_t *actin, *touched;
+    DPPR_LDS int *lhead;
+    DPPR_LDS unsigned short *lrow;
+    DPPR_LDS int *lcount, *lown;
+};
+template <int SPL, int GW, int NVX>
+__device__ __noinline__ unsigned long long gs_list_group(GsListLds s, const int *__restrict__ T, const int *__restrict__ cols, int Eg, int v0, int nv,
+                                                         const uint32_t *act_in, const double *x, int hot_rows, int phase, double eps, int lcap) {
+    constexpr int NOCT = GNT / OCT, WORDS = NVX / 32, XS = x_stride(GW), GB = 8 / SPL;
+    const int tid = threadIdx.x, j = tid & (OCT - 1), oid = tid / OCT;
+    const bool live = oct_live<SPL, GW>(j);
+    int lcol[GS_LIST_TESTS];
+    {
+        const int c0 = tid < NVX ? T[GT_HDR + tid] : 0;
+        const int os = tid < NOCT ? T[GT_HDR + NVX + 1 + tid] : 0;
+        const unsigned short cv = tid < NVX ? reinterpret_cast<const unsigned short *>(T + GT_HDR + NVX + 1 + NOCT)[tid] : 0;
+        const uint32_t wd = tid < WORDS && tid * 32 < nv ? act_in[(v0 >> 5) + tid] : 0u;
+#pragma unroll
+        for (int k = 0; k < GS_LIST_TESTS; ++k) lcol[k] = tid + k * GNT < Eg ? ld_stream(&cols[tid + k * GNT]) : -1;
+        if (tid < WORDS) {
+            s.actin[tid] = wd;
+            if (wd) *s.lown = 1;
+        }
+        if (tid < NVX) {
+            s.cstart[tid] = c0;
+            s.cvid[tid] = cv;
+        }
+        if (tid < NOCT) s.ostart[tid] = os;
+        if (tid == 0) s.cstart[NVX] = Eg;
+    }
+    {
+        uint32_t law[GS_LIST_TESTS];
+#pragma unroll
+        for (int k = 0; k < GS_LIST_TESTS; ++k) law[k] = lcol[k] >= 0 ? act_in[lcol[k] >> 5] : 0u;
+#pragma unroll
+        for (int k = 0; k < GS_LIST_TESTS; ++k) lcol[k] = lcol[k] >= 0 && ((law[k] >> (lcol[k] & 31)) & 1u) ? lcol[k] : -1;
+    }
+    __syncthreads();
+    int mine = 0;
+#pragma unroll
+    for (int k = 0; k < GS_LIST_TESTS; ++k) mine += __popcll(__ballot(lcol[k] >= 0));
+    if (mine) {
+        int base = 0;
+        if (lane_id() == 0) base = __hip_atomic_fetch_add(s.lcount, mine, __ATOMIC_RELAXED, __HIP_MEMORY_SCOPE_WORKGROUP);
+        base = __builtin_amdgcn_readfirstlane(base);
+#pragma unroll
+        for (int k = 0; k < GS_LIST_TESTS; ++k) {
+            const uint64_t bal = __ballot(lcol[k] >= 0);
+            const int pos = base + mbcnt(bal);
+            base += __popcll(bal);
+            if (lcol[k] >= 0 && pos < lcap) {
+                const int ek = tid + k * GNT;
+                int lo = 0;
+#pragma unroll
+                for (int step = NVX / 2; step > 0; step >>= 1)
+                    if (s.cstart[lo + step] <= ek) lo += step;
+                s.lhead[pos] = lcol[k];
+                s.lrow[pos] = (unsigned short)lo;
+            }
+        }
+    }
+    __syncthreads();
+    const int n_list = *s.lcount;
+    unsigned ecount = 0;
+    if (n_list <= lcap) {
+        int last = -1, vl = 0;
+        double den = 1.0, rcp = 1.0;
+        for (int b = oid; b < n_list; b += GB * NOCT) {
+            double xv[GB][SPL];
+#pragma unroll
+            for (int k = 0; k < GB; ++k) {
+#pragma unroll
+                for (int q = 0; q < SPL; ++q) xv[k][q] = 0.0;
+                if (b + k * NOCT < n_list && live) {
+                    const int hd = s.lhead[b + k * NOCT];
+                    if (!(DPPR_GS_NT & 1) || hd < hot_rows) {
+#pragma unroll
+                        for (int q = 0; q < SPL; ++q) xv[k][q] = x[(size_t)hd * XS + j * SPL + q];
+                    } else {
+#pragma unroll
+                        for (int q = 0; q < SPL; ++q) xv[k][q] = gs_ld_once<false, 1>(x + (size_t)hd * XS + j * SPL + q);
+                    }
+                }
+            }
+#pragma unroll
+            for (int k = 0; k < GB; ++k) {
+                if (b + k * NOCT < n_list) {
+                    const int cr = s.lrow[b + k * NOCT];
+                    if (cr != last) {
+                        last = cr;
+                        den = (double)(s.cstart[last + 1] - s.cstart[last] + 1);
+                        rcp = 1.0 / den;
+                        vl = s.cvid[last];
+                    }
+                    bool nz = false;
+#pragma unroll
+                    for (int q = 0; q < SPL; ++q) {
+                        if (legal(xv[k][q], phase, eps)) {
+                            const double term = push_term(xv[k][q], den, rcp);
+                            if (term != 0.0)
+                                __hip_atomic_fetch_add(&s.acc[vl * GW + j * SPL + q], term, __ATOMIC_RELAXED, __HIP_MEMORY_SCOPE_WORKGROUP);
+                            nz |= term != 0.0;
+                            ++ecount;
+                        }
+                    }
+                    if (nz) __hip_atomic_fetch_or(&s.touched[vl >> 5], 1u << (vl & 31), __ATOMIC_RELAXED, __HIP_MEMORY_SCOPE_WORKGROUP);
+                }
+            }
+        }
+    }
+    return ((unsigned long long)(unsigned)n_list << 32) | ecount;
+}
 
 template <int SPL, int GW, int NVX, bool MULTI, int CM>
 __global__ __launch_bounds__(GNT, MULTI ? 4 : 8) void k_gsweep(int V, const int *__restrict__ gtab, int n_groups,
@@ -252,7 +378,8 @@
                                                    int *cnt_zero, int phase, double eps, IterStats *__restrict__ stats,
                                                    int *log_slot, int n_iter, GridBar *bar, int *status,
                                                    unsigned long long limit_ticks, int rollcall_extra, int credit0,
-                                                   int *q_take, int *q_zero) {
+                                                   int *q_take, int *q_zero, int list_below, int list_cap, int run_below,
+                                                   int run_len) {
     constexpr int NOCT = GNT / OCT, WORDS = NVX / 32, XS = x_stride(GW);
     static_assert(sizeof(double) * NVX * GW <= 64 * 1024, "two workgroups per CU");
     constexpr int EB = 8;
@@ -273,6 +400,10 @@
     __shared__ unsigned long long s_edges;
     __shared__ int s_flag[2];
     __shared__ int s_ticket;
+    __shared__ int s_lhead[MULTI ? 1 : GS_LIST_MAX];
+    __shared__ unsigned short s_lrow[MULTI ? 1 : GS_LIST_MAX];
+    __shared__ int s_lcount, s_lown;
+    __shared__ int s_forms[GS_FORM_WORDS];
     const int tid0 = threadIdx.x, lane = lane_id(), w = wave_id();
     const int j = tid0 & (OCT - 1);
     auto opaque = [](int v) {
@@ -283,6 +414,8 @@
     };
 
     bool stamp_dense = false;
+    bool list_on = false;
+    int run = 1;
     if constexpr (!MULTI) {
         const int my_cnt = lane < GW ? cnt_in[lane] : 0;
         if (blockIdx.x == 0 && tid0 < GW) {
@@ -291,6 +424,9 @@
         }
         if (blockIdx.x == 0 && tid0 == 0) *q_zero = 0;
         if (__ballot(my_cnt != 0) == 0) return;
+        const unsigned F = (unsigned)__builtin_amdgcn_readlane(wave_inclusive_scan(my_cnt), WAVE - 1);
+        list_on = F < (unsigned)list_below;
+        run = F < (unsigned)run_below ? run_len : 1;
 #ifdef DPPR_STAMPS
 #if defined(DPPR_STAMP_MID)
         {
@@ -319,6 +455,10 @@
         s_edges = 0ull;
         s_flag[0] = 1;
         s_flag[1] = 0;
+        s_lcount = 0;
+        s_lown = 0;
+#pragma unroll
+        for (int k = 0; k < GS_FORM_WORDS; ++k) s_forms[k] = 0;
     }
     int nleg[SPL];
 #pragma unroll
@@ -374,18 +514,43 @@
     }
     int sweeps_done = 0;
     bool converged = false, fault = false;
+    int run_left = 0;
     for (int g = blockIdx.x; g < n_groups;) {
         __syncthreads();
         int ticket = 0, g_next = n_groups;
-        if (!MULTI && tid0 == 0) ticket = (int)gridDim.x + atomicAdd(q_take, 1);
+        if (!MULTI && run_left == 0 && tid0 == 0) ticket = (int)gridDim.x + run * atomicAdd(q_take, 1);
         const int *T = gtab + (size_t)g * STRIDE;
+        const int v0 = hv0, nv = hnv, E0 = hE0, Eg = hEg, per = hper;
+        const int *cols = out_col + E0;
+#ifndef DPPR_GS_LIST
+#define DPPR_GS_LIST 1
+#endif
+        const bool try_list = DPPR_GS_LIST && !MULTI && list_on && Eg <= GS_LIST_TESTS * GNT;
+        bool listed = false, idle = false;
+        if constexpr (!MULTI) {
+            if (try_list) {
+                const int lcap = min(list_cap, GS_LIST_MAX);
+                const GsListLds lds{(DPPR_LDS double *)s_acc,          (DPPR_LDS int *)s_cstart,       (DPPR_LDS unsigned short *)s_cvid,
+                                    (DPPR_LDS int *)s_ostart,          (DPPR_LDS uint32_t *)s_actin,   (DPPR_LDS uint32_t *)s_touched,
+                                    (DPPR_LDS int *)s_lhead,           (DPPR_LDS unsigned short *)s_lrow, (DPPR_LDS int *)&s_lcount,
+                                    (DPPR_LDS int *)&s_lown};
+                const unsigned long long res = gs_list_group<SPL, GW, NVX>(lds, T, cols, Eg, v0, nv, act_a, x_a, hot_rows, phase, eps, lcap);
+                listed = __builtin_amdgcn_readfirstlane((int)(res >> 32)) <= lcap;
+                if (listed) {
+                    idle = (res >> 32) == 0 && s_lown == 0;
+                    ecount += (unsigned)res;
+                }
+                if (tid0 == 0) {
+                    ++s_forms[listed ? 0 : 1];
+                    if (idle) ++s_forms[2];
+                }
+            }
+        }
         const int tid = opaque(tid0);
         const int j = tid & (OCT - 1), oid = tid / OCT;
         const bool live = oct_live<SPL, GW>(j);
-        const int v0 = hv0, nv = hnv, E0 = hE0, Eg = hEg, per = hper;
         const int e_begin = oid * per, e_end = min(Eg, e_begin + per);
-        const int *cols = out_col + E0;
-        {
+        if (!try_list) {
             const int c0 = tid < NVX ? T[GT_HDR + tid] : 0;
             const int os = tid < NOCT ? T[GT_HDR + NVX + 1 + tid] : 0;
             const unsigned short cv = tid < NVX ? reinterpret_cast<const unsigned short *>(T + GT_HDR + NVX + 1 + NOCT)[tid] : 0;
@@ -397,8 +562,11 @@
             if (tid < NOCT) s_ostart[tid] = os;
             if (tid == 0) s_cstart[NVX] = Eg;
         }
-        int mycol = e_begin + j < e_end ? ld_stream(&cols[e_begin + j]) : -1;
-        int ncol = e_begin + EB + j < e_end ? ld_stream(&cols[e_begin + EB + j]) : -1;
+        int mycol = -1, ncol = -1;
+        if (!listed) {
+            mycol = e_begin + j < e_end ? ld_stream(&cols[e_begin + j]) : -1;
+            ncol = e_begin + EB + j < e_end ? ld_stream(&cols[e_begin + EB + j]) : -1;
+        }
 
         for (int it = 0; it < (MULTI ? n_iter : 1); ++it) {
             const double *x = (it & 1) ? x_b : x_a;
@@ -424,7 +592,7 @@
             }
             __syncthreads();
 
-            if (e_begin < e_end) {
+            if (!listed && e_begin < e_end) {
                 int crow = s_ostart[oid];
                 int row_beg = s_cstart[crow], row_end = s_cstart[crow + 1];
                 double den = (double)(row_end - row_beg + 1);
@@ -510,19 +678,26 @@
                 }
                 flush();
             }
-            if (!MULTI && tid0 == 0) s_ticket = ticket;
+            if (!MULTI && run_left == 0 && tid0 == 0) s_ticket = ticket;
             GSTAMP(1);
             __syncthreads();
             GSTAMP(2);
             if constexpr (!MULTI) {
-                g_next = __builtin_amdgcn_readfirstlane(s_ticket);
+                if (run_left == 0) {
+                    g_next = __builtin_amdgcn_readfirstlane(s_ticket);
+                    run_left = run - 1;
+                    if (run > 1 && g_next + 1 < n_groups && tid0 == 0) ++s_forms[3];
+                } else {
+                    g_next = g + 1;
+                    --run_left;
+                }
                 if (g_next < n_groups) {
                     const int *H = gtab + (size_t)g_next * STRIDE;
                     hv0 = H[0]; hnv = H[1]; hE0 = H[2]; hEg = H[3]; hper = H[4];
                 }
             }
 
-            for (int i0 = 0; i0 < NVX / NOCT; i0 += FU) {
+            for (int i0 = 0; i0 < (!MULTI && idle ? 0 : NVX / NOCT); i0 += FU) {
                 const int tid_v = opaque(tid0);
                 const int j = tid_v & (OCT - 1), oid = tid_v / OCT;
                 const bool live = oct_live<SPL, GW>(j);
@@ -570,7 +745,11 @@
                             if (live) {
                                 double *ap = &s_acc[vl[i] * GW + j * SPL + q];
                                 a = *ap;
+#ifdef DPPR_GS_PLAIN_ZERO
                                 *ap = 0.0;
+#else
+                                *ap = __hiloint2double(opaque(0), opaque(0));
+#endif
                             }
                             pushed[q] = wasact[i] && legal(cur[i][q], phase, eps);
                             rn[q] = pushed[q] ? a : cur[i][q] + a;
@@ -612,6 +791,10 @@
                 if (tid * 32 < nv) gs_stu<MULTI>(act_out + (v0 >> 5) + tid, s_actout[tid]);
                 s_actout[tid] = 0u;
                 s_touched[tid] = 0u;
+            }
+            if (!MULTI && tid == 0) {
+                s_lcount = 0;
+                s_lown = 0;
             }
             if constexpr (MULTI) {
 #pragma unroll
@@ -685,6 +868,12 @@
     __syncthreads();
     if (tid < GW && s_cnt[tid]) atomicAdd(&cnt_out[tid], s_cnt[tid]);
     if (tid == 0 && s_edges) stats->blk_E[blockIdx.x] += s_edges;
+    if (tid == 0) {
+        unsigned long long *forms = gs_form_words(stats);
+#pragma unroll
+        for (int k = 0; k < GS_FORM_WORDS; ++k)
+            if (s_forms[k]) atomicAdd(&forms[k], (unsigned long long)s_forms[k]);
+    }
 }
 
 __global__ __launch_bounds__(BLOCK) void k_gint_to_ext(const double *__restrict__ a_int, int gw, int lane_s,
diff --git a/dynamicppr_amd/engine.py b/dynamicppr_amd/engine.py
--- a/dynamicppr_amd/engine.py
+++ b/dynamicppr_amd/engine.py
@@ -70,6 +70,7 @@
     "dppr_explain_at", "dppr_group_explain_at", "dppr_debug_explain",
     "dppr_certify", "dppr_group_certify", "dppr_debug_certify",
     "dppr_sample", "dppr_group_sample", "dppr_debug_sample_form",
+    "dppr_set_group_sweep_form", "dppr_debug_group_sweep_forms",
 ]
 
 DEST_HOST, DEST_DEVICE = 0, 1
@@ -208,6 +209,8 @@
     L.dppr_set_binned_sweep.argtypes = [vp, C.c_int, C.c_int, C.c_int, C.c_int64, C.c_int64, C.c_int64, C.c_int64]
     L.dppr_set_group_resident.argtypes = [vp, C.c_int]
     L.dppr_set_resident_slots.argtypes = [vp, C.c_int]
+    L.dppr_set_group_sweep_form.argtypes = [vp, C.c_int, C.c_int, C.c_int, C.c_int]
+    L.dppr_debug_group_sweep_forms.argtypes = [vp, C.c_int32, i64p]
     L.dppr_set_resident_update.argtypes = [vp, C.c_int]
     L.dppr_seed_lists.argtypes = [vp, C.c_int32, C.c_int, ip, ip]
     L.dppr_group_reset_stats.argtypes = [vp, C.c_int32]
@@ -1191,6 +1194,14 @@
     def set_group_resident(self, on):
         self._ck(self._L.dppr_set_group_resident(self._h, int(on)), "set_group_resident")
 
+    def set_group_sweep_form(self, list_gate=-1, list_cap=0, ticket_run=-1, grid_cap=0):
+        self._ck(self._L.dppr_set_group_sweep_form(self._h, int(list_gate), int(list_cap), int(ticket_run), int(grid_cap)), "set_group_sweep_form")
+
+    def debug_group_sweep_forms(self, group):
+        out = (C.c_int64 * 4)()
+        self._ck(self._L.dppr_debug_group_sweep_forms(self._h, group, out), "debug_group_sweep_forms")
+        return {"list": int(out[0]), "fell_back": int(out[1]), "no_work": int(out[2]), "run_tickets": int(out[3])}
+
     def set_group_seeding(self, from_tails):
         self._ck(self._L.dppr_set_group_seeding(self._h, int(from_tails)), "set_group_seeding")
 
diff --git a/include/dppr.h b/include/dppr.h
--- a/include/dppr.h
+++ b/include/dppr.h
@@ -338,6 +338,8 @@
 int dppr_debug_sample_form(dppr_engine *e, int form);
 
 int dppr_set_group_resident(dppr_engine *e, int on);
+int dppr_set_group_sweep_form(dppr_engine *e, int list_gate, int list_cap, int ticket_run, int grid_cap);
+int dppr_debug_group_sweep_forms(dppr_engine *e, int32_t group, int64_t out[4]);
 int dppr_set_resident_slots(dppr_engine *e, int sorted);
 int dppr_set_resident_update(dppr_engine *e, int on);
 int dppr_set_group_push(dppr_engine *e, int enter_pairs, int list_cap, int64_t max_edges);
```

New measurement: 55.38 million. -1.4%, worse.
